# Kizuna42/office-person-detection-vit

Measured on AMD Instinct MI355X. Metric: frames/sec (Phase-2 DETR detect) at 800x1333 batch 8, higher is better.
Workload: dtype f16

## Files before the change

office_person_detection_vit_amd/_capi.py:

```python

from __future__ import annotations

import ctypes as C
import os
from typing import Optional

_HERE = os.path.dirname(os.path.abspath(__file__))
LIB_PATH = os.path.join(_HERE, "libopd_hip.so")
TEST_LIB_PATH = os.path.join(_HERE, "libopd_hip_test.so")

OPD_PIXELS_U8_BGR_HWC = 0
OPD_PIXELS_F32_NCHW = 1
OPD_MEM_HOST = 0
OPD_MEM_DEVICE = 1
OPD_MEM_HOST_PIXELS_DEVICE_OUT = 2
OPD_FLAG_NO_GRAPH = 1
OPD_FLAG_MULTI_STREAM = 2
OPD_REID_MODEL_CLIP = 0
OPD_REID_MODEL_OSNET = 1
OPD_TRACK_FEAT_NONE, OPD_TRACK_FEAT_ENCODER, OPD_TRACK_FEAT_COLOR, OPD_TRACK_FEAT_REID = 0, 1, 2, 3
OPD_FLAG_BF16 = 4
OPD_FLOOR_HOMOGRAPHY, OPD_FLOOR_PWA, OPD_FLOOR_TPS = 0, 1, 2
OPD_FLOOR_VALID, OPD_FLOOR_WITHIN, OPD_FLOOR_EXTRAPOLATED = 1, 2, 4
OPD_FLOOR_MAX_POINTS, OPD_FLOOR_MAX_TRIANGLES, OPD_FLOOR_MAX_ZONES, OPD_FLOOR_MAX_VERTICES = 256, 512, 64, 64
# ... 187 lines not shown
    "opd_lwt_destroy": (None, [C.c_void_p]),
    "opd_lwt_reset": (C.c_int, [C.c_void_p]),
    "opd_lwt_info": (C.c_int, [C.c_void_p, C.POINTER(OpdLwtStatus)]),
    "opd_lwt_update": (C.c_int, [C.c_void_p, C.c_void_p, C.c_int, C.c_int, C.c_int, C.c_void_p, C.c_int, C.c_void_p]),
    "opd_lwt_interpolate": (C.c_int, [C.c_void_p, C.c_void_p, C.c_int, C.c_int, C.c_int, C.POINTER(OpdLwtRec), C.c_int, C.POINTER(C.c_int)]),
    "opd_lwt_get": (C.c_int, [C.c_void_p, C.POINTER(OpdLwtTrack), C.c_int, C.POINTER(C.c_int)]),
    "opd_detr_detect_frames_floor": (C.c_int, [C.c_void_p, C.c_void_p, C.POINTER(C.c_void_p)] + [C.c_int] * 5 + [C.c_float, C.c_int, C.POINTER(OpdDet), C.POINTER(C.c_int32),
                                                C.c_void_p]),
    "opd_last_error": (C.c_char_p, []),
    "opd_version": (C.c_char_p, []),
}

TEST_API = {
    "opd_test_conv_gemm": (C.c_int, [C.c_void_p] * 6 + [C.c_int] * 15),
    "opd_test_gemm_splitk_ln": (C.c_int, [C.c_void_p] * 8 + [C.c_int] * 3),
    "opd_test_gemm_k256": (C.c_int, [C.c_void_p] * 5 + [C.c_int] * 5),
    "opd_test_gemm_ln": (C.c_int, [C.c_void_p] * 8 + [C.c_int] * 2),
    "opd_test_bench_gemm_ln": (C.c_int, [C.c_int] * 4 + [C.POINTER(C.c_float)]),
    "opd_test_gemm_ln_deep": (C.c_int, [C.c_void_p] * 7 + [C.c_int] + [C.c_void_p] * 3 + [C.c_int] * 3),
    "opd_test_set_heads2": (C.c_int, [C.c_int]),
    "opd_test_set_heads_spare_rows": (C.c_int, [C.c_int]),
    "opd_test_enc_ffn": (C.c_int, [C.c_void_p] * 9 + [C.c_int] + [C.c_void_p] * 3 + [C.c_int] * 3 + [C.c_void_p] * 2 + [C.c_int] * 2 + [C.c_void_p] * 5 + [C.c_int]),
    "opd_test_bench_enc_ffn": (C.c_int, [C.c_int] * 6 + [C.POINTER(C.c_float)]),
    "opd_test_bench_conv": (C.c_int, [C.c_int] * 11 + [C.POINTER(C.c_float)]),
    "opd_test_trace_btail": (C.c_int, [C.c_int] * 6 + [C.POINTER(C.c_ulonglong), C.c_int, C.POINTER(C.c_int)]),
    "opd_test_trace_conv": (C.c_int, [C.c_int] * 10 + [C.POINTER(C.c_ulonglong), C.c_int, C.POINTER(C.c_int)]),
    "opd_test_btail": (C.c_int, [C.c_void_p] * 10 + [C.c_int] * 6),
    "opd_test_bench_btail": (C.c_int, [C.c_int] * 8 + [C.POINTER(C.c_float)]),
    "opd_test_bench_btail_sc2": (C.c_int, [C.c_int] * 6 + [C.POINTER(C.c_float)]),
    "opd_test_btail_repeat": (C.c_int, [C.c_void_p] * 8 + [C.c_int] * 6 + [C.POINTER(C.c_int)]),
    "opd_test_attention": (C.c_int, [C.c_void_p] * 4 + [C.c_int] * 4 + [C.c_float]),
    "opd_test_layernorm": (C.c_int, [C.c_void_p] * 5 + [C.c_int]),
    "opd_test_maxpool": (C.c_int, [C.c_void_p] * 2 + [C.c_int] * 6),
    "opd_test_preprocess_u8": (C.c_int, [C.c_void_p] * 2 + [C.c_int] * 5 + [C.c_void_p]),
    "opd_test_attention_masked": (C.c_int, [C.c_void_p] * 4 + [C.c_int] * 4 + [C.c_float, C.c_void_p, C.c_int]),
    "opd_test_stem2": (C.c_int, [C.c_void_p] * 4 + [C.c_int] * 5),
    "opd_test_stem_pool": (C.c_int, [C.c_void_p] * 4 + [C.c_int] * 7),
    "opd_test_set_fuse_stem_pool": (C.c_int, [C.c_void_p, C.c_int]),
    "opd_test_set_pos_shadow": (C.c_int, [C.c_void_p, C.c_int]),
    "opd_test_stem_pool_u8": (C.c_int, [C.c_void_p] * 6 + [C.c_int] * 3),
    "opd_test_set_fuse_btail": (C.c_int, [C.c_void_p, C.c_int]),
    "opd_test_set_fuse_gemm_ln": (C.c_int, [C.c_void_p, C.c_int]),
    "opd_test_f32_to_f16": (C.c_uint16, [C.c_float]),
    "opd_test_f16_to_f32": (C.c_float, [C.c_uint16]),
    "opd_test_normalise_key": (C.c_int, [C.c_char_p, C.c_char_p, C.c_int]),
    "opd_test_inspect_checkpoint": (C.c_int, [C.c_char_p, C.POINTER(C.c_int32)]),
    "opd_test_resize_coeffs": (C.c_int, [C.c_int, C.c_int, C.c_void_p, C.c_void_p, C.c_int]),
    "opd_test_valid_prefix": (C.c_int, [C.c_int] * 3),
    "opd_test_trunk_plan": (C.c_int, [C.c_void_p] + [C.c_int] * 6 + [C.c_void_p, C.c_int, C.c_void_p]),
    "opd_test_trunk_plan_one_launch": (C.c_int, [C.c_void_p] + [C.c_int] * 6 + [C.c_void_p, C.c_void_p, C.c_int]),
    "opd_test_transformer_plan": (C.c_int, [C.c_void_p] + [C.c_int] * 7 + [C.c_void_p, C.c_void_p, C.c_int]),
    "opd_test_sine_pos_embed": (C.c_int, [C.c_int] * 5 + [C.c_void_p]),
    "opd_test_conv_dual": (C.c_int, [C.c_void_p] * 6 + [C.c_int] * 13),
    "opd_test_btail_sc": (C.c_int, [C.c_void_p] * 11 + [C.c_int] * 3),
    "opd_test_btail_sc2": (C.c_int, [C.c_void_p] * 11 + [C.c_int] * 4),
    "opd_test_btail_chain": (C.c_int, [C.c_void_p] * 13 + [C.c_int] * 4),
    "opd_test_bench_attention": (C.c_int, [C.c_void_p] * 3 + [C.c_int] * 6 + [C.c_float, C.c_int, C.POINTER(C.c_float)]),
    "opd_test_trace_attention": (C.c_int, [C.c_void_p] * 3 + [C.c_int] * 6 + [C.c_float, C.c_void_p, C.c_int, C.POINTER(C.c_int)]),
    "opd_test_heads": (C.c_int, [C.c_void_p] * 13 + [C.c_int] * 2),
    "opd_test_postprocess": (C.c_int, [C.c_void_p] * 3 + [C.c_int] * 3 + [C.c_float, C.c_void_p, C.c_void_p]),
    "opd_test_roi_features": (C.c_int, [C.c_void_p] * 2 + [C.c_int] * 3 + [C.c_void_p]),
    "opd_test_set_conv_flags": (C.c_int, [C.c_int]),
    "opd_test_set_gemm_ln_kloop": (C.c_int, [C.c_int]),
    "opd_test_set_encffn_wprefetch": (C.c_int, [C.c_int]),
    "opd_test_set_pos_frames": (C.c_int, [C.c_int]),
    "opd_test_set_repeat": (C.c_int, [C.c_int]),
    "opd_test_repeat_result": (C.c_int, [C.POINTER(C.c_int), C.POINTER(C.c_int)]),
    "opd_test_repeat_selftest": (C.c_int, [C.c_int, C.c_int, C.POINTER(C.c_int)]),
    "opd_test_conv_splitk": (C.c_int, [C.c_void_p] * 4 + [C.c_int] * 13),
    "opd_test_reduce_act16": (C.c_int, [C.c_void_p, C.c_int, C.c_longlong, C.c_longlong, C.c_int, C.c_void_p]),
    "opd_test_gemm_alt": (C.c_int, [C.c_void_p] * 5 + [C.c_int] * 5),
    "opd_test_gemm_frame_bias": (C.c_int, [C.c_void_p] * 4 + [C.c_int] * 7),
    "opd_test_reduce_ln_pos": (C.c_int, [C.c_void_p, C.c_int] + [C.c_void_p] * 5 + [C.c_int] * 2 + [C.c_void_p] * 3 + [C.c_int]),
    "opd_test_set_graph_guard": (C.c_int, [C.c_int]),
    "opd_test_set_alloc_poison": (C.c_int, [C.c_int]),
    "opd_test_check_redzones": (C.c_int, [C.c_void_p]),
    "opd_test_set_taps": (C.c_int, [C.c_void_p, C.c_int]),
    "opd_test_read_taps": (C.c_int, [C.c_void_p, C.c_void_p, C.c_int, C.c_char_p, C.c_int]),
    "opd_test_round_f16_diffused": (C.c_int, [C.c_void_p, C.c_int, C.c_int, C.c_int]),
    "opd_test_dec_qkv": (C.c_int, [C.c_void_p, C.c_void_p, C.c_int] + [C.c_void_p] * 5 + [C.c_int] * 2 + [C.c_void_p] * 4),
    "opd_test_dec_self": (C.c_int, [C.c_void_p] * 10 + [C.c_int, C.c_int, C.c_float, C.c_void_p]),
    "opd_test_attention_map": (C.c_int, [C.c_void_p, C.c_int, C.c_void_p, C.c_int, C.c_void_p] + [C.c_int] * 3 + [C.c_float, C.c_void_p, C.c_int, C.c_void_p]),
    "opd_test_attention_split": (C.c_int, [C.c_void_p] * 3 + [C.c_int] * 4 + [C.c_float, C.c_int, C.c_void_p, C.c_int, C.c_void_p, C.c_void_p]),
    "opd_test_dec_cross_out": (C.c_int, [C.c_void_p, C.c_void_p, C.c_int, C.c_void_p, C.c_int] + [C.c_void_p] * 4 + [C.c_int, C.c_void_p]),
    "opd_test_dec_ffn": (C.c_int, [C.c_void_p] * 4 + [C.c_int, C.c_int, C.c_void_p]),
    "opd_test_bench_dec": (C.c_int, [C.c_int] * 6 + [C.POINTER(C.c_float)]),
    "opd_test_heads_fused": (C.c_int, [C.c_void_p, C.c_void_p, C.c_int] + [C.c_void_p] * 13 + [C.c_int, C.c_int, C.c_void_p, C.c_void_p]),
    "opd_test_set_elem_bf16": (C.c_int, [C.c_int]),
    "opd_test_set_btail_res_regs": (C.c_int, [C.c_int]),
    "opd_test_stem_reduce": (C.c_int, [C.c_void_p] * 10 + [C.c_int] * 4),
    "opd_test_trace_dec_self": (C.c_int, [C.c_int, C.c_int, C.c_void_p]),
    "opd_test_reid_geometry": (C.c_int, [C.c_void_p, C.c_int, C.c_int, C.c_int, C.c_void_p]),
    "opd_test_reid_coeffs": (C.c_int, [C.c_int] * 4 + [C.c_void_p, C.c_void_p, C.c_int]),
    "opd_test_reid_lut": (C.c_int, [C.c_void_p]),
    "opd_test_reid_pixels_host": (C.c_int, [C.c_void_p, C.c_int, C.c_int, C.c_void_p] + [C.c_int] * 3 + [C.c_void_p]),
    "opd_test_reid_pixels": (C.c_int, [C.c_void_p, C.POINTER(C.c_void_p), C.c_void_p, C.c_int, C.c_int, C.c_void_p, C.c_void_p, C.c_int,
                                       C.c_void_p]),
    "opd_test_reid_attention": (C.c_int, [C.c_void_p, C.c_void_p] + [C.c_int] * 3),
    "opd_test_reid_layernorm": (C.c_int, [C.c_void_p] * 5 + [C.c_int] * 3),
    "opd_test_reid_gemm": (C.c_int, [C.c_int, C.c_void_p, C.c_void_p, C.c_void_p, C.c_int, C.c_void_p] + [C.c_int] * 3),
    "opd_test_reid_l2norm": (C.c_int, [C.c_void_p] + [C.c_int] * 2),
    "opd_test_osnet_lut": (C.c_int, [C.c_void_p]),
    "opd_test_osnet_pixels_host": (C.c_int, [C.c_void_p, C.c_int, C.c_int, C.c_void_p, C.c_int, C.c_void_p]),
    "opd_test_osnet_stem": (C.c_int, [C.c_void_p] * 4 + [C.c_int] * 2),
    "opd_test_osnet_gemm": (C.c_int, [C.c_int, C.c_void_p, C.c_int, C.c_int, C.c_void_p, C.c_int, C.c_int, C.c_void_p, C.c_void_p, C.c_void_p,
                                      C.c_int, C.c_void_p] + [C.c_int] * 6),
    "opd_test_osnet_dwconv": (C.c_int, [C.c_void_p] * 4 + [C.c_int] * 7),
    "opd_test_osnet_gate": (C.c_int, [C.c_void_p] * 7 + [C.c_int] * 4),
    "opd_test_osnet_avgpool2": (C.c_int, [C.c_void_p] * 2 + [C.c_int] * 4),
    "opd_test_osnet_head": (C.c_int, [C.c_void_p] * 4 + [C.c_int] * 3),
    "opd_test_reid_kernel_table": (C.c_int, [C.c_void_p, C.POINTER(C.c_void_p), C.c_void_p, C.c_int, C.c_void_p, C.c_void_p, C.c_int, C.c_int,
                                             C.POINTER(OpdKernelStat), C.c_int, C.POINTER(C.c_int)]),
    "opd_test_crop_plan_device": (C.c_int, [C.c_int, C.c_void_p] + [C.c_int] * 3 + [C.c_void_p] * 7 + [C.c_int]),
    "opd_test_crop_plan_host": (C.c_int, [C.c_int, C.c_void_p] + [C.c_int] * 3 + [C.c_void_p] * 7 + [C.c_int]),
    "opd_test_crop_plan_staged": (C.c_int, [C.c_int, C.c_void_p] + [C.c_int] * 3 + [C.c_void_p] * 7 + [C.c_int]),
    "opd_test_nms_plan_host": (C.c_int, [C.POINTER(OpdDet), C.POINTER(C.c_int32), C.c_int, C.c_int, C.c_int, C.c_float]),
    "opd_test_tile_merge_host": (C.c_int, [C.c_void_p, C.c_void_p, C.c_int, C.c_int, C.c_int, C.c_void_p, C.c_int, C.c_int,
                                           C.POINTER(OpdTileParams), C.POINTER(OpdTileDet), C.POINTER(C.c_int32)]),
    "opd_test_tile_resize": (C.c_int, [C.c_void_p, C.c_int, C.c_int, C.c_int, C.c_void_p, C.c_int, C.c_int, C.c_int, C.c_void_p]),
    "opd_flow_test_level": (C.c_int, [C.c_void_p, C.c_int, C.c_int, C.c_void_p, C.POINTER(C.c_int), C.POINTER(C.c_int), C.POINTER(C.c_int)]),
    "opd_floor_test_tables": (C.c_int, [C.POINTER(OpdFloorConfig), C.c_void_p, C.c_void_p, C.c_void_p, C.c_int, C.c_void_p, C.POINTER(C.c_int)]),
    "opd_track_test_matrices": (C.c_int, [C.c_void_p, C.c_void_p, C.c_void_p, C.c_void_p, C.c_int, C.POINTER(C.c_int), C.POINTER(C.c_int)]),
    "opd_track_test_state": (C.c_int, [C.c_void_p, C.c_int, C.c_void_p, C.c_void_p, C.POINTER(C.c_int32), C.c_void_p]),
    "opd_track_test_ingest": (C.c_int, [C.c_int, C.c_void_p] + [C.c_int] * 5 + [C.c_void_p, C.c_int, C.c_void_p, C.c_int, C.c_int, C.c_int] + [C.c_void_p] * 5),
    "opd_track_test_assoc": (C.c_int, [C.c_int] + [C.c_void_p] * 3 + [C.c_int, C.c_int, C.c_void_p, C.c_void_p, C.c_int, C.c_double, C.c_int] + [C.c_void_p] * 12),
    "opd_track_test_bench_assoc": (C.c_int, [C.c_int] + [C.c_void_p] * 3 + [C.c_int, C.c_int, C.c_void_p, C.c_void_p, C.c_int, C.c_double, C.c_int, C.c_int,
                                              C.POINTER(C.c_float), C.POINTER(C.c_float)]),
    "opd_test_lwt_interpolate_scripted": (C.c_int, [C.c_void_p, C.c_void_p, C.c_void_p, C.POINTER(OpdLwtRec), C.c_int, C.POINTER(C.c_int)]),
}

_lib: Optional[C.CDLL] = None
_lib_has_hooks = False


def load_library(test_hooks: bool = False) -> C.CDLL:
    global _lib, _lib_has_hooks
    test_hooks = test_hooks or os.environ.get("OPD_TEST_HOOKS") == "1"
    if _lib is not None:
        if test_hooks and not _lib_has_hooks:
            raise RuntimeError("the product library is already loaded in this process; load the test build first "
                               "(_capi.load_library(test_hooks=True) or OPD_TEST_HOOKS=1)")
        return _lib
    path = TEST_LIB_PATH if test_hooks else LIB_PATH
    if not os.path.exists(path):
        raise RuntimeError(
            f"HIP extension not built: {path} is missing (run `python -c 'import __graft_entry__ as g; g.build()'`). "
            "This package has no CPU fallback.")
    lib = C.CDLL(path)
    for table in (API, TEST_API) if test_hooks else (API,):
        for name, (res, args) in table.items():
            fn = getattr(lib, name)
            fn.restype = res
            fn.argtypes = args
    _lib, _lib_has_hooks = lib, test_hooks
    return lib


def last_error() -> str:
    return load_library().opd_last_error().decode("utf-8", "replace")


def check(rc: int, what: str) -> None:
    if rc != 0:
        raise RuntimeError(f"{what} failed (code {rc}): {last_error()}")
```

office_person_detection_vit_amd/csrc/kernels_attn.hip:

```cpp
#include <hip/hip_runtime.h>
#include <type_traits>
#include <math.h>
#include "opd_kprims.h"

typedef short short4v __attribute__((__vector_size__(4 * sizeof(short))));

namespace {

constexpr float LAZY_T = 8.0f;

__device__ __forceinline__ half4 lds_tr16(const unsigned char* p) {
    short4v t = __builtin_amdgcn_ds_read_tr16_b64_v4i16(
        (__attribute__((address_space(3))) short4v*)(const_cast<unsigned char*>(p)));
    half4 r;
    __builtin_memcpy(&r, &t, 8);
    return r;
}

__device__ __forceinline__ float xmax16_32(const float v) {
    float a = v, b = v;
    asm volatile("s_nop 1\n\tv_permlane16_swap_b32 %0, %1\n\tv_max_f32 %0, %0, %1" : "+v"(a), "+v"(b));
    float c = a;
    asm volatile("s_nop 1\n\tv_permlane32_swap_b32 %0, %1\n\tv_max_f32 %0, %0, %1" : "+v"(a), "+v"(c));
    return a;
}

#define ATTN_STAMP(i)                                                                                        \
    do {                                                                                                     \
        if constexpr (TRACE) {                                                                               \
            unsigned long long now_;                                                                         \
            asm volatile("s_memtime %0\n\ts_waitcnt lgkmcnt(0)" : "=s"(now_)::"memory");                     \
            tsum[i] += now_ - tlast;                                                                         \
            tlast = now_;                                                                                    \
        }                                                                                                    \
    } while (0)

template <bool MASKED, int KT, bool TRACE = false, bool SPLIT = false>
__global__ __launch_bounds__(256) void attention_kernel(AttnParams p) {
    constexpr int NKT = KT / 16;
    constexpr int RPT = KT / 64;
    constexpr int K_BYTES = KT * 64, TILE_BYTES = KT * 128;
    __shared__ __attribute__((aligned(1024))) unsigned char lds[2 * TILE_BYTES];
    const int tid = threadIdx.x;
    const int lane = tid & 63;
    const int wave = __builtin_amdgcn_readfirstlane(tid >> 6);
    const int g = lane >> 4;
    const int li = lane & 15;
    const int nq = (p.Lq + 63) >> 6;
    const int nsp = SPLIT ? p.splits : 1;
    const int total = nq * p.heads * p.B * nsp;
    const int chunk = (total + 7) >> 3;
    const int n0 = (int)(blockIdx.x & 7u) * chunk + (int)(blockIdx.x >> 3);
    if (n0 >= total) return;
    const int split = SPLIT ? n0 % nsp : 0, n = SPLIT ? n0 / nsp : n0;
    const int b = n / (nq * p.heads), h = (n / nq) % p.heads;
    const int q = (n % nq) * 64 + wave * 16 + li;
    const bool q_ok = q < p.Lq;

    half8 qf;
#pragma unroll
    for (int j = 0; j < 8; ++j) qf[j] = (elem_t)0.f;
    if (q_ok) qf = *reinterpret_cast<const half8*>(p.q + ((size_t)b * p.Lq + q) * p.ldq + h * 32 + g * 8);
    half8 ones;
#pragma unroll
    for (int j = 0; j < 8; ++j) ones[j] = (elem_t)1.f;

    const __amdgpu_buffer_rsrc_t rsrc_k = buf_rsrc(p.k, (unsigned)((size_t)p.B * p.Lk * p.ldk * 2));
    const __amdgpu_buffer_rsrc_t rsrc_v = buf_rsrc(p.v, (unsigned)((size_t)p.B * p.Lk * p.ldv * 2));
    const int vr = ((lane >> 4) & 1) * 8 + ((lane >> 1) & 7), vc = (lane >> 5) * 2 + (lane & 1);
    const unsigned koff = (unsigned)(((size_t)b * p.Lk + wave * 16 + (lane & 15)) * p.ldk + h * 32 + (lane >> 4) * 8) * 2u;
    const unsigned voff = (unsigned)(((size_t)b * p.Lk + wave * 16 + vr) * p.ldv + h * 32 + vc * 8) * 2u;
    auto dma_tile = [&](int t, int buf) {
        unsigned char* base = lds + buf * TILE_BYTES;
#pragma unroll
        for (int i = 0; i < RPT; ++i) {
            const int row0 = t * KT + i * 64;
            dma16_buf(rsrc_k, base + (i * 4 + wave) * 1024, koff, (unsigned)(row0 * p.ldk) * 2u);
            dma16_buf(rsrc_v, base + K_BYTES + (i * 4 + wave) * 1024, voff, (unsigned)(row0 * p.ldv) * 2u);
        }
    };

    unsigned long long tsum[5] = {0, 0, 0, 0, 0}, tlast = 0, tbegin = 0, rbegin = 0;
    if constexpr (TRACE) {
        asm volatile("s_memrealtime %0\n\ts_waitcnt lgkmcnt(0)" : "=s"(rbegin)::"memory");
        asm volatile("s_memtime %0\n\ts_waitcnt lgkmcnt(0)" : "=s"(tbegin)::"memory");
        tlast = tbegin;
    }
    float m_ref = -INFINITY;
    float4v oacc[2] = {float4v{0.f, 0.f, 0.f, 0.f}, float4v{0.f, 0.f, 0.f, 0.f}};
    float4v lacc = float4v{0.f, 0.f, 0.f, 0.f};

    const int kv_rows = MASKED ? p.key_valid[2 * b] : 0, kv_cols = MASKED ? p.key_valid[2 * b + 1] : 0;
    const int ntiles = (p.Lk + KT - 1) / KT;
    const int tps = SPLIT ? (ntiles + nsp - 1) / nsp : ntiles;
    const int t0 = split * tps, t1 = SPLIT ? (t0 + tps < ntiles ? t0 + tps : ntiles) : ntiles;
    const float scale2 = p.scale * 1.44269504088896340736f;
    if (SPLIT && t0 >= t1) {
        if (q_ok) {
            const size_t prow = (size_t)split * p.B * p.Lq + (size_t)b * p.Lq + q;
#pragma unroll
            for (int dt = 0; dt < 2; ++dt) *reinterpret_cast<float4v*>(p.part_o + prow * (p.heads * 32) + h * 32 + dt * 16 + g * 4) = float4v{0.f, 0.f, 0.f, 0.f};
            if (g == 0) *reinterpret_cast<float2v*>(p.part_ml + (prow * p.heads + h) * 2) = float2v{-INFINITY, 0.f};
        }
        return;
    }
    dma_tile(t0, 0);
    __syncthreads();

    auto tile_step = [&](const int t, auto last_tag) {
        constexpr bool LAST = decltype(last_tag)::value;
        const int buf = (t - t0) & 1;
        if (!LAST && (!SPLIT || t + 1 < t1)) dma_tile(t + 1, buf ^ 1);
        ATTN_STAMP(0);
        const unsigned char* Kl = lds + buf * TILE_BYTES;
        const unsigned char* Vl = Kl + K_BYTES;

        float4v s[NKT];
#pragma unroll
        for (int kt = 0; kt < NKT; ++kt) {
            const half8 kf = *reinterpret_cast<const half8*>(Kl + kt * 1024 + lane * 16);
            s[kt] = OPD_MFMA_16x16x32(kf, qf, float4v{0.f, 0.f, 0.f, 0.f});
        }
        float mx = -INFINITY;
        if (MASKED) {
#pragma unroll
            for (int kt = 0; kt < NKT; ++kt)
#pragma unroll
                for (int r = 0; r < 4; ++r) {
                    const int key = t * KT + kt * 16 + g * 4 + r;
                    const int kr = key / p.key_row, kc = key - kr * p.key_row;
                    const bool ok = key < p.Lk && kr < kv_rows && kc < kv_cols;
                    s[kt][r] = ok ? s[kt][r] : -INFINITY;
                    mx = fmaxf(mx, s[kt][r]);
                }
        } else if (!LAST) {
#pragma unroll
            for (int kt = 0; kt < NKT; ++kt)
#pragma unroll
                for (int r = 0; r < 4; ++r) mx = fmaxf(mx, s[kt][r]);
        } else {
#pragma unroll
            for (int kt = 0; kt < NKT; ++kt)
#pragma unroll
                for (int r = 0; r < 4; ++r) {
                    const int key = t * KT + kt * 16 + g * 4 + r;
                    s[kt][r] = key < p.Lk ? s[kt][r] : -INFINITY;
                    mx = fmaxf(mx, s[kt][r]);
                }
        }
        if (__any(mx * scale2 > m_ref + LAZY_T)) {
            const float mq = xmax16_32(mx) * scale2;
            const bool up = mq > m_ref + LAZY_T;
            const float m_new = up ? mq : m_ref;
            const float alpha = up ? __builtin_amdgcn_exp2f(m_ref - m_new) : 1.0f;
#pragma unroll
            for (int dt = 0; dt < 2; ++dt)
#pragma unroll
                for (int r = 0; r < 4; ++r) oacc[dt][r] *= alpha;
#pragma unroll
            for (int r = 0; r < 4; ++r) lacc[r] *= alpha;
            m_ref = m_new;
        }
        ATTN_STAMP(1);
        const float mn = (SPLIT && MASKED && m_ref == -INFINITY) ? 0.f : -m_ref;
        const float2v sc2 = {scale2, scale2}, mneg = {mn, mn};
#pragma unroll
        for (int kt = 0; kt < NKT; ++kt)
#pragma unroll
            for (int r = 0; r < 4; r += 2) {
                const float2v a = __builtin_elementwise_fma(float2v{s[kt][r], s[kt][r + 1]}, sc2, mneg);
                s[kt][r] = __builtin_amdgcn_exp2f(a[0]);
                s[kt][r + 1] = __builtin_amdgcn_exp2f(a[1]);
            }
#pragma unroll
        for (int kb = 0; kb < NKT / 2; ++kb) {
            half8 pf;
#pragma unroll
            for (int r = 0; r < 4; ++r) {
                pf[r] = (elem_t)s[2 * kb][r];
                pf[4 + r] = (elem_t)s[2 * kb + 1][r];
            }
#pragma unroll
            for (int dt = 0; dt < 2; ++dt) {
                const unsigned char* a0 = Vl + kb * 2048 + (dt * 32 + (g >> 1) * 16 + ((g & 1) * 4 + (li >> 2)) * 2 + ((li >> 1) & 1)) * 16 + (li & 1) * 8;
                const half4 lo = lds_tr16(a0);
                const half4 hi = lds_tr16(a0 + 1024);
                half8 vf;
#pragma unroll
                for (int r = 0; r < 4; ++r) { vf[r] = lo[r]; vf[4 + r] = hi[r]; }
                oacc[dt] = OPD_MFMA_16x16x32(vf, pf, oacc[dt]);
            }
            lacc = OPD_MFMA_16x16x32(ones, pf, lacc);
        }
        ATTN_STAMP(2);
        if (TRACE && !LAST) { asm volatile("s_waitcnt vmcnt(0)" ::: "memory"); }
        ATTN_STAMP(3);
        __syncthreads();
        ATTN_STAMP(4);
    };
    if constexpr (SPLIT) {
        for (int t = t0; t < t1; ++t) {
            if (t + 1 == ntiles) tile_step(t, std::true_type{});
            else tile_step(t, std::false_type{});
        }
    } else {
        for (int t = 0; t + 1 < ntiles; ++t) tile_step(t, std::false_type{});
        tile_step(ntiles - 1, std::true_type{});
    }

    if constexpr (TRACE) {
        if (tid == 0 && p.trace) {
            unsigned long long rend;
            asm volatile("s_memrealtime %0\n\ts_waitcnt lgkmcnt(0)" : "=s"(rend)::"memory");
            unsigned long long* tr = p.trace + (size_t)blockIdx.x * 12;
            for (int i = 0; i < 5; ++i) tr[i] = tsum[i];
            tr[5] = 0;
            tr[6] = tlast - tbegin;
            tr[7] = (unsigned long long)ntiles;
            tr[8] = rbegin; tr[9] = rend;
            tr[10] = (unsigned long long)__builtin_amdgcn_s_getreg((20 << 0) | (0 << 6) | (3 << 11));
            tr[11] = (unsigned long long)__builtin_amdgcn_s_getreg((4 << 0) | (0 << 6) | (31 << 11));
        }
    }
    if constexpr (SPLIT) {
        if (q_ok) {
            const size_t prow = (size_t)split * p.B * p.Lq + (size_t)b * p.Lq + q;
#pragma unroll
            for (int dt = 0; dt < 2; ++dt) *reinterpret_cast<float4v*>(p.part_o + prow * (p.heads * 32) + h * 32 + dt * 16 + g * 4) = oacc[dt];
            if (g == 0) *reinterpret_cast<float2v*>(p.part_ml + (prow * p.heads + h) * 2) = float2v{m_ref, lacc[0]};
        }
        return;
    }
    if (q_ok) {
        const float inv = 1.0f / lacc[0];
        f16_t* orow = p.o + ((size_t)b * p.Lq + q) * p.ldo + h * 32 + g * 4;
#pragma unroll
        for (int dt = 0; dt < 2; ++dt) {
            half4 o;
#pragma unroll
            for (int r = 0; r < 4; ++r) o[r] = (elem_t)(oacc[dt][r] * inv);
            *reinterpret_cast<half4*>(orow + dt * 16) = o;
        }
    }
}

}

hipError_t OPD_SYM(opd_launch_attention)(const AttnParams& p, hipStream_t stream) {
    if (p.B <= 0 || p.heads <= 0 || p.Lq <= 0 || p.Lk <= 0) return hipErrorInvalidValue;
    if (p.splits > 0) {
        if (!p.part_o || !p.part_ml || p.trace || (p.ldq % 8) || (p.ldk % 8) || (p.ldv % 8) || (p.key_valid && p.key_row < 1)) return hipErrorInvalidValue;
        if ((size_t)p.B * p.Lk * p.ldk * 2 >= (1ull << 32) || (size_t)p.B * p.Lk * p.ldv * 2 >= (1ull << 32)) return hipErrorInvalidValue;
        const int total = ((p.Lq + 63) / 64) * p.heads * p.B * p.splits;
        dim3 grid(8 * ((total + 7) / 8));
        if (p.key_valid) OPD_LAUNCH((attention_kernel<true, 128, false, true>), grid, dim3(256), 0, stream, p);
        else OPD_LAUNCH((attention_kernel<false, 128, false, true>), grid, dim3(256), 0, stream, p);
        return hipGetLastError();
    }
    if ((p.ldq % 8) || (p.ldk % 8) || (p.ldv % 8) || (p.ldo % 4)) return hipErrorInvalidValue;
    if (p.key_valid && p.key_row < 1) return hipErrorInvalidValue;
    if ((size_t)p.B * p.Lk * p.ldk * 2 >= (1ull << 32) || (size_t)p.B * p.Lk * p.ldv * 2 >= (1ull << 32)) return hipErrorInvalidValue;
    const int total = ((p.Lq + 63) / 64) * p.heads * p.B;
    dim3 grid(8 * ((total + 7) / 8));
    const bool wide = p.Lq <= 128 && p.Lk > 128;
    if (p.trace) {
        OPD_LAUNCH((attention_kernel<false, 64, true>), grid, dim3(256), 0, stream, p);
    } else if (p.key_valid) {
        if (wide) OPD_LAUNCH((attention_kernel<true, 128>), grid, dim3(256), 0, stream, p);
        else OPD_LAUNCH((attention_kernel<true, 64>), grid, dim3(256), 0, stream, p);
    } else {
        if (wide) OPD_LAUNCH((attention_kernel<false, 128>), grid, dim3(256), 0, stream, p);
        else OPD_LAUNCH((attention_kernel<false, 64>), grid, dim3(256), 0, stream, p);
    }
    return hipGetLastError();
}
```

office_person_detection_vit_amd/csrc/opd_api.cpp:

```cpp
#include <algorithm>
#include <new>
#include <optional>
#include <stdexcept>

#include "opd_floor.h"
#include "opd_model.h"
#include "opd_nms.h"
#include "opd_reid.h"
#include "opd_tile.h"
#include "opd_track.h"

namespace opd {

static inline bool pixels_on_device(int mem_kind) { return mem_kind == OPD_MEM_DEVICE; }
static inline bool outputs_on_device(int mem_kind) { return mem_kind != OPD_MEM_HOST; }

static int check_device_outputs(int mem_kind, const void* out, const void* counts, const char* who) {
    if (!outputs_on_device(mem_kind)) return OPD_OK;
    if (!device_accessible(out) || !device_accessible(counts))
        return fail(OPD_EINVAL, std::string(who) + ": this mem_kind takes DEVICE output pointers; the ones given are not device-accessible memory");
    return OPD_OK;
}

int check_shape(opd_detr* m, const void* pixels, int pixel_format, int mem_kind, int B, int H, int W) {
// ... 321 lines not shown
        HIPCHK(hipMemcpyAsync(enc_features, m->d_x32, (size_t)B * m->last_fh * m->last_fw * m->arch.d_model * 4, kind, m->stream));
    HIPCHK(hipStreamSynchronize(m->stream));
    if (m->profiling == 1) timed_collect(m);
    return OPD_OK;
}

static int check_tiles(const std::string& who, const opd_tile_params* p, const int32_t* tiles, int n_tiles, int h, int w, bool one_size) {
    if (!p || !tiles) return fail(OPD_EINVAL, who + ": null argument");
    if (p->struct_size != (int32_t)sizeof(opd_tile_params)) return fail(OPD_EINVAL, who + ": opd_tile_params.struct_size mismatch");
    if (n_tiles < 1) return fail(OPD_EINVAL, who + ": n_tiles < 1");
    if (!frame_size_ok(h, w)) return fail(OPD_EINVAL, who + ": frame size " + std::to_string(h) + " x " + std::to_string(w) + " out of range");
    for (int t = 0; t < n_tiles; ++t) {
        const int32_t* g = tiles + 4 * t;
        if (g[0] < 0 || g[1] < 0 || g[2] < 1 || g[3] < 1 || (long long)g[0] + g[2] > h || (long long)g[1] + g[3] > w)
            return fail(OPD_EINVAL, who + ": tile " + std::to_string(t) + " (y0 " + std::to_string(g[0]) + ", x0 " + std::to_string(g[1]) + ", " + std::to_string(g[2]) + " x " +
                                        std::to_string(g[3]) + ") lies outside the " + std::to_string(h) + " x " + std::to_string(w) + " frame");
        if (one_size && (g[2] != tiles[2] || g[3] != tiles[3]))
            return fail(OPD_EINVAL, who + ": tiles of more than one size (" + std::to_string(tiles[2]) + " x " + std::to_string(tiles[3]) + " and " + std::to_string(g[2]) + " x " +
                                        std::to_string(g[3]) + "): one forward has one model size");
    }
    return OPD_OK;
}

static int merge_tiles(opd_detr* m, const opd_det* recs, const int32_t* tile_counts, int n_frames, int n_tiles, int stride, const int32_t* tiles, int h, int w,
                       const opd_tile_params* p, opd_tile_det* out, int32_t* counts) {
    const size_t nt = (size_t)n_frames * n_tiles, nr = nt * stride;
    DevMem tmp;
    TileMergeParams mp{};
    mp.recs = tmp.up(recs, nr); mp.tile_counts = tmp.up(tile_counts, nt); mp.tiles_yxhw = tmp.up(tiles, (size_t)n_tiles * 4);
    mp.out = tmp.alloc<opd_tile_det>(nr); mp.counts = tmp.alloc<int32_t>((size_t)n_frames);
    const int32_t zero = 0;
    mp.flag = tmp.up(&zero, 1);
    if (!tmp.ok) return fail(OPD_ENOMEM, "opd_detr_merge_tiles: device allocation failed");
    fill_tile_merge(&mp, p, n_frames, n_tiles, stride, h, w);
    if (m->profiling == 1) m->timer.reset();
    RCCHK(launch(m, m->stream, CLS_OTHER, 0.0, [&] { return opd_launch_tile_merge(mp, m->stream); }));
    HIPCHK(hipStreamSynchronize(m->stream));
    int32_t over = 0;
    HIPCHK(hipMemcpy(counts, mp.counts, (size_t)n_frames * 4, hipMemcpyDeviceToHost));
    HIPCHK(hipMemcpy(out, mp.out, nr * sizeof(opd_tile_det), hipMemcpyDeviceToHost));
    HIPCHK(hipMemcpy(&over, mp.flag, 4, hipMemcpyDeviceToHost));
    if (m->profiling == 1) timed_collect(m);
    if (over) return fail(OPD_EINVAL, "opd_detr_merge_tiles: a tile holds more records than its slots (its frame comes back empty)");
    return OPD_OK;
}

}

static void drop_streams(opd_detr* m) {
    if (m->ev_fork) (void)hipEventDestroy(m->ev_fork);
    if (m->ev_join) (void)hipEventDestroy(m->ev_join);
    if (m->stream2) (void)hipStreamDestroy(m->stream2);
    if (m->stream) (void)hipStreamDestroy(m->stream);
    m->ev_fork = m->ev_join = nullptr; m->stream2 = m->stream = nullptr;
}

Switches opd::read_switches(int flags) {
    Switches sw;
    auto env = [](const char* name, int* v) { if (const char* e = getenv(name)) *v = atoi(e); };
    env("OPD_DUAL_OVER_TAIL", &sw.dual_over_tail);
    env("OPD_SC2_TAIL", &sw.sc2_tail);
    env("OPD_TAIL_REV", &sw.tail_rev);
    env("OPD_TAIL3", &sw.tail3);
    env("OPD_TAIL_RC", &sw.tail_rc);
    sw.tail_rc = sw.tail_rc != 0;
    env("OPD_WPREFETCH", &sw.wprefetch);
    env("OPD_W8", &sw.w8);
    if (sw.w8 < 0) sw.w8 = (flags & OPD_FLAG_MULTI_STREAM) ? 1 : 0;
    env("OPD_SMALL_SPLITK", &sw.small_splitk);
    env("OPD_SMALL_ENC", &sw.small_enc);
    env("OPD_Y_STRIDE2", &sw.y_stride2);
    env("OPD_RES_DMA128", &sw.res_dma128);
    env("OPD_STEM_REDUCE", &sw.stem_reduce);
    env("OPD_TAIL3_SPLIT", &sw.tail3_split);
    env("OPD_FUSE_PREP", &sw.fuse_prep);
    env("OPD_POS_SHADOW", &sw.pos_shadow);
    env("OPD_DEEP_FC2", &sw.deep_fc2);
    env("OPD_WROUND", &sw.wround);
    env("OPD_FUSED_DEC", &sw.fused_dec);
    env("OPD_FUSED_ENC_FFN", &sw.fused_enc_ffn);
    env("OPD_ENC_TAIL", &sw.enc_tail);
    env("OPD_ENC_FRONT", &sw.enc_front);
    env("OPD_HEADS2", &sw.heads2);
    env("OPD_DBG_DEC_LAYERS", &sw.dbg_dec_layers);
    env("OPD_DBG_BTAIL", &sw.dbg_btail);
    env("OPD_DBG_SKIP", &sw.dbg_skip);
    env("OPD_DBG_GEMM", &sw.dbg_gemm);
    return sw;
}

static int open_handle(std::unique_ptr<opd_detr> m, const StateDict* sd, opd_detr** out) {
    auto cleanup = [&](int code) {
        for (void* p : m->allocs) (void)hipFree(p);
        drop_streams(m.get());
        return code;
    };
    hipError_t he = hipSetDevice(m->device);
    if (he == hipSuccess) he = hipStreamCreateWithFlags(&m->stream, hipStreamNonBlocking);
    if (he == hipSuccess) he = hipStreamCreateWithFlags(&m->stream2, hipStreamNonBlocking);
    if (he == hipSuccess) he = hipEventCreateWithFlags(&m->ev_fork, hipEventDisableTiming);
    if (he == hipSuccess) he = hipEventCreateWithFlags(&m->ev_join, hipEventDisableTiming);
    if (he != hipSuccess) { drop_streams(m.get()); return fail(OPD_EHIP, std::string("device/stream setup failed: ") + hipGetErrorString(he)); }
    int rc;
    if (sd) {
        int cus = 0;
        if (hipDeviceGetAttribute(&cus, hipDeviceAttributeMultiprocessorCount, m->device) == hipSuccess && cus > 0) m->num_cus = cus;
        m->weights = std::make_shared<WeightSet>();
        m->weights->device = m->device;
        if ((rc = build_weights(m.get(), *sd))) return cleanup(rc);
    }
    m->weights_sealed = true;
    if ((rc = build_workspace(m.get()))) return cleanup(rc);
    for (auto& e : m->ev)
        if (hipEventCreate(&e) != hipSuccess) return cleanup(fail(OPD_EHIP, "hipEventCreate failed"));
    *out = m.release();
    ++g_handle_epoch;
    return OPD_OK;
}

static int create_impl(const opd_config* cfg, const char* weights_path, int device_ordinal, opd_detr** out) {
    if (!cfg || !weights_path || !out) return fail(OPD_EINVAL, "opd_detr_create: null argument");
    if (cfg->struct_size != (int32_t)sizeof(opd_config)) return fail(OPD_EINVAL, "opd_config.struct_size mismatch");
    if (cfg->max_batch < 1 || cfg->max_height < 32 || cfg->max_width < 32) return fail(OPD_EINVAL, "opd_config maxima must be >= 1 x 32 x 32");
    StateDict sd;
    std::string err;
    int rc = load_safetensors(weights_path, &sd, &err);
    if (rc) return fail(rc, err);
    std::unique_ptr<opd_detr> m(new opd_detr());
    rc = infer_arch(sd, &m->arch, &err);
    if (rc) return fail(rc, err);
    m->cfg = *cfg;
    m->dtype = (cfg->flags & OPD_FLAG_BF16) ? OPD_DT_BF16 : OPD_DT_F16;
    m->sw = read_switches(cfg->flags);
    m->device = device_ordinal;
    RCCHK(use_device("opd_detr_create", device_ordinal, "device_ordinal out of range"));
    return open_handle(std::move(m), &sd, out);
}

static int clone_impl(const opd_detr* src, opd_detr** out) {
    if (!src || !out) return fail(OPD_EINVAL, "opd_detr_clone: null argument");
    std::unique_ptr<opd_detr> m(new opd_detr());
    static_cast<DetrWeights&>(*m) = *src;
    m->weights = src->weights;
    m->arch = src->arch; m->cfg = src->cfg; m->device = src->device; m->dtype = src->dtype;
    m->sw = src->sw; m->num_cus = src->num_cus;
    return open_handle(std::move(m), nullptr, out);
}

extern "C" {

const char* opd_version(void) {
    const char* text = "";
    (void)api_call_unlocked("opd_version", [&] { text = "opd_hip 0.2 gfx950 (fp16 MFMA operands, fp32 accumulate; OPD_FLAG_BF16: bf16 operands)"; return OPD_OK; });
    return text;
}

int opd_detr_create(const opd_config* cfg, const char* weights_path, int device_ordinal, opd_detr** out) { return api_call("opd_detr_create", [&] {
    if (out) *out = nullptr;
    return create_impl(cfg, weights_path, device_ordinal, out);
}, API_CREATE); }
int opd_detr_clone(const opd_detr* src, opd_detr** out) { return api_call("opd_detr_clone", [&] {
    if (out) *out = nullptr;
    return clone_impl(src, out);
}); }
void opd_detr_destroy(opd_detr* m) { (void)api_call("opd_detr_destroy", [&]() -> int {
    if (!m) return OPD_OK;
// ... 415 lines not shown
```

office_person_detection_vit_amd/csrc/opd_kernels.h:

```cpp
#pragma once
#include <hip/hip_runtime.h>
#include <stdint.h>
#include <vector>
#include "opd_pack.h"

typedef uint16_t f16_t;
enum { OPD_DT_F16 = 0, OPD_DT_BF16 = 1 };

#include <mutex>
#define OPD_SET_MAX_LDS_ONCE(kernel, bytes)                                                                                  \
    do {                                                                                                                     \
        static std::once_flag once_[16];                                                                                     \
        static hipError_t err_[16];                                                                                          \
        int dev_ = 0;                                                                                                        \
        if (hipGetDevice(&dev_) != hipSuccess || dev_ < 0 || dev_ >= 16) return hipErrorInvalidDevice;    \
        std::call_once(once_[dev_], [&] { err_[dev_] = hipFuncSetAttribute(reinterpret_cast<const void*>(kernel), hipFuncAttributeMaxDynamicSharedMemorySize, (bytes)); }); \
        if (err_[dev_] != hipSuccess) return err_[dev_];                                                                     \
    } while (0)

extern thread_local const char* opd_last_kernel_name;
extern thread_local int opd_dbg_skip_launch;
const char* opd_kernel_name(const char* fmt, ...);
#define OPD_LAUNCH(kernel, ...)                       \
    do {                                              \
// ... 246 lines not shown
__host__ __device__ inline bool opd_color_rect(double x, double y, double w, double h, int H, int W, int* x1, int* y1, int* x2, int* y2) {
    *x1 = opd_py_int(fmax(0.0, x));
    *y1 = opd_py_int(fmax(0.0, y));
    *x2 = opd_py_int(fmin((double)W, x + w));
    *y2 = opd_py_int(fmin((double)H, y + h));
    return *x2 > *x1 && *y2 > *y1;
}
struct ColorParams {
    const ColorCrop* crops;
    const void* records;
    const int32_t* counts;
    const uint8_t* frames;
    int Q, fh, fw, label;
    int n;
    uint32_t* acc;
    float* out;
};
hipError_t opd_launch_color_features(const ColorParams& p, int spans, hipStream_t stream);

struct DecQkvParams {
    const float* h_in;
    const float* partials;
    int nsplit;
    const float* b2;
    const float *ln_g, *ln_b;
    float* h_out;
    const f16_t* w;
    const float* bias;
    f16_t* q16;
    f16_t* k16;
    f16_t* vT;
    int M, Q;
};
hipError_t opd_launch_dec_qkv(const DecQkvParams& p, hipStream_t stream);
struct DecSelfParams {
    const f16_t *q16, *k16, *vT;
    float* h;
    const f16_t* wo;
    const float *bo, *ln_g, *ln_b;
    const f16_t* wq;
    const float* rbq;
    f16_t* qc16;
    int qc_bf16;
    int B, Q;
    float scale;
    unsigned long long* trace;
};
hipError_t opd_launch_dec_self(const DecSelfParams& p, hipStream_t stream);
struct DecCrossOutParams {
    const float* part_o;
    const float* part_ml;
    int splits;
    const float* res;
    int res_period;
    float* h;
    const f16_t* wo;
    const float *bo, *ln_g, *ln_b;
    int M;
};
hipError_t opd_launch_dec_cross_out(const DecCrossOutParams& p, hipStream_t stream);
#define OPD_DEC_FFN_CHUNK 128
struct DecFfnParams {
    const float* h;
    const f16_t* w1;
    const float* b1;
    const f16_t* w2;
    float* partials;
    int M, F;
};
hipError_t opd_launch_dec_ffn(const DecFfnParams& p, hipStream_t stream);

struct AttnParams {
    const f16_t *q, *k, *v;
    f16_t* o;
    int B, heads, Lq, Lk;
    int ldq, ldk, ldv, ldo;
    float scale;
    const int32_t* key_valid;
    int key_row;
    unsigned long long* trace;
    int splits;
    float *part_o, *part_ml;
    int dtype;
};
hipError_t opd_launch_attention(const AttnParams& p, hipStream_t stream);

#define OPD_DECL_ELEM(name, ...)          \
    hipError_t name##_f16(__VA_ARGS__);   \
    hipError_t name##_bf16(__VA_ARGS__);
OPD_DECL_ELEM(opd_launch_conv_gemm, const ConvGemmParams& p, hipStream_t stream)
OPD_DECL_ELEM(opd_launch_conv_w8, const ConvGemmParams& p, hipStream_t stream)
OPD_DECL_ELEM(opd_launch_stem_pool_u8, const uint8_t* frames, const int32_t* valid_hw, const f16_t* w, const float* bias, f16_t* out, int B, int H, int W, int OH,
              int OW, int PH, int PW, hipStream_t stream, const StemReduce& red)
OPD_DECL_ELEM(opd_launch_stem_pool, const f16_t* x4p, const f16_t* w, const float* bias, f16_t* out, int B, int Hp, int Wp, int OH, int OW, int PH, int PW,
              hipStream_t stream, const StemReduce& red)
OPD_DECL_ELEM(opd_launch_btail, const BtailParams& p, hipStream_t stream)
OPD_DECL_ELEM(opd_launch_btail256, const BtailParams& p, hipStream_t stream)
OPD_DECL_ELEM(opd_launch_gemm_ln, const GemmLnParams& p, hipStream_t stream)
OPD_DECL_ELEM(opd_launch_enc_ffn, const EncFfnParams& p, hipStream_t stream)
OPD_DECL_ELEM(opd_launch_gemm_k256, const GemmK256Params& p, hipStream_t stream)
OPD_DECL_ELEM(opd_launch_attention, const AttnParams& p, hipStream_t stream)
OPD_DECL_ELEM(opd_launch_attention_map, const f16_t* q, int ldq, const f16_t* k, int ldk, const int32_t* sel, int nsel, int heads, int Lk, float scale,
              const int32_t* key_valid2, int key_row, void* stat, float* out, hipStream_t stream)
OPD_DECL_ELEM(opd_launch_preprocess_u8, const uint8_t* frames, f16_t* out, int B, int H, int W, int Hp, int Wp, const int32_t* valid_hw, hipStream_t stream)
OPD_DECL_ELEM(opd_launch_preprocess_f32, const float* pv, f16_t* out, int B, int H, int W, int Hp, int Wp, const int32_t* valid_hw, hipStream_t stream)
OPD_DECL_ELEM(opd_launch_maxpool, const f16_t* x, f16_t* out, int B, int H, int W, int C, int OH, int OW, hipStream_t stream)
OPD_DECL_ELEM(opd_launch_layernorm, const float* x, const float* gamma, const float* beta, float* y, f16_t* y16, int rows, hipStream_t stream)
OPD_DECL_ELEM(opd_launch_broadcast_rows, const float* c, float* y, f16_t* y16, int rows, hipStream_t stream)
OPD_DECL_ELEM(opd_launch_reduce_ln, const float* partials, int nsplit, size_t slab_stride, const float* residual, const float* gamma, const float* beta, float* y,
              f16_t* y16, int rows, hipStream_t stream)
OPD_DECL_ELEM(opd_launch_reduce_ln_pos, const float* partials, int nsplit, size_t slab_stride, const float* residual, const float* gamma, const float* beta,
              float* y, f16_t* y16, int rows, const float* pos, const float* const* pos_ptrs, int period, f16_t* yp16, hipStream_t stream)
OPD_DECL_ELEM(opd_launch_cast_f16, const float* x, f16_t* y, size_t n, hipStream_t stream)
OPD_DECL_ELEM(opd_launch_reduce_act16, const float* partials, int nsplit, size_t slab_stride, f16_t* out, size_t n, int relu, hipStream_t stream)
```

office_person_detection_vit_amd/csrc/opd_model.cpp:

```cpp
#include <algorithm>

#include "opd_model.h"

namespace opd {

std::atomic<int> g_alloc_poison{-1};

static void compute_dims(int B, int H, int W, Dims* d) {
    d->B = B; d->H = H; d->W = W;
    d->H1 = down2(H); d->W1 = down2(W);
    d->H2 = down2(d->H1); d->W2 = down2(d->W1);
    d->stage_h[0] = d->H2; d->stage_w[0] = d->W2;
    for (int s = 1; s < 4; ++s) { d->stage_h[s] = down2(d->stage_h[s - 1]); d->stage_w[s] = down2(d->stage_w[s - 1]); }
}

int fill_qc0(opd_detr* m) {
    if (!m->qc0 || !m->d_qd16) return OPD_OK;
    const size_t QD = (size_t)m->arch.queries * m->arch.d_model;
    for (int b = 0; b < m->cfg.max_batch; ++b) HIPCHK(hipMemcpy(m->d_qd16 + b * QD, m->qc0, QD * 2, hipMemcpyDeviceToDevice));
    return OPD_OK;
}

static int conv_splits(const opd_detr* m, const Conv& c, int stage) {
    if (!m->sw.small_splitk || stage < 0 || stage > 3 || c.stem || c.K % 64 != 0 || c.Cout % 64 != 0) return 1;
// ... 102 lines not shown
        explicit Unseal(opd_detr* mm) : m(mm) { m->weights_sealed = false; }
        ~Unseal() { m->weights_sealed = true; }
    } unseal(m);
    const Arch& a = m->arch;
    const int D = a.d_model, hw = fh * fw;
    std::unique_ptr<Plan> p(new Plan());
    p->fh = fh; p->fw = fw; p->vh = vh; p->vw = vw;
    std::vector<float> pos;
    sine_pos_embed(fh, fw, vh, vw, D, &pos);
    float* d_pos = nullptr;
    RCCHK(upload_f32(m, &d_pos, pos));
    p->d_pos = d_pos;
    p->rb_enc.resize(a.enc_layers);
    for (int i = 0; i < a.enc_layers; ++i) RCCHK(upload_fold(m, d_pos, m->h_enc_cat_w[i], m->h_enc_cat_b[i], hw, 768, D, &p->rb_enc[i]));
    RCCHK(upload_fold(m, d_pos, m->h_kv_cat_w, m->h_kv_cat_b, hw, a.dec_layers * 512, D, &p->rb_kv));
    HIPCHK(hipStreamSynchronize(m->stream));
    *out = p.get();
    plans.push_back(std::move(p));
    return OPD_OK;
}

static int tap(opd_detr* m, hipStream_t s, const Tap& t) {
    if (!m->taps || !m->d_taps || m->tap_next >= OPD_MAX_TAPS) return OPD_OK;
    HIPCHK(opd_launch_checksum(t.p, t.bytes, m->d_taps + (size_t)m->tap_next * OPD_TAP_BLOCKS, s));
    if ((int)m->tap_names.size() <= m->tap_next) m->tap_names.resize(m->tap_next + 1);
    m->tap_names[m->tap_next++] = t.name;
    return OPD_OK;
}
int launch_end(opd_detr* m, hipStream_t s, std::initializer_list<Tap> taps) {
    if (m->profiling == 1) RCCHK(m->timer.end(s));
    for (const Tap& t : taps)
        if (t.name && t.p) RCCHK(tap(m, s, t));
    return OPD_OK;
}
void timed_collect(opd_detr* m) {
    static const char* const cls_name[4] = {"(convolution)", "(linear layer)", "(attention)", "(other)"};
    for (int c = 0; c < 4; ++c) { m->class_ms[c] = 0.f; m->class_launches[c] = 0; m->class_flops[c] = 0.0; }
    m->ktable.clear();
    (void)m->timer.fold(&m->ktable, cls_name);
    for (const auto& t : m->timer.marks)
        if (t.ms >= 0.f) { m->class_ms[t.cls] += t.ms; m->class_launches[t.cls] += 1; m->class_flops[t.cls] += t.flops; }
    std::sort(m->ktable.begin(), m->ktable.end(), [](const KernelRow& a, const KernelRow& b) { return a.ms > b.ms; });
    for (auto& r : m->ktable) {
        const bool label = std::find_if(cls_name, cls_name + 4, [&](const char* c) { return r.name == c; }) != cls_name + 4;
        if (!label && r.name.size() > 1 && r.name.front() == '(' && r.name.back() == ')') r.name = r.name.substr(1, r.name.size() - 2);
    }
}

struct PosShadow { const float* pos; const float* const* pos_ptrs; int period; f16_t* yp16; };
struct Fwd {
    opd_detr* m;
    hipStream_t stream;
    int B, H, W;
    Dims d;
    int D, F, Q, Md, NKV;
    Plan* plan = nullptr;
    const float* const* enc_bias_ptrs[16] = {};
    const float* const* kv_bias_ptrs = nullptr;
    const float* const* pos_ptrs = nullptr;
    const int32_t *d_valid = nullptr, *d_keyv = nullptr;
    const f16_t* feat = nullptr;
    int fh = 0, fw = 0, hw = 0, M = 0;
    bool shadow = false;
    PosShadow psh{};
    const PosShadow* ps() const { return shadow ? &psh : nullptr; }
    template <typename Fn>
    int launch(int cls, double flops, Fn&& issue, std::initializer_list<Tap> taps = {}) const { return opd::launch(m, stream, cls, flops, issue, taps); }
};

static ConvGemmParams gemm_params(const opd_detr* m, const f16_t* x, const f16_t* w, const float* bias, void* out, int M, int N, int K) {
    ConvGemmParams p{}; p.dtype = m->dtype;
    p.x = x; p.w = w; p.bias = bias; p.out = out; p.zero16 = m->zero_bias;
    p.B = M; p.H = 1; p.W = 1; p.Cin = K; p.OH = 1; p.OW = 1; p.N = N; p.KH = 1; p.KW = 1; p.stride = 1; p.pad = 0;
    p.M = M; p.K = K; p.dbg = m->sw.dbg_gemm; p.wprefetch = m->sw.wprefetch & 1;
    return p;
}
static ConvGemmParams conv_params(const opd_detr* m, const Conv& c, const f16_t* x, int B, int H, int W, int OH, int OW, void* out, bool relu) {
    ConvGemmParams p = gemm_params(m, x, c.w, c.bias, out, B * OH * OW, c.Cout, c.K);
    p.B = B; p.H = H; p.W = W; p.Cin = c.Cin; p.OH = OH; p.OW = OW; p.KH = c.KH; p.KW = c.KW; p.stride = c.stride; p.pad = c.pad;
    p.relu = relu ? 1 : 0; p.stem = c.stem ? 1 : 0;
    return p;
}
static AttnParams attn_params(const Fwd& c, const f16_t* q, int ldq, const f16_t* k, int ldk, const f16_t* v, int ldv, f16_t* o, int ldo, int Lq, int Lk,
                              const int32_t* key_valid, int key_row) {
    AttnParams p{}; p.dtype = c.m->dtype;
    p.key_valid = key_valid; p.key_row = key_row;
    p.q = q; p.k = k; p.v = v; p.o = o; p.B = c.B; p.heads = c.m->arch.heads; p.Lq = Lq; p.Lk = Lk;
    p.ldq = ldq; p.ldk = ldk; p.ldv = ldv; p.ldo = ldo;
    p.scale = 1.0f / sqrtf((float)(c.m->arch.d_model / c.m->arch.heads));
    return p;
}
static double attn_flops(const AttnParams& p) { return 4.0 * p.B * (double)p.heads * p.Lq * p.Lk * 32; }

static int run_conv(const Fwd& c, const Conv& cv, const f16_t* x, int B, int H, int W, int OH, int OW, void* out, bool relu, const f16_t* res16, int stage = -1) {
    opd_detr* m = c.m;
    ConvGemmParams p = conv_params(m, cv, x, B, H, W, OH, OW, out, relu);
    p.res16 = res16;
    const double flops = 2.0 * p.M * (double)cv.Cout * cv.KH * cv.KW * cv.Cin;
    const size_t n = (size_t)p.M * cv.Cout;
    const Tap t{cv.KH == 3 ? "conv3x3" : "conv1x1", out, n * 2};
    if (const int splits = res16 ? 1 : conv_splits(m, cv, stage); splits > 1 && (size_t)splits * n <= m->slab_floats) {
        p.out = m->d_slab; p.out_f32 = 1; p.relu = 0; p.split_k = splits;
        RCCHK(c.launch(CLS_CONV, flops, [&] { return opd_launch_conv_gemm(p, c.stream); }));
        return c.launch(CLS_OTHER, 0.0, [&] { return opd_launch_reduce_act16(m->d_slab, splits, n, reinterpret_cast<f16_t*>(out), n, relu ? 1 : 0, c.stream, m->dtype); }, {t});
    }
    bool w8 = false;
    if (m->sw.w8 && cv.Cout % 256 == 0 && cv.Cout >= 512) {
        const long long tiles = (((long long)OH * OW * m->cfg.max_batch + 127) / 128) * (cv.Cout / 256);
        const bool few = tiles <= 3LL * m->num_cus;
        const int kind = cv.KH == 3 ? (m->sw.w8 & 1) : (cv.K >= 1024 ? (m->sw.w8 & 2) : (cv.K == 512 ? (m->sw.w8 & 4) : 0));
        w8 = few && kind && opd_conv_w8_supported(p);
    }
    return c.launch(CLS_CONV, flops, [&] { return w8 ? opd_launch_conv_w8(p, c.stream) : opd_launch_conv_gemm(p, c.stream); }, {t});
}

static int run_gemm(const Fwd& c, const ConvGemmParams& p) {
    return c.launch(CLS_GEMM, 2.0 * p.M * (double)p.N * p.K, [&] { return opd_launch_conv_gemm(p, c.stream); }, {{"gemm", p.out, (size_t)p.M * p.N * (p.out_f32 ? 4 : 2)}});
}
static int run_linear(const Fwd& c, const f16_t* x, const f16_t* w, const float* bias, int bias_period, int M, int N, int K, f16_t* out, bool relu) {
    ConvGemmParams p = gemm_params(c.m, x, w, bias, out, M, N, K);
    p.bias_period = bias_period; p.relu = relu ? 1 : 0;
    return run_gemm(c, p);
}
static int run_pos_proj(const Fwd& c, const f16_t* w, const float* bias_vec, const float* table, const float* const* table_ptrs, int N, int mod, int pos_cols, f16_t* out) {
    opd_detr* m = c.m;
    ConvGemmParams p = gemm_params(m, c.shadow ? m->d_xp16 : m->d_x16, w, c.shadow ? bias_vec : table, out, c.M, N, c.D);
    if (c.shadow) { p.x_alt = m->d_x16; p.alt_mod = mod; p.alt_cols = pos_cols; }
    else { p.bias_period = c.hw; p.bias_ptrs = table_ptrs; p.bias_pmod = mod; p.bias_pcols = pos_cols; }
    return run_gemm(c, p);
}

static int run_gemm_splitk_ln(const Fwd& c, const f16_t* x, const f16_t* w, const float* bias, int M, int N, int K, int splits, const float* res32,
                              const LNp* ln, float* y32, f16_t* y16, int cls, const PosShadow* ps = nullptr) {
    opd_detr* m = c.m;
    ConvGemmParams p = gemm_params(m, x, w, bias, m->d_slab, M, N, K);
    p.out_f32 = 1; p.split_k = splits; p.dbg = 0; p.wprefetch = 0;
    RCCHK(c.launch(cls, 2.0 * M * (double)N * K, [&] { return opd_launch_conv_gemm(p, c.stream); }, {{"splitk_slabs", m->d_slab, (size_t)splits * M * N * 4}}));
    return c.launch(CLS_OTHER, 0.0, [&] {
        return opd_launch_reduce_ln_pos(m->d_slab, splits, (size_t)M * N, res32, ln ? ln->g : nullptr, ln ? ln->b : nullptr, y32, y16, M, ps ? ps->pos : nullptr,
                                        ps ? ps->pos_ptrs : nullptr, ps ? ps->period : 0, ps ? ps->yp16 : nullptr, c.stream, m->dtype);
    }, {{"reduce_ln", y32, (size_t)M * N * 4}});
}

static int run_gemm_ln(const Fwd& c, const f16_t* x, const f16_t* w, const float* bias, int M, int K, const float* res32, const LNp& ln, float* y32, f16_t* y16) {
    GemmLnParams p{}; p.dtype = c.m->dtype;
    p.x = x; p.w = w; p.bias = bias; p.res32 = res32; p.gamma = ln.g; p.beta = ln.b; p.y32 = y32; p.y16 = y16; p.M = M; p.K = K;
    return c.launch(CLS_GEMM, 2.0 * M * 256.0 * K, [&] { return opd_launch_gemm_ln(p, c.stream); }, {{"gemm_ln", y32, (size_t)M * 256 * 4}});
}
static int run_deep(const Fwd& c, const f16_t* x, const f16_t* w, const float* bias, int K, const float* res32, const LNp* ln, int cls) {
    opd_detr* m = c.m;
    GemmLnParams gp{}; gp.dtype = m->dtype;
    gp.x = x; gp.w = w; gp.bias = bias; gp.res32 = res32; gp.gamma = ln ? ln->g : nullptr; gp.beta = ln ? ln->b : nullptr;
    gp.y32 = m->d_x32; gp.y16 = m->d_x16; gp.M = c.M; gp.K = K; gp.deep_k = 1;
    if (const PosShadow* ps = c.ps()) { gp.pos = ps->pos; gp.pos_ptrs = ps->pos_ptrs; gp.pos_period = ps->period; gp.yp16 = ps->yp16; }
    return c.launch(cls, 2.0 * c.M * (double)c.D * K, [&] { return opd_launch_gemm_ln(gp, c.stream); }, {{ln ? "fc2_ln_ring" : "input_proj_ring", m->d_x32, (size_t)c.M * c.D * 4}});
}

static int run_small_gemm(const Fwd& c, const f16_t* x, const f16_t* w, const float* bias, int bias_period, int M, int N, int K, f16_t* out16, bool relu) {
    GemmK256Params p{}; p.dtype = c.m->dtype;
    p.x = x; p.w = w; p.bias = bias; p.out16 = out16; p.M = M; p.N = N; p.ldx = K; p.ldw = K; p.slices = 1;
    p.bias_period = bias_period; p.relu = relu ? 1 : 0;
    return c.launch(CLS_GEMM, 2.0 * M * (double)N * K, [&] { return opd_launch_gemm_k256(p, c.stream); }, {{"gemm_k256", out16, (size_t)M * N * 2}});
}
static int run_small_gemm_ln(const Fwd& c, const f16_t* x, const f16_t* w, const float* bias, int M, int K, const float* res32, const LNp& ln, float* y32, f16_t* y16) {
    opd_detr* m = c.m;
    GemmK256Params p{}; p.dtype = m->dtype;
    p.x = x; p.w = w; p.bias = bias; p.out32 = m->d_slab; p.M = M; p.N = 256; p.ldx = K; p.ldw = K; p.slices = K / 256;
    RCCHK(c.launch(CLS_GEMM, 2.0 * M * 256.0 * K, [&] { return opd_launch_gemm_k256(p, c.stream); }));
    return c.launch(CLS_OTHER, 0.0, [&] { return opd_launch_reduce_ln(m->d_slab, p.slices, (size_t)M * 256, res32, ln.g, ln.b, y32, y16, M, c.stream, m->dtype); },
                    {{"small_gemm_ln", y32, (size_t)M * 256 * 4}});
}

static int run_attn(const Fwd& c, const f16_t* q, int ldq, const f16_t* k, int ldk, const f16_t* v, int ldv, f16_t* o, int Lq, int Lk,
                    const int32_t* key_valid = nullptr, int key_row = 0) {
    const int D = c.m->arch.d_model;
    const AttnParams p = attn_params(c, q, ldq, k, ldk, v, ldv, o, D, Lq, Lk, key_valid, key_row);
    return c.launch(CLS_ATTN, attn_flops(p), [&] { return opd_launch_attention(p, c.stream); }, {{"attention", o, (size_t)c.B * Lq * D * 2}});
}

TrunkPlan plan_trunk(const Arch& a, const std::vector<Block>& blocks, const opd_config& cfg, const Switches& sw, int B, int H2, int W2, int num_cus,
                     bool taps, int profiling, bool has_stream2) {
    TrunkPlan plan;
    plan.steps.resize(blocks.size());
    plan.split = B;
    const bool multi = (cfg.flags & OPD_FLAG_MULTI_STREAM) != 0;
    int ch = H2, cw = W2, oh3 = 0, ow3 = 0;
    for (int s = 0, bi = 0; s < 4; ++s) {
        for (int l = 0; l < a.depths[s]; ++l, ++bi) {
            const Block& b = blocks[bi];
            const Block* nbk = bi + 1 < (int)blocks.size() ? &blocks[bi + 1] : nullptr;
            const int oh = (b.c1.stride == 2) ? down2(ch) : ch, ow = (b.c1.stride == 2) ? down2(cw) : cw;
            const int C1 = b.c1.Cin;
            const bool sc_in_tail = b.has_sc && sw.fuse_shortcut && sw.fuse_btail && block_has_bias2sc(b) && b.sc.KH == 1 && b.sc.stride == 1 &&
                                    b.sc.Cin == 64 && b.c1.Cin == 64 && b.c1.stride == 1 && b.c2.Cout == 256 && nbk && conv_has_kperm(nbk->c0) &&
                                    nbk->c0.Cin == 256 && nbk->c0.Cout == 64;
            bool tail = sw.fuse_btail && b.c1.KH == 3 && b.c1.Cout == C1 && b.c2.Cin == C1 && b.c2.Cout == 4 * C1 && conv_has_kperm(b.c2) &&
                        opd_btail_supported(C1, 0);
            const bool tail128 = tail && C1 == 128;
            if (sw.dual_over_tail && tail && b.has_sc && !sc_in_tail && block_has_w2sc(b)) tail = false;
            if (C1 == 256 && tail) {
                const long long tiles = ((long long)cfg.max_batch * oh * ow + 127) / 128;
                const bool pays = tiles * 10 >= (long long)num_cus * 6;
                if (sw.tail3 == 0 || (sw.tail3 == 1 && !pays && !multi)) tail = false;
            }
            const bool sc_in_expand = b.has_sc && sw.fuse_shortcut && block_has_w2sc(b) && !sc_in_tail && !tail;
            tail = tail && (size_t)B * ch * cw * C1 * 2 < 0x7ff00000ull;
            TrunkStep& t = plan.steps[bi];
            t.path = tail ? PATH_TAIL : sc_in_expand ? PATH_DUAL : PATH_CONVS;
            t.sc = !b.has_sc ? SC_NONE : (sc_in_tail && tail) ? SC_TAIL : sc_in_expand ? SC_EXPAND : SC_LAUNCH;
            t.res = (t.sc == SC_TAIL || t.sc == SC_EXPAND) ? RES_NONE : t.sc == SC_LAUNCH ? RES_SHORTCUT : RES_TRUNK;
            t.store = STORE_Y;
            t.C3 = 0;
            if (tail && nbk && conv_has_kperm(nbk->c0) && nbk->c0.Cin == 4 * C1 && opd_btail_supported(C1, nbk->c0.Cout)) t.C3 = nbk->c0.Cout;
            t.one_launch = t.one_C3 = t.one_rev = 0;
            if (t.path == PATH_DUAL && sw.sc2_tail && sw.fuse_btail && tail128 && b.sc.KH == 1 && b.sc.stride == b.c1.stride &&
                opd_btail_sc_supported(C1, 0, b.sc.Cin, b.c1.stride) && (size_t)B * ch * cw * b.sc.Cin * 2 < 0x7ff00000ull) {
                t.one_launch = 1;
                if (nbk && conv_has_kperm(nbk->c0) && nbk->c0.Cin == 4 * C1 && opd_btail_sc_supported(C1, nbk->c0.Cout, b.sc.Cin, b.c1.stride)) t.one_C3 = nbk->c0.Cout;
                t.one_rev = sw.tail_rev ? 1 : 0;
            }
            if (tail && sw.y_stride2 && t.C3 && b.c1.stride == 1 && l + 1 == a.depths[s] && nbk && nbk->has_sc && nbk->sc.stride == 2 && nbk->sc.KH == 1 &&
                nbk->c1.stride == 2 && !taps)
                t.store = STORE_Y_STRIDE2;
            if (l > 0 && sw.tail_rc && !taps) {
                TrunkStep& prev = plan.steps[bi - 1];
                if (prev.path == PATH_TAIL && prev.sc == SC_TAIL && prev.C3 == 64 && prev.store == STORE_Y && tail && C1 == 64 && t.C3 == 64 &&
                    t.res == RES_TRUNK) {
                    prev.store = STORE_A1;
                    t.res = RES_REBUILD;
                }
            }
            if (s == 2 && l == 0) { oh3 = oh; ow3 = ow; }
            ch = oh; cw = ow;
        }
    }
    const int s3 = a.depths[0] + a.depths[1], s4 = s3 + a.depths[2];
    bool fused3 = a.depths[2] > 2 && profiling != 1 && !taps && has_stream2 && sw.tail3_split && !multi && B >= 2;
    for (int bi = s3 + 1; bi < s4 && fused3; ++bi) fused3 = plan.steps[bi].path == PATH_TAIL;
    if (fused3) {
        auto tiles_of = [&](int frames) { return ((long long)frames * oh3 * ow3 + 127) / 128; };
        const long long total = tiles_of(B), cus = num_cus, last = total % cus;
        if (total > cus && last > 0 && last < cus / 2) {
            const long long whole = (total / cus) * cus;
            int bA = B - 1;
            while (bA > 1 && tiles_of(bA) > whole) --bA;
            if (tiles_of(bA) <= whole) plan.split = bA;
        }
    }
    int n = 0;
    auto rev = [&](const TrunkStep& t) { return t.path == PATH_TAIL && sw.tail_rev ? (n++ & 1) : 0; };
    for (int bi = 0; bi < s4; ++bi) plan.steps[bi].rev = rev(plan.steps[bi]);
    for (int bi = s3 + 1; bi < s4 && plan.split < B; ++bi) plan.steps[bi].rev_b = rev(plan.steps[bi]);
    for (int bi = s4; bi < (int)blocks.size(); ++bi) plan.steps[bi].rev = rev(plan.steps[bi]);
    return plan;
}

TransformerPlan plan_transformer(const Arch& a, const opd_config& cfg, const Switches& sw, size_t stage4_px, int B, int fh, int fw) {
    TransformerPlan t;
    const int D = a.d_model, F = a.ffn, Q = a.queries, Kp = a.hidden[3];
    const size_t M = (size_t)B * fh * fw, NKV = (size_t)a.dec_layers * 2 * D;
    const bool row256 = D == 256;
    t.shadow = sw.pos_shadow && row256;
    t.small_enc = sw.small_enc && (size_t)cfg.max_batch * stage4_px <= 1400;
    t.enc_splits = t.small_enc ? 8 : 4;
    auto splits_of = [&](int K) { return (K / 64) % t.enc_splits == 0 ? t.enc_splits : 4; };
    auto deep = [&](int K) { return sw.deep_fc2 && row256 && !t.small_enc && K % 64 == 0 && M * K * 2 < 0x7fffff00ull; };
    t.proj_splits = deep(Kp) ? 0 : splits_of(Kp);
    const bool ffn_one = sw.fused_enc_ffn && sw.fuse_gemm_ln && enc_has_ffn_pack(a) && !t.small_enc;
    const int ffn_two = deep(F) ? FFN_FC1_DEEP : FFN_FC1_SPLITK;
    t.enc.resize(a.enc_layers);
    bool prev_tail = false;
    for (int i = 0; i < a.enc_layers; ++i) {
        EncStep& e = t.enc[i];
        const bool last = i + 1 == a.enc_layers;
        e.qkv = prev_tail ? QKV_PREV_TAIL : QKV_LAUNCH;
        e.oproj = ffn_one && sw.enc_front ? OPROJ_IN_FFN : sw.fuse_gemm_ln && row256 ? OPROJ_GEMM_LN : OPROJ_GEMM_THEN_LN;
        e.ffn = ffn_one ? FFN_ONE_LAUNCH : ffn_two;
        e.splits = e.ffn == FFN_FC1_SPLITK ? splits_of(F) : 0;
        e.tail = ffn_one && t.shadow && sw.enc_tail && (!last || M * NKV * 2 < (1ull << 32)) ? enc_pack_tail(a, i) : 0;
        prev_tail = e.tail > 0;
    }
    t.kv_launch = !prev_tail;
    t.dec0 = sw.fuse_dec0 && row256;
    t.dec_fused = sw.fused_dec && t.dec0 && a.heads == 8 && Q <= 128 && (Q & 3) == 0 && F % OPD_DEC_FFN_CHUNK == 0 && F / OPD_DEC_FFN_CHUNK <= 16 &&
                  sw.dec_splits <= 6 && dec_has_frag_weights(a) && M * NKV * 2 < (1ull << 32);
    t.dec_splits = sw.dec_splits;
    t.dec_small_m = sw.small_m_gemm && row256 && F % 256 == 0 && F / 256 <= 8;
    t.dec_oproj = sw.fuse_gemm_ln && row256 ? OPROJ_GEMM_LN : OPROJ_GEMM_THEN_LN;
    t.heads = sw.heads2 && heads_have_frag_weights(a) ? HEADS_SPLIT16 : HEADS_F32;
    t.heads_ln3 = t.dec_fused;
    t.heads_ln = t.dec_fused || sw.fuse_gemm_ln;
    return t;
}

static bool is_ragged(const int32_t* valid_hw, int B, int H, int W) {
    if (!valid_hw) return false;
    for (int b = 0; b < B; ++b)
        if (valid_hw[2 * b] != H || valid_hw[2 * b + 1] != W) return true;
    return false;
}

static int fwd_prepare_ragged(Fwd& c, const int32_t* valid_hw) {
    opd_detr* m = c.m;
    const Arch& a = m->arch;
    const int B = c.B, fh = c.d.stage_h[3], fw = c.d.stage_w[3];
    if (a.enc_layers > 16) return fail(OPD_EINVAL, "ragged batches: at most 16 encoder layers");
    m->h_valid_hw.assign(valid_hw, valid_hw + 2 * B);
    m->h_key_valid.resize((size_t)2 * B);
    m->h_bias_ptrs.assign((size_t)(a.enc_layers + 2) * B, nullptr);
    for (int b = 0; b < B; ++b) {
        const int vh = valid_hw[2 * b], vw = valid_hw[2 * b + 1];
        if (vh < 1 || vw < 1 || vh > c.H || vw > c.W) return fail(OPD_EINVAL, "valid_hw outside the frame canvas");
        const int vfh = valid_prefix(vh, c.H, fh), vfw = valid_prefix(vw, c.W, fw);
        if (vfh < 1 || vfw < 1) return fail(OPD_EINVAL, "frame too small: no valid feature-map position");
        m->h_key_valid[2 * b] = vfh; m->h_key_valid[2 * b + 1] = vfw;
        Plan* pb = nullptr;
        RCCHK(get_plan(m, fh, fw, vfh, vfw, &pb));
        if (b == 0) c.plan = pb;
        for (int i = 0; i < a.enc_layers; ++i) m->h_bias_ptrs[(size_t)i * B + b] = pb->rb_enc[i];
        m->h_bias_ptrs[(size_t)a.enc_layers * B + b] = pb->rb_kv;
        m->h_bias_ptrs[(size_t)(a.enc_layers + 1) * B + b] = pb->d_pos;
    }
    HIPCHK(hipMemcpyAsync(m->d_valid_hw, m->h_valid_hw.data(), (size_t)2 * B * 4, hipMemcpyHostToDevice, c.stream));
    HIPCHK(hipMemcpyAsync(m->d_key_valid, m->h_key_valid.data(), (size_t)2 * B * 4, hipMemcpyHostToDevice, c.stream));
    HIPCHK(hipMemcpyAsync(m->d_bias_ptrs, m->h_bias_ptrs.data(), m->h_bias_ptrs.size() * sizeof(float*), hipMemcpyHostToDevice, c.stream));
    for (int i = 0; i < a.enc_layers; ++i) c.enc_bias_ptrs[i] = m->d_bias_ptrs + (size_t)i * B;
    c.kv_bias_ptrs = m->d_bias_ptrs + (size_t)a.enc_layers * B;
    c.pos_ptrs = m->d_bias_ptrs + (size_t)(a.enc_layers + 1) * B;
    c.d_valid = m->d_valid_hw;
    c.d_keyv = m->d_key_valid;
    return OPD_OK;
}

static bool stem_reduces(const opd_detr* m) {
    if (!m->sw.stem_reduce || !m->sw.fuse_stem_pool || m->taps || m->blocks.empty() || m->arch.depths[0] < 1) return false;
    const Conv& c0 = m->blocks[0].c0;
    return c0.KH == 1 && c0.KW == 1 && c0.stride == 1 && c0.pad == 0 && c0.Cin == 64 && c0.Cout == 64 && c0.w && c0.bias;
}

static int fwd_stem(const Fwd& c, const void* d_pixels, int pixel_format) {
    opd_detr* m = c.m;
    const Dims& d = c.d;
    const int B = c.B, H = c.H, W = c.W;
    const int Hp = 2 * d.H1 + 6, Wp = 2 * d.W1 + 6;
    const bool u8 = pixel_format == OPD_PIXELS_U8_BGR_HWC;
    StemReduce red;
    if (stem_reduces(m)) { red.z0 = m->d_m0; red.w0 = m->blocks[0].c0.w; red.b0 = m->blocks[0].c0.bias; }
    const double flops = 2.0 * B * d.H1 * d.W1 * 64.0 * 147.0 + (red.z0 ? 2.0 * B * d.H2 * d.W2 * 64.0 * 64.0 : 0.0);
    if (m->sw.fuse_prep && m->sw.fuse_stem_pool && u8)
        return c.launch(CLS_CONV, flops, [&] {
            return opd_launch_stem_pool_u8(reinterpret_cast<const uint8_t*>(d_pixels), c.d_valid, m->stem.w, m->stem.bias, m->d_pool, B, H, W, d.H1, d.W1, d.H2, d.W2,
                                           c.stream, m->dtype, red);
        }, {{"stem_pool_u8", m->d_pool, (size_t)B * d.H2 * d.W2 * 64 * 2}});
    RCCHK(c.launch(CLS_OTHER, 0.0, [&] {
        return u8 ? opd_launch_preprocess_u8(reinterpret_cast<const uint8_t*>(d_pixels), m->d_x4, B, H, W, Hp, Wp, c.d_valid, c.stream, m->dtype)
                  : opd_launch_preprocess_f32(reinterpret_cast<const float*>(d_pixels), m->d_x4, B, H, W, Hp, Wp, c.d_valid, c.stream, m->dtype);
    }));
    if (m->sw.fuse_stem_pool)
        return c.launch(CLS_CONV, flops, [&] { return opd_launch_stem_pool(m->d_x4, m->stem.w, m->stem.bias, m->d_pool, B, Hp, Wp, d.H1, d.W1, d.H2, d.W2, c.stream, m->dtype, red); });
    ConvGemmParams p = gemm_params(m, m->d_x4, m->stem.w, m->stem.bias, m->d_stem, B * d.H1 * d.W1, 64, 256);
    p.B = B; p.H = Hp; p.W = Wp; p.OH = d.H1; p.OW = d.W1; p.stride = 2; p.relu = 1; p.stem = 2;
    p.dbg = 0; p.wprefetch = 0;
    RCCHK(c.launch(CLS_CONV, 2.0 * p.M * 64.0 * 147.0, [&] { return opd_launch_conv_gemm(p, c.stream); }));
// ... 34 lines not shown
            BtailParams p{}; p.dtype = m->dtype;
            p.x1 = x1; p.w1 = b.c1.w; p.b1 = b.c1.bias; p.w2p = C1 == 256 ? b.c2.wp : b.c2.w; p.b2 = b.c2.bias; p.res = res;
            p.y = t.store == STORE_A1 ? nullptr : out;
            if (t.sc == SC_TAIL || t.one_launch) { p.xs = cur; p.wsc = b.sc.w; p.b2 = b.bias2sc; }
            f16_t* z = mid(1 - x1_id, (size_t)oh * ow * C3);
            if (C3) { p.w3p = C1 == 256 ? nbk->c0.wp : nbk->c0.w; p.b3 = nbk->c0.bias; p.z = z; }
            f16_t* const a1_keep = m->d_sc + (size_t)b0 * oh * ow * C1;
            if (t.store == STORE_A1) p.a1_out = a1_keep;
            if (t.res == RES_REBUILD) {
                const Block& pb = m->blocks[bi - 1];
                p.rc = 1; p.rc_a1 = a1_keep; p.rc_xs = trunk(st.prev_id, (size_t)ch * cw * pb.c0.Cin); p.rc_w2 = pb.c2.w; p.rc_wsc = pb.sc.w; p.rc_b = pb.bias2sc;
            }
            p.y_stride2 = t.store == STORE_Y_STRIDE2;
            p.B = nb; p.H = ch; p.W = cw; p.OH = oh; p.OW = ow; p.stride = b.c1.stride; p.M = nb * oh * ow; p.C1 = C1; p.C3 = C3;
            p.rev = t.one_launch ? t.one_rev : b0 ? t.rev_b : t.rev;
            p.dbg = m->sw.dbg_btail | (C1 == 128 && !m->sw.res_dma128 ? 16 : 0);
            RCCHK(c.launch(CLS_CONV, 2.0 * p.M * ((double)C1 * 9 * C1 + 4.0 * C1 * C1 + 4.0 * C1 * C3 + (p.xs ? (double)b.sc.Cin * C2 : 0.0)),
                           [&] { return opd_launch_btail(p, c.stream); },
                           {{"btail_y", p.y ? out : nullptr, (size_t)p.M * 4 * C1 * 2}, {"btail_z", C3 ? z : nullptr, (size_t)p.M * C3 * 2}}));
            if (C3) st.z_id = 1 - x1_id;
        } else {
            f16_t* a1 = mid(1 - x1_id, (size_t)oh * ow * C1);
            RCCHK(run_conv(c, b.c1, x1, nb, ch, cw, oh, ow, a1, true, nullptr, s));
            if (t.path == PATH_DUAL) {
                ConvGemmParams p = gemm_params(m, a1, b.w2sc, b.bias2sc, out, nb * oh * ow, C2, C1 + b.sc.Cin);
                p.B = nb; p.H = oh; p.W = ow; p.OH = oh; p.OW = ow; p.Cin = C1; p.K1 = C1; p.relu = 1;
                p.x2 = cur; p.H2 = ch; p.W2 = cw; p.Cin2 = b.sc.Cin; p.stride2 = b.sc.stride;
                RCCHK(c.launch(CLS_CONV, 2.0 * p.M * (double)C2 * p.K, [&] { return opd_launch_conv_gemm(p, c.stream); }, {{"dual_expand", out, (size_t)p.M * C2 * 2}}));
            } else {
                RCCHK(run_conv(c, b.c2, a1, nb, oh, ow, oh, ow, out, true, res));
            }
        }
        st.prev_id = st.cur_id; st.cur_id = out_id; st.ch = oh; st.cw = ow;
    }
    return OPD_OK;
}

static int trunk_stage3_split(const Fwd& c, const TrunkPlan& tp, TrunkState& st) {
    opd_detr* m = c.m;
    RCCHK(trunk_blocks(c, tp, 2, 0, c.B, st, 0, 1));
    if (tp.split == c.B) return trunk_blocks(c, tp, 2, 0, c.B, st, 1);
    TrunkState ta = st, tb = st;
    Fwd c2 = c;
    c2.stream = m->stream2;
    HIPCHK(hipEventRecord(m->ev_fork, c.stream));
    HIPCHK(hipStreamWaitEvent(m->stream2, m->ev_fork, 0));
    const int rc_a = trunk_blocks(c, tp, 2, 0, tp.split, ta, 1);
    const int rc_b = rc_a == OPD_OK ? trunk_blocks(c2, tp, 2, tp.split, c.B - tp.split, tb, 1) : OPD_OK;
    const hipError_t ej = hipEventRecord(m->ev_join, m->stream2);
    const hipError_t ew = ej == hipSuccess ? hipStreamWaitEvent(c.stream, m->ev_join, 0) : ej;
    RCCHK(rc_a);
    RCCHK(rc_b);
    HIPCHK(ew);
    st = ta;
    return OPD_OK;
}

static int fwd_trunk(Fwd& c) {
    opd_detr* m = c.m;
    const TrunkPlan tp = plan_trunk(m->arch, m->blocks, m->cfg, m->sw, c.B, c.d.H2, c.d.W2, m->num_cus, m->taps != 0, m->profiling, m->stream2 != nullptr);
    TrunkState st{0, c.d.H2, c.d.W2, stem_reduces(m) ? 0 : -1, -1};
    for (int s = 0; s < 4; ++s) {
        RCCHK(s == 2 ? trunk_stage3_split(c, tp, st) : trunk_blocks(c, tp, s, 0, c.B, st));
        MARK(2 + s);
    }
    c.feat = st.cur_id == 1 ? m->d_t0 : m->d_t1;
    c.fh = st.ch; c.fw = st.cw; c.hw = st.ch * st.cw; c.M = c.B * c.hw;
    return OPD_OK;
}

static int fwd_encoder(Fwd& c, const TransformerPlan& tp) {
    opd_detr* m = c.m;
    const Arch& a = m->arch;
    const int M = c.M, D = c.D, F = c.F;
    c.shadow = tp.shadow;
    c.psh = PosShadow{c.plan->d_pos, c.pos_ptrs, c.hw, m->d_xp16};
    const PosShadow* ps = c.ps();
    if (!tp.proj_splits) RCCHK(run_deep(c, c.feat, m->proj.w, m->proj.bias, m->proj.K, nullptr, nullptr, CLS_CONV));
    else RCCHK(run_gemm_splitk_ln(c, c.feat, m->proj.w, m->proj.bias, M, D, m->proj.K, tp.proj_splits, nullptr, nullptr, m->d_x32, m->d_x16, CLS_CONV, ps));
    for (int i = 0; i < a.enc_layers; ++i) {
        const EncLayer& L = m->enc[i];
        const EncStep& e = tp.enc[i];
        if (e.qkv == QKV_LAUNCH) RCCHK(run_pos_proj(c, L.wqkv, L.bqkv, c.plan->rb_enc[i], c.enc_bias_ptrs[i], 3 * D, 3 * D, 2 * D, m->d_qkv16));
        RCCHK(run_attn(c, m->d_qkv16, 3 * D, m->d_qkv16 + D, 3 * D, m->d_qkv16 + 2 * D, 3 * D, m->d_attn16, c.hw, c.hw, c.d_keyv, c.fw));
        if (e.oproj == OPROJ_GEMM_LN) {
            RCCHK(run_gemm_ln(c, m->d_attn16, L.o.w, L.o.b, M, D, m->d_x32, L.ln1, m->d_x32, m->d_x16));
        } else if (e.oproj == OPROJ_GEMM_THEN_LN) {
            ConvGemmParams p = gemm_params(m, m->d_attn16, L.o.w, L.o.b, m->d_y32, M, D, D);
            p.out_f32 = 1; p.res32 = m->d_x32;
            RCCHK(run_gemm(c, p));
            RCCHK(c.launch(CLS_OTHER, 0.0, [&] { return opd_launch_layernorm(m->d_y32, L.ln1.g, L.ln1.b, m->d_x32, m->d_x16, M, c.stream, m->dtype); }));
        }
        if (e.ffn == FFN_ONE_LAUNCH) {
            const bool front = e.oproj == OPROJ_IN_FFN, last = i + 1 == a.enc_layers;
            EncFfnParams fp{}; fp.dtype = m->dtype; fp.wprefetch = (m->sw.wprefetch >> 1) & 1;
            fp.x = m->d_x16; fp.wpack = L.ffn_pack; fp.b2 = L.fc2.b; fp.res32 = m->d_x32; fp.gamma = L.ln2.g; fp.beta = L.ln2.b;
            fp.y32 = m->d_x32; fp.y16 = m->d_x16; fp.M = M; fp.F = F; fp.pack_tail = enc_pack_tail(a, i); fp.pack_front = 1;
            if (front) { fp.attn = m->d_attn16; fp.bo = L.o.b; fp.gamma1 = L.ln1.g; fp.beta1 = L.ln1.b; }
            if (ps) { fp.pos = ps->pos; fp.pos_ptrs = ps->pos_ptrs; fp.pos_period = ps->period; fp.yp16 = ps->yp16; }
            if (e.tail) {
                fp.tail = e.tail; fp.tail_pos = L.tail_pos; fp.tail_ld = L.tail_ld;
                fp.tail_out = last ? m->d_memkv16 : m->d_qkv16;
                for (int t = 0; t < e.tail; ++t) fp.tail_col[t] = L.tail_col[t];
            }
            RCCHK(c.launch(CLS_GEMM, 4.0 * M * (double)D * F + 2.0 * M * (double)D * 256 * (fp.tail + (front ? 1 : 0)), [&] { return opd_launch_enc_ffn(fp, c.stream); },
                           {{"enc_ffn", m->d_x32, (size_t)M * D * 4}}));
        } else {
            RCCHK(run_linear(c, m->d_x16, L.fc1.w, L.fc1.b, 0, M, F, D, m->d_ffn16, true));
            if (e.ffn == FFN_FC1_DEEP) RCCHK(run_deep(c, m->d_ffn16, L.fc2.w, L.fc2.b, F, m->d_x32, &L.ln2, CLS_GEMM));
            else RCCHK(run_gemm_splitk_ln(c, m->d_ffn16, L.fc2.w, L.fc2.b, M, D, F, e.splits, m->d_x32, &L.ln2, m->d_x32, m->d_x16, CLS_GEMM, ps));
        }
    }
    return OPD_OK;
}

static int fwd_memory_kv(const Fwd& c, const TransformerPlan& tp) {
    if (!tp.kv_launch) return OPD_OK;
    return run_pos_proj(c, c.m->wkv_all, c.m->bkv_all, c.plan->rb_kv, c.kv_bias_ptrs, c.NKV, 2 * c.D, c.D, c.m->d_memkv16);
}

static int fwd_decoder_fused(const Fwd& c, const TransformerPlan& tp, const float** final_h) {
    opd_detr* m = c.m;
    const Arch& a = m->arch;
    const int B = c.B, D = c.D, F = c.F, Q = c.Q, Md = c.Md;
    const int S = tp.dec_splits, nchunk = F / OPD_DEC_FFN_CHUNK;
    float* hbuf[2] = {m->d_h32, m->d_yd32};
    int cur = 0;
    for (int i = 0; i < a.dec_layers && i < m->sw.dbg_dec_layers; ++i) {
        const DecLayer& L = m->dec[i];
        f16_t* qd = m->d_qd16 + (size_t)i * m->cfg.max_batch * Q * D;
        if (i > 0) {
            const DecLayer& P = m->dec[i - 1];
            DecQkvParams qp{};
            qp.h_in = hbuf[cur]; qp.partials = m->d_ffn_part; qp.nsplit = nchunk; qp.b2 = P.fc2.b; qp.ln_g = P.ln3.g; qp.ln_b = P.ln3.b;
            qp.h_out = hbuf[cur ^ 1]; qp.w = L.wqkv_f; qp.bias = L.rb_self;
            qp.q16 = m->d_dq16; qp.k16 = m->d_dk16; qp.vT = m->d_dvT; qp.M = Md; qp.Q = Q;
            cur ^= 1;
            RCCHK(c.launch(CLS_GEMM, 2.0 * Md * 768.0 * D, [&] { return opd_launch_dec_qkv(qp, c.stream); }, {{"dec_qkv_h", hbuf[cur], (size_t)Md * D * 4}}));
            DecSelfParams sp{};
            sp.q16 = m->d_dq16; sp.k16 = m->d_dk16; sp.vT = m->d_dvT; sp.h = hbuf[cur]; sp.wo = L.so_f; sp.bo = L.so.b;
            sp.ln_g = L.ln1.g; sp.ln_b = L.ln1.b; sp.wq = L.wqc_f; sp.rbq = L.rb_q; sp.qc16 = qd; sp.qc_bf16 = m->dtype == OPD_DT_BF16; sp.B = B; sp.Q = Q;
            sp.scale = 1.0f / sqrtf((float)(D / a.heads));
            RCCHK(c.launch(CLS_GEMM, 4.0 * Md * (double)D * D + 4.0 * B * (double)a.heads * Q * Q * 32, [&] { return opd_launch_dec_self(sp, c.stream); },
                           {{"dec_self_h", hbuf[cur], (size_t)Md * D * 4}}));
        }
        AttnParams ap = attn_params(c, qd, D, m->d_memkv16 + (size_t)i * 2 * D, c.NKV, m->d_memkv16 + (size_t)i * 2 * D + D, c.NKV, nullptr, D, Q, c.hw, c.d_keyv, c.fw);
        ap.splits = S; ap.part_o = m->d_part_o; ap.part_ml = m->d_part_ml;
        RCCHK(c.launch(CLS_ATTN, attn_flops(ap), [&] { return opd_launch_attention(ap, c.stream); }, {{"dec_cross_part", m->d_part_o, (size_t)S * Md * D * 4}}));
        DecCrossOutParams cp{};
        cp.part_o = m->d_part_o; cp.part_ml = m->d_part_ml; cp.splits = S;
        cp.res = i == 0 ? m->dec0_h : hbuf[cur]; cp.res_period = i == 0 ? 1 : 0; cp.h = hbuf[cur];
        cp.wo = L.co_f; cp.bo = L.co.b; cp.ln_g = L.ln2.g; cp.ln_b = L.ln2.b; cp.M = Md;
        RCCHK(c.launch(CLS_GEMM, 2.0 * Md * (double)D * D, [&] { return opd_launch_dec_cross_out(cp, c.stream); }, {{"dec_cross_h", hbuf[cur], (size_t)Md * D * 4}}));
        DecFfnParams fp{};
        fp.h = hbuf[cur]; fp.w1 = L.fc1_f; fp.b1 = L.fc1.b; fp.w2 = L.fc2_f;
        fp.partials = m->d_ffn_part; fp.M = Md; fp.F = F;
        RCCHK(c.launch(CLS_GEMM, 4.0 * Md * (double)D * F, [&] { return opd_launch_dec_ffn(fp, c.stream); }, {{"dec_ffn_part", m->d_ffn_part, (size_t)nchunk * Md * D * 4}}));
    }
    *final_h = hbuf[cur];
    return OPD_OK;
}

static int fwd_decoder_chain(const Fwd& c, const TransformerPlan& tp) {
    opd_detr* m = c.m;
    const Arch& a = m->arch;
    const int D = c.D, F = c.F, Q = c.Q, Md = c.Md;
    if (tp.dec0) {
        RCCHK(c.launch(CLS_OTHER, 0.0, [&] { return opd_launch_broadcast_rows(m->dec0_h, m->d_h32, m->d_h16, Md, c.stream, m->dtype); },
                       {{"dec0_broadcast", m->d_h32, (size_t)Md * D * 4}}));
    } else {
        HIPCHK(hipMemsetAsync(m->d_h32, 0, (size_t)Md * D * 4, c.stream));
        HIPCHK(hipMemsetAsync(m->d_h16, 0, (size_t)Md * D * 2, c.stream));
    }
    auto linear = [&](const f16_t* x, const f16_t* w, const float* bias, int bias_period, int N, int K, f16_t* out, bool relu) {
        return tp.dec_small_m ? run_small_gemm(c, x, w, bias, bias_period, Md, N, K, out, relu) : run_linear(c, x, w, bias, bias_period, Md, N, K, out, relu);
    };
    auto out_proj_ln = [&](const Lin& o, const LNp& ln) {
        return tp.dec_oproj == OPROJ_GEMM_LN ? run_gemm_ln(c, m->d_attnd16, o.w, o.b, Md, D, m->d_h32, ln, m->d_h32, m->d_h16)
                                              : run_gemm_splitk_ln(c, m->d_attnd16, o.w, o.b, Md, D, D, 4, m->d_h32, &ln, m->d_h32, m->d_h16, CLS_GEMM);
    };
    for (int i = 0; i < a.dec_layers && i < m->sw.dbg_dec_layers; ++i) {
        const DecLayer& L = m->dec[i];
        if (!(tp.dec0 && i == 0)) {
            RCCHK(linear(m->d_h16, L.wqkv, L.rb_self, Q, 3 * D, D, m->d_qkvd16, false));
            RCCHK(run_attn(c, m->d_qkvd16, 3 * D, m->d_qkvd16 + D, 3 * D, m->d_qkvd16 + 2 * D, 3 * D, m->d_attnd16, Q, Q));
            RCCHK(out_proj_ln(L.so, L.ln1));
        }
        f16_t* qd = m->d_qd16 + (size_t)i * m->cfg.max_batch * Q * D;
        RCCHK(linear(m->d_h16, L.wq_c, L.rb_q, Q, D, D, qd, false));
        RCCHK(run_attn(c, qd, D, m->d_memkv16 + (size_t)i * 2 * D, c.NKV, m->d_memkv16 + (size_t)i * 2 * D + D, c.NKV, m->d_attnd16, Q, c.hw, c.d_keyv, c.fw));
        RCCHK(out_proj_ln(L.co, L.ln2));
        RCCHK(linear(m->d_h16, L.fc1.w, L.fc1.b, 0, F, D, m->d_ffnd16, true));
        if (tp.dec_small_m) RCCHK(run_small_gemm_ln(c, m->d_ffnd16, L.fc2.w, L.fc2.b, Md, F, m->d_h32, L.ln3, m->d_h32, m->d_h16));
        else RCCHK(run_gemm_splitk_ln(c, m->d_ffnd16, L.fc2.w, L.fc2.b, Md, D, F, 8, m->d_h32, &L.ln3, m->d_h32, m->d_h16, CLS_GEMM));
    }
    return OPD_OK;
}

static int fwd_heads(const Fwd& c, const TransformerPlan& tp, const float* h) {
    opd_detr* m = c.m;
    const Arch& a = m->arch;
    HeadParams hp{};
    hp.hs = h;
    if (tp.heads_ln3) {
        const DecLayer& P = m->dec[a.dec_layers - 1];
        hp.partials = m->d_ffn_part; hp.nsplit = c.F / OPD_DEC_FFN_CHUNK; hp.ffn_b2 = P.fc2.b; hp.ln3_gamma = P.ln3.g; hp.ln3_beta = P.ln3.b;
    }
    if (tp.heads_ln) {
        hp.ln_gamma = m->dec_ln.g; hp.ln_beta = m->dec_ln.b;
    } else {
        RCCHK(c.launch(CLS_OTHER, 0.0, [&] { return opd_launch_layernorm(h, m->dec_ln.g, m->dec_ln.b, m->d_hs32, nullptr, c.Md, c.stream, m->dtype); }));
        hp.hs = m->d_hs32;
    }
    hp.wc = m->wc; hp.bc = m->bc; hp.w1 = m->w1; hp.b1 = m->b1; hp.w2 = m->w2; hp.b2 = m->b2;
    hp.w3 = m->w3; hp.b3 = m->b3; hp.logits = m->d_logits; hp.boxes = m->d_boxes; hp.rows = c.Md; hp.ncls = a.ncls;
    const bool split16 = tp.heads == HEADS_SPLIT16;
    if (split16) { hp.wc_f = m->wc_f; hp.w1_f = m->w1_f; hp.w2_f = m->w2_f; }
    return c.launch(CLS_OTHER, 2.0 * c.Md * 256.0 * (a.ncls + 256 + 256 + 4), [&] { return split16 ? opd_launch_heads2(hp, c.stream) : opd_launch_heads(hp, c.stream); },
                    {{"heads_logits", m->d_logits, (size_t)c.Md * a.ncls * 4}});
}

static int enqueue_forward(opd_detr* m, const void* d_pixels, int pixel_format, int B, int H, int W, const int32_t* valid_hw = nullptr) {
    const Arch& a = m->arch;
    Fwd c{};
    c.m = m; c.stream = m->stream; c.B = B; c.H = H; c.W = W;
    compute_dims(B, H, W, &c.d);
    c.D = a.d_model; c.F = a.ffn; c.Q = a.queries; c.Md = B * c.Q; c.NKV = a.dec_layers * 2 * c.D;
    const bool ragged = is_ragged(valid_hw, B, H, W);
    if (ragged) RCCHK(fwd_prepare_ragged(c, valid_hw));
// ... 57 lines not shown
```

office_person_detection_vit_amd/csrc/opd_model.h:

```cpp
#pragma once
#include <math.h>
#include <stdlib.h>
#include <string.h>

#include <atomic>
#include <initializer_list>
#include <memory>
#include <mutex>
#include <shared_mutex>
#include <string>
#include <vector>

#include "opd_device.h"
#include "opd_kernels.h"
#include "opd_loader.h"

namespace opd {


struct Conv {
    f16_t* w = nullptr;
    f16_t* wp = nullptr;
    float* bias = nullptr;
    int Cin = 0, Cout = 0, KH = 1, KW = 1, stride = 1, pad = 0, K = 0;
    bool stem = false;
};
struct Lin {
    f16_t* w = nullptr;
    float* b = nullptr;
    int N = 0, K = 0;
};
struct LNp {
    float* g = nullptr;
    float* b = nullptr;
};
struct Block {
    Conv c0, c1, c2, sc;
    bool has_sc = false;
    float* bias2sc = nullptr;
    f16_t* w2sc = nullptr;
};
inline bool conv_has_kperm(const Conv& c) { return c.KH == 1 && c.KW == 1 && c.Cin % 32 == 0 && c.Cin <= 1024; }
inline bool block_has_bias2sc(const Block& b) { return b.has_sc && b.sc.Cout == b.c2.Cout; }
inline bool block_has_w2sc(const Block& b) {
    return block_has_bias2sc(b) && b.sc.KH == 1 && b.c2.KH == 1 && b.c2.Cout % 128 == 0 && b.c2.Cin >= 128;
}
inline bool enc_has_ffn_pack(const Arch& a) { return a.d_model == 256 && a.ffn % 128 == 0; }
inline int enc_pack_tail(const Arch& a, int i, int* pos = nullptr) {
    const bool last = i + 1 == a.enc_layers;
    const int n = !last ? 3 : 2 * a.dec_layers <= 16 ? 2 * a.dec_layers : 0;
    if (pos) *pos = !last ? 2 : n / 2;
    return n;
}
inline bool dec_has_frag_weights(const Arch& a) { return a.d_model % 32 == 0 && a.ffn % 32 == 0; }
inline bool heads_have_frag_weights(const Arch& a) { return a.d_model == 256 && a.ncls <= 128; }
struct EncLayer {
    f16_t* wqkv = nullptr;
    float* bqkv = nullptr;
    Lin o, fc1, fc2;
    LNp ln1, ln2;
    unsigned char* ffn_pack = nullptr;
    int tail_pos = 0, tail_ld = 0;
    int tail_col[16] = {};
};
struct DecLayer {
    f16_t* wqkv = nullptr;
    f16_t* wq_c = nullptr;
    Lin so, co, fc1, fc2;
    LNp ln1, ln2, ln3;
    float* rb_self = nullptr;
    float* rb_q = nullptr;
    f16_t *wqkv_f = nullptr, *so_f = nullptr, *wqc_f = nullptr, *co_f = nullptr, *fc1_f = nullptr, *fc2_f = nullptr;
};

struct Plan {
    int fh = 0, fw = 0;
    int vh = 0, vw = 0;
    std::vector<float*> rb_enc;
    float* rb_kv = nullptr;
    float* d_pos = nullptr;
};

struct Dims {
    int B, H, W, H1, W1, H2, W2;
    int stage_h[4], stage_w[4];
};

inline int down2(int n) { return (n - 1) / 2 + 1; }

struct Switches {
    int small_m_gemm = 1;
    int fuse_gemm_ln = 1;
    int deep_fc2 = 1;
    int fuse_dec0 = 1;
    int enc_front = 1;
    int enc_tail = 0;
    int fused_enc_ffn = 1;
    int fused_dec = 1;
    int dec_splits = 3;
    int heads2 = 1;
    int fuse_btail = 1;
    int fuse_shortcut = 1;
    int dual_over_tail = 1;
    int sc2_tail = 1;
    int tail_rev = 1;
    int tail3 = 1;
    int tail3_split = 1;
    int tail_rc = 1;
    int y_stride2 = 1;
    int stem_reduce = 1;
    int res_dma128 = 1;
    int wprefetch = 3;
    int w8 = -1;
    int small_splitk = 1;
    int small_enc = 1;
    int fuse_stem_pool = 1;
    int fuse_prep = 1;
    int pos_shadow = 1;
    int wround = 1;
    int dbg_btail = 0, dbg_gemm = 0;
    int dbg_dec_layers = 1 << 20;
    int dbg_skip = 0;
};

enum TrunkPath { PATH_TAIL, PATH_CONVS, PATH_DUAL };
enum TrunkShortcut { SC_NONE, SC_TAIL, SC_EXPAND, SC_LAUNCH };
enum TrunkResidual { RES_NONE, RES_TRUNK, RES_SHORTCUT, RES_REBUILD };
enum TrunkStore { STORE_Y, STORE_A1, STORE_Y_STRIDE2 };
struct TrunkStep {
    int path, sc, res, store;
    int C3;
    int rev, rev_b;
    int one_launch;
    int one_C3;
    int one_rev;
};
struct TrunkPlan {
    std::vector<TrunkStep> steps;
    int split = 0;
};
TrunkPlan plan_trunk(const Arch& a, const std::vector<Block>& blocks, const opd_config& cfg, const Switches& sw, int B, int H2, int W2, int num_cus,
                     bool taps, int profiling, bool has_stream2);

enum EncQkv { QKV_LAUNCH, QKV_PREV_TAIL };
enum OutProj { OPROJ_IN_FFN, OPROJ_GEMM_LN, OPROJ_GEMM_THEN_LN };
enum EncFfn { FFN_ONE_LAUNCH, FFN_FC1_DEEP, FFN_FC1_SPLITK };
enum HeadsKernel { HEADS_F32, HEADS_SPLIT16 };
struct EncStep {
    int qkv, oproj, ffn;
    int splits;
    int tail;
};
struct TransformerPlan {
    bool shadow = false;
    bool small_enc = false;
    int enc_splits = 4;
    int proj_splits = 0;
    std::vector<EncStep> enc;
    bool kv_launch = true;
    bool dec_fused = false;
    int dec_splits = 0;
    bool dec0 = false;
    bool dec_small_m = false;
    int dec_oproj = OPROJ_GEMM_LN;
    int heads = HEADS_F32;
    bool heads_ln3 = false;
    bool heads_ln = false;
};
struct FrameBounds { size_t lvl[6], side[6]; };
FrameBounds frame_bounds(const opd_config& cfg);
TransformerPlan plan_transformer(const Arch& a, const opd_config& cfg, const Switches& sw, size_t stage4_px, int B, int fh, int fw);
Switches read_switches(int flags);

}

using namespace opd;

struct RedZoned { void* base; size_t bytes; int poison; };
struct WeightSet {
    std::vector<void*> allocs;
    std::vector<RedZoned> zoned;
    int device = 0;
    std::mutex plan_mu;
    std::vector<std::unique_ptr<Plan>> plans;
    ~WeightSet() {
        (void)hipSetDevice(device);
        for (void* p : allocs) (void)hipFree(p);
    }
};

struct DetrWeights {
    int64_t weight_bytes = 0;
    Conv stem;
    std::vector<Block> blocks;
    std::vector<int> stage_first;
    Conv proj;
    std::vector<EncLayer> enc;
    std::vector<DecLayer> dec;
    f16_t* wkv_all = nullptr;
    float* bkv_all = nullptr;
    float* dec0_h = nullptr;
    f16_t* qc0 = nullptr;
    LNp dec_ln;
    float *wc = nullptr, *bc = nullptr, *w1 = nullptr, *b1 = nullptr, *w2 = nullptr, *b2 = nullptr, *w3 = nullptr, *b3 = nullptr;
    f16_t *wc_f = nullptr, *w1_f = nullptr, *w2_f = nullptr;
    float* zero_bias = nullptr;

    std::vector<std::vector<float>> h_enc_cat_w, h_enc_cat_b;
    std::vector<float> h_kv_cat_w, h_kv_cat_b;
};

struct opd_detr : DetrWeights {
    Arch arch;
    opd_config cfg{};
    Switches sw;
    int dtype = 0;
    int device = 0;
    hipStream_t stream = nullptr;
    hipStream_t stream2 = nullptr;
    hipEvent_t ev_fork = nullptr, ev_join = nullptr;
    std::vector<void*> allocs;
    std::vector<RedZoned> zoned;
    std::shared_ptr<WeightSet> weights;
    bool weights_sealed = false;
    int64_t workspace_bytes = 0;

    uint8_t* d_u8 = nullptr;
    float* d_pv = nullptr;
    f16_t *d_x4 = nullptr, *d_stem = nullptr, *d_pool = nullptr, *d_t0 = nullptr, *d_t1 = nullptr, *d_m0 = nullptr,
          *d_m1 = nullptr, *d_sc = nullptr;
    float *d_x32 = nullptr, *d_y32 = nullptr, *d_slab = nullptr;
    f16_t* d_xp16 = nullptr;
    f16_t *d_x16 = nullptr, *d_qkv16 = nullptr, *d_attn16 = nullptr, *d_ffn16 = nullptr, *d_memkv16 = nullptr;
    float *d_h32 = nullptr, *d_yd32 = nullptr, *d_hs32 = nullptr;
    f16_t *d_h16 = nullptr, *d_qkvd16 = nullptr, *d_qd16 = nullptr, *d_attnd16 = nullptr, *d_ffnd16 = nullptr;
    f16_t *d_dq16 = nullptr, *d_dk16 = nullptr, *d_dvT = nullptr;
    float *d_part_o = nullptr, *d_part_ml = nullptr, *d_ffn_part = nullptr;
    float *d_logits = nullptr, *d_boxes = nullptr;
    opd_det* d_records = nullptr;
    int32_t *d_counts = nullptr, *d_orig_hw = nullptr;
    int32_t *d_valid_hw = nullptr, *d_key_valid = nullptr;
    const float** d_bias_ptrs = nullptr;
    std::vector<int32_t> h_valid_hw, h_key_valid;
    std::vector<const float*> h_bias_ptrs;
    hipEvent_t ev_async[4] = {};
    unsigned async_next = 0;
    bool async_pending[4] = {};
    struct AsyncHost { void* pinned = nullptr; opd_det* out = nullptr; int32_t* counts = nullptr; int B = 0; };
    AsyncHost async_host[4];
    void* sync_pinned = nullptr;
    uint32_t* d_color_acc = nullptr;
    opd_floor_rec* d_floor = nullptr;
    opd_floor_rec* h_floor = nullptr;
    float* d_feat_all = nullptr;
// ... 139 lines not shown
```

office_person_detection_vit_amd/csrc/opd_test_api.cpp:

```cpp
#include <string.h>

#include <algorithm>
#include <vector>

#include "opd_test_util.h"

using namespace opd;

int opd::g_conv_flags = 0, opd::g_gemm_ln_kloop = 0, opd::g_test_dtype = 0, opd::g_encffn_wprefetch = 0, opd::g_pos_frames = 0, opd::g_btail_dbg = 0;
TAPI int opd_test_set_encffn_wprefetch(int on) { g_encffn_wprefetch = on ? 1 : 0; return OPD_OK; }
TAPI int opd_test_set_pos_frames(int frames) { g_pos_frames = frames > 0 ? frames : 0; return OPD_OK; }
TAPI int opd_test_set_elem_bf16(int on) { g_test_dtype = on ? OPD_DT_BF16 : OPD_DT_F16; return OPD_OK; }
TAPI int opd_test_set_conv_flags(int flags) { g_conv_flags = flags; return OPD_OK; }
TAPI int opd_test_set_gemm_ln_kloop(int on) { g_gemm_ln_kloop = on ? 1 : 0; return OPD_OK; }
TAPI int opd_test_set_btail_res_regs(int on) { g_btail_dbg = on ? 16 : 0; return OPD_OK; }

static int g_repeat = 0, g_rep_launches = 0, g_rep_diff = 0, g_rep_keep = 0;
TAPI int opd_test_set_repeat(int reps) {
    g_repeat = reps >= 2 ? reps : 0;
    g_rep_launches = g_rep_diff = 0;
    return OPD_OK;
}
TAPI int opd_test_repeat_result(int* launches, int* n_diff) {
    if (!launches || !n_diff) return fail(OPD_EINVAL, "repeat_result: null pointer");
// ... 521 lines not shown
    p.x1 = dm.up(x1, HW * C1);
    p.w1 = dm.up(w1, (size_t)C1 * 9 * C1);
    p.b1 = dm.up(b1, C1);
    btail_weights(dm, p, C1, C3, w2, w3);
    p.b2 = dm.up(b2sc, C2);
    p.xs = dm.up(xs, HW * Csc);
    p.wsc = dm.up(wsc, (size_t)C2 * Csc);
    p.y = dm.alloc<uint16_t>(M * C2);
    p.b3 = C3 ? dm.up(b3, C3) : nullptr;
    p.z = C3 ? dm.alloc<uint16_t>(M * C3) : nullptr;
    if (!dm.ok) return fail(OPD_ENOMEM, "test alloc failed");
    RCCHK(launch_repeated([&](int rep) { p.rev = rep & 1; return LAUNCHED(opd_launch_btail(p, nullptr)); }, {{p.y, M * C2 * 2, 0xff}, {p.z, M * C3 * 2, 0xff}}));
    HIPCHK(hipDeviceSynchronize());
    RCCHK(down(y, p.y, M * C2));
    return C3 ? down(z, p.z, M * C3) : OPD_OK;
}

TAPI int opd_test_btail_chain(const uint16_t* x1, const uint16_t* xs, const uint16_t* const* w1, const float* const* b1, const uint16_t* const* w2,
                              const float* const* b2, const uint16_t* wsc, const uint16_t* const* w3, const float* const* b3, uint16_t* const* yb,
                              uint16_t* const* zb, uint16_t* const* yc, uint16_t* const* zc, int B, int H, int W, int fill) {
    DevMem dm;
    const size_t M = (size_t)B * H * W;
    const uint16_t* d_x1 = dm.up(x1, M * 64);
    const uint16_t* d_xs = dm.up(xs, M * 64);
    const uint16_t* d_wsc = dm.up(wsc, (size_t)256 * 64);
    const uint16_t *d_w1[3], *d_w2[3], *d_w3[3];
    const float *d_b1[3], *d_b2[3], *d_b3[3];
    for (int i = 0; i < 3; ++i) {
        const int c3 = i == 2 ? 128 : 64;
        d_w1[i] = dm.up(w1[i], (size_t)64 * 9 * 64); d_b1[i] = dm.up(b1[i], 64);
        d_w2[i] = dm.up(w2[i], (size_t)256 * 64); d_b2[i] = dm.up(b2[i], 256);
        d_w3[i] = dm.up(w3[i], (size_t)c3 * 256); d_b3[i] = dm.up(b3[i], c3);
    }
    uint16_t* ya = dm.alloc<uint16_t>(M * 256);
    uint16_t* za = dm.alloc<uint16_t>(M * 64);
    uint16_t* a1a = dm.alloc<uint16_t>(M * 64);
    uint16_t* d_yb = dm.alloc<uint16_t>(M * 256);
    uint16_t* d_zb = dm.alloc<uint16_t>(M * 64);
    uint16_t* d_yc = dm.alloc<uint16_t>(M * 256);
    uint16_t* d_zc = dm.alloc<uint16_t>(M * 128);
    if (!dm.ok) return fail(OPD_ENOMEM, "test alloc failed");
    for (int route = 0; route < 2; ++route) {
        HIPCHK(hipMemset(ya, 0xEE, M * 256 * 2));
        HIPCHK(hipMemset(d_yc, fill, M * 256 * 2));
        auto base = [&](int i, const uint16_t* in, uint16_t* y, uint16_t* z, int c3) {
            BtailParams p{}; p.dtype = g_test_dtype;
            p.x1 = in; p.w1 = d_w1[i]; p.b1 = d_b1[i]; p.w2p = d_w2[i]; p.b2 = d_b2[i]; p.y = y; p.w3p = d_w3[i]; p.b3 = d_b3[i]; p.z = z;
            btail_geometry(p, B, H, W, 1, 64, c3);
            return p;
        };
        BtailParams pa = base(0, d_x1, ya, za, 64);
        pa.xs = d_xs; pa.wsc = d_wsc;
        if (route) { pa.y = nullptr; pa.a1_out = a1a; }
        HIPCHK(opd_launch_btail(pa, nullptr));
        BtailParams pb = base(1, za, d_yb, d_zb, 64);
        if (route) { pb.rc = 1; pb.rc_a1 = a1a; pb.rc_xs = d_xs; pb.rc_w2 = d_w2[0]; pb.rc_wsc = d_wsc; pb.rc_b = d_b2[0]; }
        else pb.res = ya;
        HIPCHK(opd_launch_btail(pb, nullptr));
        BtailParams pc = base(2, d_zb, d_yc, d_zc, 128);
        pc.y_stride2 = route;
        pc.res = d_yb;
        HIPCHK(opd_launch_btail(pc, nullptr));
        HIPCHK(hipDeviceSynchronize());
        RCCHK(down(yb[route], d_yb, M * 256));
        RCCHK(down(zb[route], d_zb, M * 64));
        RCCHK(down(yc[route], d_yc, M * 256));
        RCCHK(down(zc[route], d_zc, M * 128));
    }
    return OPD_OK;
}

static int attention_params(DevMem& dm, AttnParams& p, const uint16_t* q, const uint16_t* k, const uint16_t* v, int B, int heads, int Lq, int Lk,
                            float scale, const int32_t* key_valid, int key_row) {
    const int D = heads * 32;
    p.dtype = g_test_dtype;
    p.q = dm.up(q, (size_t)B * Lq * D);
    p.k = dm.up(k, (size_t)B * Lk * D);
    p.v = dm.up(v, (size_t)B * Lk * D);
    p.key_valid = key_valid ? dm.up(key_valid, (size_t)B * 2) : nullptr;
    p.B = B; p.heads = heads; p.Lq = Lq; p.Lk = Lk; p.ldq = p.ldk = p.ldv = p.ldo = D; p.scale = scale; p.key_row = key_row;
    return D;
}
static int run_attention(const uint16_t* q, const uint16_t* k, const uint16_t* v, uint16_t* o, int B, int heads, int Lq, int Lk, float scale,
                         const int32_t* key_valid, int key_row) {
    DevMem dm;
    AttnParams p{};
    const size_t n = (size_t)B * Lq * attention_params(dm, p, q, k, v, B, heads, Lq, Lk, scale, key_valid, key_row);
    p.o = dm.alloc<uint16_t>(n);
    if (!dm.ok) return fail(OPD_ENOMEM, "test alloc failed");
    RCCHK(launch_repeated([&](int) { return LAUNCHED(opd_launch_attention(p, nullptr)); }, {{p.o, n * 2, 0xff}}));
    HIPCHK(hipDeviceSynchronize());
    return down(o, p.o, n);
}
TAPI int opd_test_attention(const uint16_t* q, const uint16_t* k, const uint16_t* v, uint16_t* o, int B, int heads, int Lq, int Lk,
                            float scale) {
    return run_attention(q, k, v, o, B, heads, Lq, Lk, scale, nullptr, 0);
}
TAPI int opd_test_attention_masked(const uint16_t* q, const uint16_t* k, const uint16_t* v, uint16_t* o, int B, int heads, int Lq,
                                   int Lk, float scale, const int32_t* key_valid, int key_row) {
    return run_attention(q, k, v, o, B, heads, Lq, Lk, scale, key_valid, key_row);
}
TAPI int opd_test_attention_split(const uint16_t* q, const uint16_t* k, const uint16_t* v, int B, int heads, int Lq, int Lk, float scale, int splits,
                                  const int32_t* key_valid, int key_row, float* part_o, float* part_ml) {
    DevMem dm;
    AttnParams p{};
    const int D = attention_params(dm, p, q, k, v, B, heads, Lq, Lk, scale, key_valid, key_row);
    const size_t no = (size_t)splits * B * Lq * D, nm = (size_t)splits * B * Lq * heads * 2;
    p.part_o = dm.alloc<float>(no); p.part_ml = dm.alloc<float>(nm); p.splits = splits;
    if (!dm.ok) return fail(OPD_ENOMEM, "test alloc failed");
    RCCHK(launch_repeated([&](int) { return LAUNCHED(opd_launch_attention(p, nullptr)); }, {{p.part_o, no * 4, 0xff}, {p.part_ml, nm * 4, 0xff}}));
    HIPCHK(hipDeviceSynchronize());
    RCCHK(down(part_o, p.part_o, no));
    return down(part_ml, p.part_ml, nm);
}

TAPI int opd_test_attention_map(const uint16_t* q, int ldq, const uint16_t* k, int ldk, const int32_t* sel, int nsel, int heads, int Lk, float scale,
                                const int32_t* key_valid2, int key_row, float* out) {
    if (!q || !k || !sel || !out || nsel <= 0 || heads <= 0 || Lk <= 0 || key_row <= 0 || ldq < heads * 32 || ldk < heads * 32)
        return fail(OPD_EINVAL, "attention_map: bad arguments");
    int qrows = 0;
    for (int i = 0; i < nsel; ++i) {
        if (sel[i] < 0) return fail(OPD_EINVAL, "attention_map: negative query index");
        qrows = std::max(qrows, sel[i] + 1);
    }
    DevMem dm;
    const uint16_t* dq = dm.up(q, (size_t)qrows * ldq);
    const uint16_t* dk = dm.up(k, (size_t)Lk * ldk);
    const int32_t* dsel = dm.up(sel, (size_t)nsel);
    const int32_t* dvalid = key_valid2 ? dm.up(key_valid2, 2) : nullptr;
    float* stat = dm.alloc<float>((size_t)nsel * heads * 2);
    float* dout = dm.alloc<float>((size_t)Lk);
    if (!dm.ok) return fail(OPD_ENOMEM, "test alloc failed");
    HIPCHK(opd_launch_attention_map(dq, ldq, dk, ldk, dsel, nsel, heads, Lk, scale, dvalid, key_row, stat, dout, nullptr, g_test_dtype));
    HIPCHK(hipDeviceSynchronize());
    return down(out, dout, (size_t)Lk);
}

TAPI int opd_test_layernorm(const float* x, const float* g, const float* b, float* y, uint16_t* y16, int rows) {
    DevMem dm;
    const size_t n = (size_t)rows * 256;
    const float* dx = dm.up(x, n);
    const float* dg = dm.up(g, 256);
    const float* db = dm.up(b, 256);
    float* dy = dm.alloc<float>(n);
    uint16_t* dy16 = dm.alloc<uint16_t>(n);
    if (!dm.ok) return fail(OPD_ENOMEM, "test alloc failed");
    HIPCHK(opd_launch_layernorm(dx, dg, db, dy, dy16, rows, nullptr, g_test_dtype));
    HIPCHK(hipDeviceSynchronize());
    RCCHK(down(y, dy, n));
    return down(y16, dy16, n);
}

TAPI int opd_test_maxpool(const uint16_t* x, uint16_t* out, int B, int H, int W, int C, int OH, int OW) {
    DevMem dm;
    const size_t n = (size_t)B * OH * OW * C;
    const uint16_t* dx = dm.up(x, (size_t)B * H * W * C);
    uint16_t* dout = dm.alloc<uint16_t>(n);
    if (!dm.ok) return fail(OPD_ENOMEM, "test alloc failed");
    HIPCHK(opd_launch_maxpool(dx, dout, B, H, W, C, OH, OW, nullptr, g_test_dtype));
    HIPCHK(hipDeviceSynchronize());
    return down(out, dout, n);
}

TAPI int opd_test_preprocess_u8(const uint8_t* frames, uint16_t* out, int B, int H, int W, int Hp, int Wp, const int32_t* valid_hw) {
    DevMem dm;
    const size_t n = (size_t)B * Hp * Wp * 4;
    const uint8_t* din = dm.up(frames, (size_t)B * H * W * 3);
    uint16_t* dout = dm.alloc<uint16_t>(n);
    const int32_t* dvalid = valid_hw ? dm.up(valid_hw, (size_t)B * 2) : nullptr;
    if (!dm.ok) return fail(OPD_ENOMEM, "test alloc failed");
    HIPCHK(opd_launch_preprocess_u8(din, dout, B, H, W, Hp, Wp, dvalid, nullptr, g_test_dtype));
    HIPCHK(hipDeviceSynchronize());
    return down(out, dout, n);
}

TAPI int opd_test_stem2(const uint16_t* x4p, const uint16_t* w, const float* bias, uint16_t* out, int B, int Hp, int Wp, int OH, int OW) {
    DevMem dm;
    ConvGemmParams p{}; p.dtype = g_test_dtype;
    conv_geometry(p, B, Hp, Wp, 256, OH, OW, 64, 1, 1, 2, 0);
    p.K = 256; p.relu = 1; p.stem = 2;
    const size_t n = (size_t)p.M * 64;
    p.x = dm.up(x4p, (size_t)B * Hp * Wp * 4);
    p.w = dm.up(w, (size_t)64 * 256);
    p.bias = dm.up(bias, 64);
    p.zero16 = zeros<float>(dm, 64);
    uint16_t* dout = dm.alloc<uint16_t>(n);
    p.out = dout;
    if (!dm.ok) return fail(OPD_ENOMEM, "test alloc failed");
    HIPCHK(opd_launch_conv_gemm(p, nullptr));
    HIPCHK(hipDeviceSynchronize());
    return down(out, dout, n);
}

TAPI int opd_test_stem_pool(const uint16_t* x4p, const uint16_t* w, const float* bias, uint16_t* out, int B, int Hp, int Wp, int OH, int OW,
                            int PH, int PW) {
    DevMem dm;
// ... 246 lines not shown
```

office_person_detection_vit_amd/csrc/opd_test_bench_api.cpp:

```cpp
#include <vector>

#include "opd_test_util.h"

using namespace opd;

TAPI int opd_test_bench_gemm_ln(int M, int K, int deep, int iters, float* us_out) {
    DevMem dm;
    GemmLnParams p{}; p.dtype = g_test_dtype;
    p.x = filled16(dm, (size_t)M * K, 0x2c);
    p.w = filled16(dm, (size_t)256 * K, 0x1c);
    float* f = zeros<float>(dm, 1024);
    float* res = zeros<float>(dm, (size_t)M * 256);
    p.y16 = dm.alloc<uint16_t>((size_t)M * 256);
    if (!dm.ok) return fail(OPD_ENOMEM, "bench alloc failed");
    p.bias = f; p.gamma = f + 256; p.beta = f + 512; p.res32 = res; p.y32 = res; p.M = M; p.K = K; p.deep_k = deep;
    return time_launches(3, iters, [&] { return opd_launch_gemm_ln(p, nullptr); }, us_out);
}

TAPI int opd_test_bench_enc_ffn(int M, int F, int iters, int dbg, int tail, int front, float* us_out) {
    if (M <= 0 || F <= 0 || F % 128) return fail(OPD_EINVAL, "bench_enc_ffn: F must be a multiple of 128");
    DevMem dm;
    EncFfnParams p{}; p.dtype = g_test_dtype;
    uint16_t* x = filled16(dm, (size_t)M * 256, 0x2c);
    p.wpack = filled<unsigned char>(dm, opd_encffn_pack_bytes(F, tail, 1), 0x1c);
// ... 73 lines not shown
TAPI int opd_test_trace_btail(int B, int H, int W, int C1, int C3, int dbg, unsigned long long* trace_out, int max_wgs, int* wgs_out) {
    if (!opd_btail_supported(C1, C3)) return fail(OPD_EINVAL, "btail: unsupported (C1, C3)");
    DevMem dm;
    const int wgs = (int)(((size_t)B * H * W + 127) / 128);
    if (wgs > max_wgs) return fail(OPD_EINVAL, "trace buffer too small");
    BtailParams p{};
    btail_layer(dm, p, B, H, W, C1, C3, 1, dbg);
    unsigned long long* tr = zeros<unsigned long long>(dm, (size_t)wgs * 16);
    if (!dm.ok) return fail(OPD_ENOMEM, "trace alloc failed");
    for (int i = 0; i < 2; ++i) HIPCHK(opd_launch_btail(p, nullptr));
    p.trace = tr;
    HIPCHK(opd_launch_btail(p, nullptr));
    HIPCHK(hipDeviceSynchronize());
    *wgs_out = wgs;
    return down(trace_out, tr, (size_t)wgs * 16);
}

TAPI int opd_test_bench_btail(int B, int H, int W, int C1, int C3, int stride, int dbg, int iters, float* us_out) {
    if (!opd_btail_supported(C1, C3)) return fail(OPD_EINVAL, "btail: unsupported (C1, C3)");
    DevMem dm;
    const int C2 = 4 * C1;
    BtailParams p{};
    btail_layer(dm, p, B, H, W, C1, C3, stride, dbg);
    uint16_t* a1 = dm.alloc<uint16_t>((size_t)p.M * C1);
    float* zero = zeros<float>(dm, 4096);
    if (!dm.ok) return fail(OPD_ENOMEM, "bench alloc failed");
    ConvGemmParams c[3] = {};
    c[0].x = p.x1; c[0].w = p.w1; c[0].out = a1;
    conv_geometry(c[0], B, H, W, C1, p.OH, p.OW, C1, 3, 3, stride, 1);
    c[1].x = a1; c[1].w = p.w2p; c[1].res16 = p.res; c[1].out = p.y;
    conv_geometry(c[1], B, p.OH, p.OW, C1, p.OH, p.OW, C2, 1, 1, 1, 0);
    c[2].x = p.y; c[2].w = p.w3p; c[2].out = p.z;
    conv_geometry(c[2], B, p.OH, p.OW, C2, p.OH, p.OW, C3 ? C3 : 64, 1, 1, 1, 0);
    for (auto& q : c) { q.bias = p.b1; q.zero16 = zero; q.relu = 1; }
    for (int k = 0; k < 4; ++k) {
        us_out[k] = 0.f;
        if (k == 3 && !C3) break;
        if (k > 0 && dbg) continue;
        RCCHK(time_launches(2, iters, [&] { return k == 0 ? opd_launch_btail(p, nullptr) : opd_launch_conv_gemm(c[k - 1], nullptr); }, &us_out[k]));
    }
    return OPD_OK;
}

TAPI int opd_test_bench_btail_sc2(int B, int H, int W, int C3, int dbg, int iters, float* us_out) {
    const int C1 = 128, C2 = 512, Csc = 256;
    if (!opd_btail_sc_supported(C1, C3, Csc, 2)) return fail(OPD_EINVAL, "btail_sc2: unsupported C3");
    DevMem dm;
    BtailParams p{};
    btail_layer(dm, p, B, H, W, C1, C3, 2, dbg);
    p.res = nullptr;
    p.xs = filled16(dm, (size_t)B * H * W * Csc, 0x2c);
    p.wsc = filled16(dm, (size_t)C2 * Csc, 0x1c);
    uint16_t* a1 = dm.alloc<uint16_t>((size_t)p.M * C1);
    uint16_t* w2sc = filled16(dm, (size_t)C2 * (C1 + Csc), 0x1c);
    float* zero = zeros<float>(dm, 4096);
    if (!dm.ok) return fail(OPD_ENOMEM, "bench alloc failed");
    ConvGemmParams c[3] = {};
    c[0].x = p.x1; c[0].w = p.w1; c[0].out = a1;
    conv_geometry(c[0], B, H, W, C1, p.OH, p.OW, C1, 3, 3, 2, 1);
    c[1].x = a1; c[1].w = w2sc; c[1].out = p.y; c[1].x2 = p.xs;
    conv_geometry(c[1], B, p.OH, p.OW, C1, p.OH, p.OW, C2, 1, 1, 1, 0);
    c[1].K = C1 + Csc; c[1].K1 = C1; c[1].H2 = H; c[1].W2 = W; c[1].Cin2 = Csc; c[1].stride2 = 2;
    c[2].x = p.y; c[2].w = p.w3p; c[2].out = p.z;
    conv_geometry(c[2], B, p.OH, p.OW, C2, p.OH, p.OW, C3 ? C3 : 64, 1, 1, 1, 0);
    for (auto& q : c) { q.dtype = g_test_dtype; q.bias = p.b1; q.zero16 = zero; q.relu = 1; }
    for (int k = 0; k < 4; ++k) {
        us_out[k] = 0.f;
        if (k > 0 && dbg) continue;
        RCCHK(time_launches(2, iters, [&] { return k == 0 ? opd_launch_btail(p, nullptr) : opd_launch_conv_gemm(c[k - 1], nullptr); }, &us_out[k]));
    }
    return OPD_OK;
}

static void attention_operands(DevMem& dm, AttnParams& p, const uint16_t* q, const uint16_t* k, const uint16_t* v, int B, int heads, int Lq, int Lk,
                               int ldq, int ldkv, float scale) {
    p.dtype = g_test_dtype;
    p.q = dm.up(q, (size_t)B * Lq * ldq);
    p.k = dm.up(k, (size_t)B * Lk * ldkv);
    p.v = dm.up(v, (size_t)B * Lk * ldkv);
    p.o = dm.alloc<uint16_t>((size_t)B * Lq * heads * 32);
    p.B = B; p.heads = heads; p.Lq = Lq; p.Lk = Lk; p.ldq = ldq; p.ldk = p.ldv = ldkv; p.ldo = heads * 32; p.scale = scale;
}

TAPI int opd_test_bench_attention(const uint16_t* q, const uint16_t* k, const uint16_t* v, int B, int heads, int Lq, int Lk, int ldq, int ldkv,
                                  float scale, int iters, float* us_out) {
    DevMem dm;
    AttnParams p{};
    attention_operands(dm, p, q, k, v, B, heads, Lq, Lk, ldq, ldkv, scale);
    if (!dm.ok) return fail(OPD_ENOMEM, "bench alloc failed");
    return time_launches(3, iters, [&] { return opd_launch_attention(p, nullptr); }, us_out);
}

TAPI int opd_test_trace_attention(const uint16_t* q, const uint16_t* k, const uint16_t* v, int B, int heads, int Lq, int Lk, int ldq, int ldkv,
                                  float scale, unsigned long long* trace_out, int max_wgs, int* wgs_out) {
    DevMem dm;
    AttnParams p{};
    attention_operands(dm, p, q, k, v, B, heads, Lq, Lk, ldq, ldkv, scale);
    const int total = ((Lq + 63) / 64) * heads * B, grid = 8 * ((total + 7) / 8);
    unsigned long long* tr = zeros<unsigned long long>(dm, (size_t)grid * 12);
    if (!dm.ok) return fail(OPD_ENOMEM, "trace alloc failed");
    for (int i = 0; i < 2; ++i) HIPCHK(opd_launch_attention(p, nullptr));
    p.trace = tr;
    HIPCHK(opd_launch_attention(p, nullptr));
    HIPCHK(hipDeviceSynchronize());
    const int n = grid < max_wgs ? grid : max_wgs;
    *wgs_out = n;
    return down(trace_out, tr, (size_t)n * 12);
}

TAPI int opd_test_bench_dec(int B, int Q, int Lk, int F, int splits, int iters, float* us5) {
    DevMem dm;
    const int M = B * Q, nchunk = F / OPD_DEC_FFN_CHUNK;
    const size_t n = (size_t)M * 256;
    DecQkvParams a{}; DecSelfParams b{}; AttnParams c{}; DecCrossOutParams d{}; DecFfnParams e{};
    float *vec = zeros<float>(dm, 4096), *h0 = zeros<float>(dm, n), *h1 = zeros<float>(dm, n), *part = zeros<float>(dm, n * nchunk), *tabs = zeros<float>(dm, (size_t)Q * 768), *po = zeros<float>(dm, n * splits),
          *pml = zeros<float>(dm, (size_t)splits * M * 16);
    const size_t nv = (size_t)B * 8 * 8 * 512;
    uint16_t *q16 = zeros<uint16_t>(dm, n), *k16 = zeros<uint16_t>(dm, nv), *vT = zeros<uint16_t>(dm, nv), *qc = zeros<uint16_t>(dm, n);
    uint16_t *w768 = zeros<uint16_t>(dm, 2 * 768 * 256), *w256 = zeros<uint16_t>(dm, 2 * 65536), *wf = zeros<uint16_t>(dm, (size_t)2 * F * 256), *mem = zeros<uint16_t>(dm, (size_t)B * Lk * 512);
    if (!dm.ok) return fail(OPD_ENOMEM, "test alloc failed");
    a.h_in = h0; a.partials = part; a.nsplit = nchunk; a.b2 = vec; a.ln_g = vec; a.ln_b = vec; a.h_out = h1; a.w = w768; a.bias = tabs;
    a.q16 = q16; a.k16 = k16; a.vT = vT; a.M = M; a.Q = Q;
    b.q16 = q16; b.k16 = k16; b.vT = vT; b.h = h1; b.wo = w256; b.bo = vec; b.ln_g = vec; b.ln_b = vec; b.wq = w256;
    b.rbq = tabs; b.qc16 = qc; b.B = B; b.Q = Q; b.scale = 0.17677669f;
    c.q = qc; c.k = mem; c.v = mem + 256; c.B = B; c.heads = 8; c.Lq = Q; c.Lk = Lk; c.ldq = 256; c.ldk = c.ldv = 512; c.ldo = 256; c.scale = 0.17677669f;
    c.splits = splits; c.part_o = po; c.part_ml = pml;
    d.part_o = po; d.part_ml = pml; d.splits = splits; d.res = h1; d.h = h1; d.wo = w256; d.bo = vec; d.ln_g = vec; d.ln_b = vec; d.M = M;
    e.h = h1; e.w1 = wf; e.b1 = vec; e.w2 = wf; e.partials = part; e.M = M; e.F = F;
    for (int k = 0; k < 5; ++k) {
        auto run = [&]() -> hipError_t {
            switch (k) {
                case 0: return opd_launch_dec_qkv(a, nullptr);
                case 1: return opd_launch_dec_self(b, nullptr);
                case 2: return opd_launch_attention(c, nullptr);
                case 3: return opd_launch_dec_cross_out(d, nullptr);
                default: return opd_launch_dec_ffn(e, nullptr);
            }
        };
        RCCHK(time_launches(3, iters, run, &us5[k]));
    }
    return OPD_OK;
}

TAPI int opd_test_trace_dec_self(int B, int Q, unsigned long long* trace_out) {
    DevMem dm;
    DecSelfParams b{};
    const size_t n = (size_t)B * Q * 256, nv = (size_t)B * 8 * 8 * 512, stamps = (size_t)((Q + 15) / 16) * B * 8;
    b.q16 = zeros<uint16_t>(dm, n); b.k16 = zeros<uint16_t>(dm, nv); b.vT = zeros<uint16_t>(dm, nv); b.h = zeros<float>(dm, n);
    b.wo = zeros<uint16_t>(dm, 2 * 65536); b.wq = zeros<uint16_t>(dm, 2 * 65536);
    b.bo = b.ln_g = b.ln_b = zeros<float>(dm, 4096);
    b.rbq = zeros<float>(dm, (size_t)Q * 256); b.qc16 = zeros<uint16_t>(dm, n); b.B = B; b.Q = Q; b.scale = 0.17677669f;
    unsigned long long* tr = dm.alloc<unsigned long long>(stamps);
    if (!dm.ok) return fail(OPD_ENOMEM, "test alloc failed");
    for (int i = 0; i < 3; ++i) HIPCHK(opd_launch_dec_self(b, nullptr));
    b.trace = tr;
    HIPCHK(opd_launch_dec_self(b, nullptr));
    HIPCHK(hipDeviceSynchronize());
    return down(trace_out, tr, stamps);
}
```

office_person_detection_vit_amd/csrc/opd_test_model_api.cpp:

```cpp
#include <string.h>

#include <algorithm>
#include <string>
#include <vector>

#include "opd_model.h"
#include "opd_test_util.h"

TAPI uint16_t opd_test_f32_to_f16(float f) { return opd::f32_to_f16(f); }
TAPI float opd_test_f16_to_f32(uint16_t h) { return opd::f16_to_f32(h); }
TAPI int opd_test_normalise_key(const char* in, char* out, int cap) {
    const std::string k = opd::normalise_key(in);
    if ((int)k.size() + 1 > cap) return OPD_EINVAL;
    memcpy(out, k.c_str(), k.size() + 1);
    return OPD_OK;
}
TAPI int opd_test_inspect_checkpoint(const char* path, int32_t* info8) {
    opd::StateDict sd;
    std::string err;
    int rc = opd::load_safetensors(path, &sd, &err);
    if (rc) return fail(rc, err);
    opd::Arch a;
    rc = opd::infer_arch(sd, &a, &err);
    if (rc) return fail(rc, err);
    for (int i = 0; i < 4; ++i) info8[i] = a.depths[i];
    info8[4] = a.enc_layers; info8[5] = a.dec_layers; info8[6] = a.queries; info8[7] = a.ncls;
    return OPD_OK;
}
TAPI int opd_test_resize_coeffs(int in_size, int out_size, int32_t* bounds, int32_t* coeffs, int coeffs_capacity) {
    std::vector<int32_t> b, k;
    int ksize = 0;
    opd_resize_coeffs(in_size, out_size, &b, &k, &ksize);
    if ((int)k.size() > coeffs_capacity) return fail(OPD_EINVAL, "coefficient buffer too small");
    memcpy(bounds, b.data(), b.size() * 4);
    memcpy(coeffs, k.data(), k.size() * 4);
    return ksize;
}
TAPI int opd_test_valid_prefix(int valid, int in, int out) { return valid_prefix(valid, in, out); }
TAPI int opd_test_sine_pos_embed(int h, int w, int vh, int vw, int D, float* out) {
    if (!out || h < 1 || w < 1 || vh < 1 || vw < 1 || vh > h || vw > w || D < 2 || (D & 1)) return fail(OPD_EINVAL, "bad sine_pos_embed arguments");
    std::vector<float> pos;
    sine_pos_embed(h, w, vh, vw, D, &pos);
    memcpy(out, pos.data(), pos.size() * sizeof(float));
    return OPD_OK;
}
TAPI int opd_test_round_f16_diffused(float* w, int rows, int taps, int cin) {
    if (!w || rows < 0 || taps < 1 || cin < 1) return fail(OPD_EINVAL, "opd_test_round_f16_diffused: bad arguments");
    opd::round_f16_diffused(w, (size_t)rows, taps, cin);
    return OPD_OK;
}
static int test_trunk_plan(const int* depths, int max_batch, int flags, int B, int H, int W, int num_cus, const Switches& sw, int max_steps, TrunkPlan* out) {
    if (!depths || B < 1 || H < 1 || W < 1 || num_cus < 1) return fail(OPD_EINVAL, "bad trunk_plan arguments");
    Arch a;
    std::vector<Block> blocks;
    auto conv = [](int cin, int cout, int k, int stride) {
        Conv c;
        c.Cin = cin; c.Cout = cout; c.KH = c.KW = k; c.stride = stride; c.pad = k / 2; c.K = k * k * cin;
        return c;
    };
    for (int s = 0, cin = 64; s < 4; ++s) {
        a.depths[s] = depths[s];
        if (depths[s] < 1) return fail(OPD_EINVAL, "every stage needs a block");
        const int cout = a.hidden[s], mid = cout / 4;
        for (int l = 0; l < depths[s]; ++l) {
            const int stride = (l == 0 && s > 0) ? 2 : 1;
            Block b;
            b.has_sc = l == 0;
            if (b.has_sc) b.sc = conv(cin, cout, 1, stride);
            b.c0 = conv(cin, mid, 1, 1); b.c1 = conv(mid, mid, 3, stride); b.c2 = conv(mid, cout, 1, 1);
            blocks.push_back(b);
            cin = cout;
        }
    }
    if ((int)blocks.size() > max_steps) return fail(OPD_EINVAL, "steps_out too small");
    opd_config cfg{};
    cfg.struct_size = sizeof(opd_config); cfg.max_batch = max_batch; cfg.max_height = H; cfg.max_width = W; cfg.flags = flags;
    *out = plan_trunk(a, blocks, cfg, sw, B, down2(down2(H)), down2(down2(W)), num_cus, false, 0, true);
    return (int)blocks.size();
}
TAPI int opd_test_trunk_plan(const int* depths, int max_batch, int flags, int B, int H, int W, int num_cus, int* steps_out, int max_steps, int* split_out) {
    if (!steps_out || !split_out) return fail(OPD_EINVAL, "bad trunk_plan arguments");
    TrunkPlan plan;
    const int n = test_trunk_plan(depths, max_batch, flags, B, H, W, num_cus, Switches{}, max_steps, &plan);
    if (n < 0) return n;
    for (size_t i = 0; i < plan.steps.size(); ++i) {
        const TrunkStep& t = plan.steps[i];
        const int row[7] = {t.path, t.sc, t.res, t.store, t.C3, t.rev, t.rev_b};
        memcpy(steps_out + 7 * i, row, sizeof(row));
    }
    *split_out = plan.split;
    return n;
}
TAPI int opd_test_trunk_plan_one_launch(const int* depths, int max_batch, int flags, int B, int H, int W, int num_cus, int* steps_out, int* one_out, int max_steps) {
    if (!one_out) return fail(OPD_EINVAL, "bad trunk_plan arguments");
    TrunkPlan plan;
    const int n = test_trunk_plan(depths, max_batch, flags, B, H, W, num_cus, read_switches(flags), max_steps, &plan);
    if (n < 0) return n;
    for (size_t i = 0; i < plan.steps.size(); ++i) {
        const TrunkStep& t = plan.steps[i];
        const int row[7] = {t.path, t.sc, t.res, t.store, t.C3, t.rev, t.rev_b}, one[3] = {t.one_launch, t.one_C3, t.one_rev};
        if (steps_out) memcpy(steps_out + 7 * i, row, sizeof(row));
        memcpy(one_out + 3 * i, one, sizeof(one));
    }
    return n;
}
TAPI int opd_test_transformer_plan(const int* arch7, int max_batch, int max_height, int max_width, int flags, int B, int H, int W, int* head_out, int* enc_out,
                                   int max_layers) {
    if (!arch7 || !head_out || !enc_out || max_batch < 1 || max_height < 32 || max_width < 32 || B < 1 || H < 1 || W < 1)
        return fail(OPD_EINVAL, "bad transformer_plan arguments");
    Arch a;
    a.d_model = arch7[0]; a.heads = arch7[1]; a.ffn = arch7[2]; a.enc_layers = arch7[3]; a.dec_layers = arch7[4]; a.queries = arch7[5]; a.ncls = arch7[6];
    if (a.enc_layers < 1 || a.dec_layers < 1 || a.enc_layers > max_layers) return fail(OPD_EINVAL, "transformer_plan: layer counts");
    opd_config cfg{};
    cfg.struct_size = sizeof(opd_config); cfg.max_batch = max_batch; cfg.max_height = max_height; cfg.max_width = max_width; cfg.flags = flags;
    const size_t px = frame_bounds(cfg).lvl[5];
    int fh = H, fw = W;
    for (int k = 0; k < 5; ++k) { fh = down2(fh); fw = down2(fw); }
    const TransformerPlan t = plan_transformer(a, cfg, read_switches(flags), px, B, fh, fw);
    const int head[14] = {t.shadow, t.small_enc, t.enc_splits, t.proj_splits, t.kv_launch, t.dec_fused, t.dec_splits, t.dec0, t.dec_small_m,
                          t.dec_oproj, t.heads, t.heads_ln3, t.heads_ln, (int)((size_t)max_batch * px)};
    memcpy(head_out, head, sizeof(head));
    for (size_t i = 0; i < t.enc.size(); ++i) {
        const EncStep& e = t.enc[i];
        const int row[5] = {e.qkv, e.oproj, e.ffn, e.splits, e.tail};
        memcpy(enc_out + 5 * i, row, sizeof(row));
    }
    return (int)t.enc.size();
}

TAPI int opd_test_set_fuse_gemm_ln(opd_detr* m, int on) {
    if (!m) return fail(OPD_EINVAL, "null model handle");
    m->sw.fuse_gemm_ln = on ? 1 : 0;
    m->sw.small_m_gemm = on ? 1 : 0;
    m->sw.deep_fc2 = on ? 1 : 0;
    m->sw.fuse_dec0 = on ? 1 : 0;
    m->sw.fused_dec = on ? 1 : 0;
    if (fill_qc0(m) != OPD_OK) return OPD_EHIP;
    drop_graphs(m);
    return OPD_OK;
}
TAPI int opd_test_set_fuse_btail(opd_detr* m, int on) {
    if (!m) return fail(OPD_EINVAL, "null model handle");
    m->sw.fuse_btail = (on & 1) ? 1 : 0;
    m->sw.fuse_shortcut = (on & 2) ? 1 : 0;
    drop_graphs(m);
    return OPD_OK;
}
TAPI int opd_test_set_pos_shadow(opd_detr* m, int on) {
    if (!m) return fail(OPD_EINVAL, "null model handle");
    m->sw.pos_shadow = on ? 1 : 0;
    drop_graphs(m);
    return OPD_OK;
}
TAPI int opd_test_set_fuse_stem_pool(opd_detr* m, int on) {
    if (!m) return fail(OPD_EINVAL, "null model handle");
    m->sw.fuse_stem_pool = (on & 1) ? 1 : 0;
    m->sw.fuse_prep = (on & 2) ? 1 : 0;
    drop_graphs(m);
    return OPD_OK;
}

TAPI int opd_test_set_alloc_poison(int byte) {
    g_alloc_poison = byte < 0 ? -1 : (byte & 255);
    return OPD_OK;
}
TAPI int opd_test_check_redzones(opd_detr* m) {
    ApiScope api_scope;
    if (!m) return fail(OPD_EINVAL, "null model handle");
    HIPCHK(hipSetDevice(m->device));
    HIPCHK(hipDeviceSynchronize());
    std::vector<unsigned char> h(OPD_REDZONE);
    int bad = 0;
    std::string first;
    auto scan = [&](const std::vector<RedZoned>& v, const char* what) -> int {
        for (size_t i = 0; i < v.size(); ++i)
            for (int side = 0; side < 2; ++side) {
                const unsigned char* z = static_cast<const unsigned char*>(v[i].base) + (side ? OPD_REDZONE + v[i].bytes : 0);
                RCCHK(down(h.data(), z, OPD_REDZONE));
                size_t lo = OPD_REDZONE, hi = 0;
                for (size_t k = 0; k < OPD_REDZONE; ++k)
                    if (h[k] != (unsigned char)v[i].poison) { lo = std::min(lo, k); hi = k; }
                if (lo <= hi) {
                    if (!bad++) first = std::string(what) + " buffer #" + std::to_string(i) + " (" + std::to_string(v[i].bytes) + " bytes): " +
                                        (side ? "zone BEHIND it" : "zone IN FRONT of it") + " overwritten at zone offsets " + std::to_string(lo) + " .. " + std::to_string(hi);
                }
            }
        return OPD_OK;
    };
    RCCHK(scan(m->zoned, "handle"));
    if (m->weights) RCCHK(scan(m->weights->zoned, "weight-set"));
    if (bad) g_err = first;
    return bad;
}
TAPI int opd_test_set_graph_guard(int on) {
    g_graph_guard = on ? 1 : 0;
    return OPD_OK;
}
TAPI int opd_test_set_taps(opd_detr* m, int on) {
    ApiScope api_scope;
    if (!m) return fail(OPD_EINVAL, "null model handle");
    HIPCHK(hipSetDevice(m->device));
    if (on && !m->d_taps) RCCHK(dalloc(m, &m->d_taps, (size_t)OPD_MAX_TAPS * OPD_TAP_BLOCKS, false));
    m->taps = on ? 1 : 0;
    drop_graphs(m);
    return OPD_OK;
}
TAPI int opd_test_read_taps(opd_detr* m, unsigned long long* sums, int cap, char* names, int names_cap) {
    ApiScope api_scope;
    if (!m || !sums || !m->d_taps) return fail(OPD_EINVAL, "opd_test_read_taps: taps are not enabled");
// ... 17 lines not shown
```

office_person_detection_vit_amd/csrc/opd_weights.cpp:

```cpp
#include <algorithm>

#include "opd_model.h"

namespace opd {

template <typename E>
static int upload(opd_detr* m, E** dst, const std::vector<E>& v) {
    RCCHK(dalloc(m, dst, v.size(), true));
    HIPCHK(hipMemcpy(*dst, v.data(), v.size() * sizeof(E), hipMemcpyHostToDevice));
    return OPD_OK;
}
int upload_f32(opd_detr* m, float** dst, const std::vector<float>& v) { return upload(m, dst, v); }
int upload_fold(opd_detr* m, const float* d_x, const std::vector<float>& w, const std::vector<float>& b, int rows, int N, int K, float** out) {
    float *d_w = nullptr, *d_b = nullptr;
    RCCHK(upload_f32(m, &d_w, w));
    RCCHK(upload_f32(m, &d_b, b));
    RCCHK(dalloc(m, out, (size_t)rows * N, true));
    HIPCHK(opd_launch_gemm_f32(d_x, d_w, d_b, *out, rows, N, K, N, m->stream));
    return OPD_OK;
}
static std::vector<f16_t> to_h16(const opd_detr* m, const std::vector<float>& v) {
    std::vector<f16_t> h(v.size());
    if (m->dtype == OPD_DT_BF16) for (size_t i = 0; i < v.size(); ++i) h[i] = f32_to_bf16(v[i]);
    else for (size_t i = 0; i < v.size(); ++i) h[i] = f32_to_f16(v[i]);
// ... 44 lines not shown
            for (int kh = 0; kh < KH; ++kh)
                for (int kw = 0; kw < KW; ++kw) wt[o * Kt + (size_t)(kh * KW + kw) * Cin + ci] = w.data[(((size_t)o * Cin + ci) * KH + kh) * KW + kw] * scale[o];
    if (m->sw.wround) round_f16_diffused(wt.data(), (size_t)Cout, KH * KW, Cin, m->dtype == OPD_DT_BF16);
    if (c->stem) {
        std::vector<float> padded((size_t)Cout * 256, 0.f);
        for (int o = 0; o < Cout; ++o)
            for (int kh = 0; kh < 7; ++kh)
                for (int kw = 0; kw < 7; ++kw)
                    for (int ci = 0; ci < 3; ++ci) padded[(size_t)o * 256 + kh * 32 + kw * 4 + ci] = wt[(size_t)o * 147 + (kh * 7 + kw) * 3 + ci];
        wt.swap(padded);
    }
    std::vector<f16_t> w16 = to_h16(m, wt);
    RCCHK(upload(m, &c->w, w16));
    if (conv_has_kperm(*c)) {
        std::vector<f16_t> wp(w16.size());
        opd_permute_k32(w16.data(), wp.data(), Cout, Cin);
        RCCHK(upload(m, &c->wp, wp));
    }
    RCCHK(upload_f32(m, &c->bias, bias));
    if (host) { host->w16 = std::move(w16); host->bias = std::move(bias); }
    return OPD_OK;
}

static int make_lin(opd_detr* m, const StateDict& sd, const std::string& prefix, Lin* l) {
    const HostTensor& w = T(sd, prefix + ".weight");
    l->N = (int)w.shape[0]; l->K = (int)w.shape[1];
    RCCHK(upload_f16(m, &l->w, w.data));
    RCCHK(upload_f32(m, &l->b, T(sd, prefix + ".bias").data));
    return OPD_OK;
}
static int make_ln(opd_detr* m, const StateDict& sd, const std::string& prefix, LNp* l) {
    RCCHK(upload_f32(m, &l->g, T(sd, prefix + ".weight").data));
    RCCHK(upload_f32(m, &l->b, T(sd, prefix + ".bias").data));
    return OPD_OK;
}
static void append(std::vector<float>& dst, const std::vector<float>& src) { dst.insert(dst.end(), src.begin(), src.end()); }

static void cat3(const StateDict& sd, const std::string& p, int D, std::vector<float>* w_full, std::vector<float>* w_pos, std::vector<float>* b_cat) {
    w_full->clear(); w_pos->clear(); b_cat->clear();
    for (const char* pr : {".q_proj", ".k_proj", ".v_proj"}) { append(*w_full, T(sd, p + pr + ".weight").data); append(*b_cat, T(sd, p + pr + ".bias").data); }
    append(*w_pos, T(sd, p + ".q_proj.weight").data); append(*w_pos, T(sd, p + ".k_proj.weight").data);
    w_pos->resize(w_pos->size() + (size_t)D * D, 0.f);
}

static int build_backbone(opd_detr* m, const StateDict& sd) {
    const std::string bb = "model.backbone.model.";
    RCCHK(make_conv(m, sd, bb + "embedder.embedder", 2, &m->stem));
    for (int s = 0; s < 4; ++s) {
        m->stage_first.push_back((int)m->blocks.size());
        for (int l = 0; l < m->arch.depths[s]; ++l) {
            const std::string p = bb + "encoder.stages." + std::to_string(s) + ".layers." + std::to_string(l);
            const int stride = (l == 0 && s > 0) ? 2 : 1;
            Block b;
            ConvHost h2, hs;
            b.has_sc = sd.count(p + ".shortcut.convolution.weight") > 0;
            if (b.has_sc) RCCHK(make_conv(m, sd, p + ".shortcut", stride, &b.sc, &hs));
            RCCHK(make_conv(m, sd, p + ".layer.0", 1, &b.c0));
            RCCHK(make_conv(m, sd, p + ".layer.1", stride, &b.c1));
            RCCHK(make_conv(m, sd, p + ".layer.2", 1, &b.c2, &h2));
            if (block_has_bias2sc(b)) {
                std::vector<float> b2 = h2.bias;
                for (size_t j = 0; j < b2.size(); ++j) b2[j] += hs.bias[j];
                RCCHK(upload_f32(m, &b.bias2sc, b2));
                if (block_has_w2sc(b)) {
                    const size_t K1 = (size_t)b.c2.K, K2 = (size_t)b.sc.K, N = (size_t)b.c2.Cout;
                    std::vector<f16_t> cat(N * (K1 + K2));
                    for (size_t n = 0; n < N; ++n) {
                        memcpy(&cat[n * (K1 + K2)], &h2.w16[n * K1], K1 * 2);
                        memcpy(&cat[n * (K1 + K2) + K1], &hs.w16[n * K2], K2 * 2);
                    }
                    RCCHK(upload(m, &b.w2sc, cat));
                }
            }
            m->blocks.push_back(b);
        }
    }
    const HostTensor& w = T(sd, "model.input_projection.weight");
    m->proj.Cin = (int)w.shape[1]; m->proj.Cout = (int)w.shape[0]; m->proj.K = m->proj.Cin;
    RCCHK(upload_f16(m, &m->proj.w, w.data));
    RCCHK(upload_f32(m, &m->proj.bias, T(sd, "model.input_projection.bias").data));
    return OPD_OK;
}

static int build_encoder(opd_detr* m, const StateDict& sd) {
    const Arch& a = m->arch;
    m->enc.resize(a.enc_layers); m->h_enc_cat_w.resize(a.enc_layers); m->h_enc_cat_b.resize(a.enc_layers);
    for (int i = 0; i < a.enc_layers; ++i) {
        const std::string p = "model.encoder.layers." + std::to_string(i);
        EncLayer& L = m->enc[i];
        std::vector<float> wfull;
        cat3(sd, p + ".self_attn", a.d_model, &wfull, &m->h_enc_cat_w[i], &m->h_enc_cat_b[i]);
        RCCHK(upload_f16(m, &L.wqkv, wfull));
        RCCHK(upload_f32(m, &L.bqkv, m->h_enc_cat_b[i]));
        RCCHK(make_lin(m, sd, p + ".self_attn.o_proj", &L.o));
        RCCHK(make_ln(m, sd, p + ".self_attn_layer_norm", &L.ln1));
        RCCHK(make_lin(m, sd, p + ".mlp.fc1", &L.fc1));
        RCCHK(make_lin(m, sd, p + ".mlp.fc2", &L.fc2));
        RCCHK(make_ln(m, sd, p + ".final_layer_norm", &L.ln2));
    }
    return OPD_OK;
}

static int build_encoder_ffn_packs(opd_detr* m, const StateDict& sd, const std::vector<float>& kv_full) {
    const Arch& a = m->arch;
    if (!enc_has_ffn_pack(a)) return OPD_OK;
    const int D = 256, L = a.dec_layers;
    for (int i = 0; i < a.enc_layers; ++i) {
        EncLayer& E = m->enc[i];
        const std::string p = "model.encoder.layers." + std::to_string(i);
        std::vector<float> wt, bt;
        const int tail = enc_pack_tail(a, i, &E.tail_pos);
        E.tail_ld = tail * D;
        if (i + 1 < a.enc_layers) {
            const std::string n = "model.encoder.layers." + std::to_string(i + 1) + ".self_attn.";
            for (const char* pr : {"q_proj", "k_proj", "v_proj"}) { append(wt, T(sd, n + pr + ".weight").data); append(bt, T(sd, n + pr + ".bias").data); }
            for (int t = 0; t < 3; ++t) E.tail_col[t] = t * D;
        } else if (tail) {
            for (int kv = 0; kv < 2; ++kv)
                for (int l = 0; l < L; ++l) {
                    wt.insert(wt.end(), kv_full.begin() + (size_t)(2 * l + kv) * D * D, kv_full.begin() + (size_t)(2 * l + kv + 1) * D * D);
                    bt.insert(bt.end(), m->h_kv_cat_b.begin() + (size_t)(2 * l + kv) * D, m->h_kv_cat_b.begin() + (size_t)(2 * l + kv + 1) * D);
                    E.tail_col[kv * L + l] = (2 * l + kv) * D;
                }
        }
        RCCHK(upload_encffn(m, &E.ffn_pack, T(sd, p + ".mlp.fc1.weight").data, T(sd, p + ".mlp.fc1.bias").data, T(sd, p + ".mlp.fc2.weight").data, a.ffn, wt, bt, tail,
                            T(sd, p + ".self_attn.o_proj.weight").data));
    }
    return OPD_OK;
}

static int build_decoder_layer0(opd_detr* m, const StateDict& sd) {
    const int D = m->arch.d_model, Q = m->arch.queries;
    const std::string p0 = "model.decoder.layers.0";
    const auto& bv = T(sd, p0 + ".self_attn.v_proj.bias").data;
    const auto& wo = T(sd, p0 + ".self_attn.o_proj.weight").data;
    const auto& bo = T(sd, p0 + ".self_attn.o_proj.bias").data;
    const auto& g = T(sd, p0 + ".self_attn_layer_norm.weight").data;
    const auto& be = T(sd, p0 + ".self_attn_layer_norm.bias").data;
    std::vector<float> x(D), c(D);
    for (int n = 0; n < D; ++n) {
        float acc = 0.f;
        for (int k = 0; k < D; ++k) acc += wo[(size_t)n * D + k] * bv[k];
        x[n] = acc + bo[n];
    }
    float mean = 0.f, var = 0.f;
    for (int n = 0; n < D; ++n) mean += x[n];
    mean /= (float)D;
    for (int n = 0; n < D; ++n) var += (x[n] - mean) * (x[n] - mean);
    var /= (float)D;
    const float rstd = 1.0f / sqrtf(var + 1e-5f);
    for (int n = 0; n < D; ++n) c[n] = (x[n] - mean) * rstd * g[n] + be[n];
    RCCHK(upload_f32(m, &m->dec0_h, c));
    const auto& qpos = T(sd, "model.query_position_embeddings.weight").data;
    const auto& wq = T(sd, p0 + ".encoder_attn.q_proj.weight").data;
    const auto& bq = T(sd, p0 + ".encoder_attn.q_proj.bias").data;
    std::vector<float> q0((size_t)Q * D);
    for (int q = 0; q < Q; ++q)
        for (int n = 0; n < D; ++n) {
            double acc = bq[n];
            for (int k = 0; k < D; ++k) acc += ((double)c[k] + qpos[(size_t)q * D + k]) * wq[(size_t)n * D + k];
            q0[(size_t)q * D + n] = (float)acc;
        }
    return upload_f16(m, &m->qc0, q0);
}

static int build_decoder(opd_detr* m, const StateDict& sd, std::vector<float>* kv_full) {
    const Arch& a = m->arch;
    const int D = a.d_model, Q = a.queries;
    const std::vector<float> zerosW((size_t)D * D, 0.f);
    float* d_qpos = nullptr;
    RCCHK(upload_f32(m, &d_qpos, T(sd, "model.query_position_embeddings.weight").data));
    m->dec.resize(a.dec_layers);
    for (int i = 0; i < a.dec_layers; ++i) {
        const std::string p = "model.decoder.layers." + std::to_string(i);
        DecLayer& L = m->dec[i];
        std::vector<float> wfull, wpos, bcat;
        cat3(sd, p + ".self_attn", D, &wfull, &wpos, &bcat);
        RCCHK(upload_f16(m, &L.wqkv, wfull));
        RCCHK(upload_fold(m, d_qpos, wpos, bcat, Q, 768, D, &L.rb_self));
        RCCHK(make_lin(m, sd, p + ".self_attn.o_proj", &L.so));
        RCCHK(make_ln(m, sd, p + ".self_attn_layer_norm", &L.ln1));
        RCCHK(upload_f16(m, &L.wq_c, T(sd, p + ".encoder_attn.q_proj.weight").data));
        RCCHK(upload_fold(m, d_qpos, T(sd, p + ".encoder_attn.q_proj.weight").data, T(sd, p + ".encoder_attn.q_proj.bias").data, Q, D, D, &L.rb_q));
        append(*kv_full, T(sd, p + ".encoder_attn.k_proj.weight").data);
        append(*kv_full, T(sd, p + ".encoder_attn.v_proj.weight").data);
        append(m->h_kv_cat_w, T(sd, p + ".encoder_attn.k_proj.weight").data);
        append(m->h_kv_cat_w, zerosW);
        append(m->h_kv_cat_b, T(sd, p + ".encoder_attn.k_proj.bias").data);
        append(m->h_kv_cat_b, T(sd, p + ".encoder_attn.v_proj.bias").data);
        RCCHK(make_lin(m, sd, p + ".encoder_attn.o_proj", &L.co));
        RCCHK(make_ln(m, sd, p + ".encoder_attn_layer_norm", &L.ln2));
        RCCHK(make_lin(m, sd, p + ".mlp.fc1", &L.fc1));
        RCCHK(make_lin(m, sd, p + ".mlp.fc2", &L.fc2));
        RCCHK(make_ln(m, sd, p + ".final_layer_norm", &L.ln3));
        if (dec_has_frag_weights(a)) {
            RCCHK(upload_frag(m, &L.wqkv_f, wfull, 3 * D, D));
            RCCHK(upload_frag(m, &L.so_f, T(sd, p + ".self_attn.o_proj.weight").data, D, D));
            RCCHK(upload_frag(m, &L.wqc_f, T(sd, p + ".encoder_attn.q_proj.weight").data, D, D));
// ... 53 lines not shown
```

Baseline: 3190.

## Fold softmax scale and log2e into encoder Q projection weights

Pre-multiplies the encoder Q projection weights and bias by 1/sqrt(d_head)*log2(e) at load time and adds a PRE variant of the attention kernel. The variant seeds the QK MFMA accumulator with the negated running max, so the per-element scale multiply and max subtraction before exp2 are dropped. This aims to cut VALU work in the softmax inner loop of encoder attention. It adds kernel instantiations, and the lazy rescale logic changes, which could affect numerics. The decoder flag dec_q_pre is never set, so only encoder attention uses the new path.

```diff
diff --git a/office_person_detection_vit_amd/_capi.py b/office_person_detection_vit_amd/_capi.py
--- a/office_person_detection_vit_amd/_capi.py
+++ b/office_person_detection_vit_amd/_capi.py
@@ -293,6 +293,11 @@
     "opd_test_dec_self": (C.c_int, [C.c_void_p] * 10 + [C.c_int, C.c_int, C.c_float, C.c_void_p]),
     "opd_test_attention_map": (C.c_int, [C.c_void_p, C.c_int, C.c_void_p, C.c_int, C.c_void_p] + [C.c_int] * 3 + [C.c_float, C.c_void_p, C.c_int, C.c_void_p]),
     "opd_test_attention_split": (C.c_int, [C.c_void_p] * 3 + [C.c_int] * 4 + [C.c_float, C.c_int, C.c_void_p, C.c_int, C.c_void_p, C.c_void_p]),
+    "opd_test_attention_pre": (C.c_int, [C.c_void_p] * 4 + [C.c_int] * 4 + [C.c_float, C.c_void_p, C.c_int, C.c_int]),
+    "opd_test_attention_split_pre": (C.c_int, [C.c_void_p] * 3 + [C.c_int] * 4 + [C.c_float, C.c_int, C.c_void_p, C.c_int, C.c_void_p, C.c_void_p, C.c_int]),
+    "opd_test_bench_attention_pre": (C.c_int, [C.c_void_p] * 3 + [C.c_int] * 6 + [C.c_float, C.c_int, C.POINTER(C.c_float), C.c_int]),
+    "opd_test_trace_attention_pre": (C.c_int, [C.c_void_p] * 3 + [C.c_int] * 6 + [C.c_float, C.c_void_p, C.c_int, C.POINTER(C.c_int), C.c_int]),
+    "opd_test_transformer_plan_attn": (C.c_int, [C.c_void_p] + [C.c_int] * 7 + [C.c_void_p, C.c_void_p, C.c_int]),
     "opd_test_dec_cross_out": (C.c_int, [C.c_void_p, C.c_void_p, C.c_int, C.c_void_p, C.c_int] + [C.c_void_p] * 4 + [C.c_int, C.c_void_p]),
     "opd_test_dec_ffn": (C.c_int, [C.c_void_p] * 4 + [C.c_int, C.c_int, C.c_void_p]),
     "opd_test_bench_dec": (C.c_int, [C.c_int] * 6 + [C.POINTER(C.c_float)]),
diff --git a/office_person_detection_vit_amd/csrc/kernels_attn.hip b/office_person_detection_vit_amd/csrc/kernels_attn.hip
--- a/office_person_detection_vit_amd/csrc/kernels_attn.hip
+++ b/office_person_detection_vit_amd/csrc/kernels_attn.hip
@@ -35,7 +35,7 @@
         }                                                                                                    \
     } while (0)
 
-template <bool MASKED, int KT, bool TRACE = false, bool SPLIT = false>
+template <bool MASKED, int KT, bool TRACE = false, bool SPLIT = false, bool PRE = false>
 __global__ __launch_bounds__(256) void attention_kernel(AttnParams p) {
     constexpr int NKT = KT / 16;
     constexpr int RPT = KT / 64;
@@ -86,6 +86,8 @@
         asm volatile("s_memtime %0\n\ts_waitcnt lgkmcnt(0)" : "=s"(tbegin)::"memory");
         tlast = tbegin;
     }
+    float4v nref = float4v{0.f, 0.f, 0.f, 0.f};
+    float thr = -INFINITY;
     float m_ref = -INFINITY;
     float4v oacc[2] = {float4v{0.f, 0.f, 0.f, 0.f}, float4v{0.f, 0.f, 0.f, 0.f}};
     float4v lacc = float4v{0.f, 0.f, 0.f, 0.f};
@@ -119,7 +121,8 @@
 #pragma unroll
         for (int kt = 0; kt < NKT; ++kt) {
             const half8 kf = *reinterpret_cast<const half8*>(Kl + kt * 1024 + lane * 16);
-            s[kt] = OPD_MFMA_16x16x32(kf, qf, float4v{0.f, 0.f, 0.f, 0.f});
+            if constexpr (PRE) s[kt] = OPD_MFMA_16x16x32(kf, qf, nref);
+            else s[kt] = OPD_MFMA_16x16x32(kf, qf, float4v{0.f, 0.f, 0.f, 0.f});
         }
         float mx = -INFINITY;
         if (MASKED) {
@@ -148,6 +151,30 @@
                     mx = fmaxf(mx, s[kt][r]);
                 }
         }
+        if constexpr (PRE) {
+            if (__any(mx > thr)) {
+                const float mq = xmax16_32(mx);
+                const bool up = mq > thr, first = m_ref == -INFINITY;
+                const float m_new = up ? (first ? mq : m_ref + mq) : m_ref;
+                const float delta = up ? (first ? mq : m_new - m_ref) : 0.f;
+                const float alpha = up ? __builtin_amdgcn_exp2f(m_ref - m_new) : 1.0f;
+#pragma unroll
+                for (int kt = 0; kt < NKT; ++kt)
+#pragma unroll
+                    for (int r = 0; r < 4; ++r) s[kt][r] -= delta;
+#pragma unroll
+                for (int dt = 0; dt < 2; ++dt)
+#pragma unroll
+                    for (int r = 0; r < 4; ++r) oacc[dt][r] *= alpha;
+#pragma unroll
+                for (int r = 0; r < 4; ++r) lacc[r] *= alpha;
+                if (up) {
+                    m_ref = m_new;
+                    thr = LAZY_T;
+                    nref = float4v{-m_new, -m_new, -m_new, -m_new};
+                }
+            }
+        } else
         if (__any(mx * scale2 > m_ref + LAZY_T)) {
             const float mq = xmax16_32(mx) * scale2;
             const bool up = mq > m_ref + LAZY_T;
@@ -164,6 +191,12 @@
         ATTN_STAMP(1);
         const float mn = (SPLIT && MASKED && m_ref == -INFINITY) ? 0.f : -m_ref;
         const float2v sc2 = {scale2, scale2}, mneg = {mn, mn};
+        if constexpr (PRE) {
+#pragma unroll
+            for (int kt = 0; kt < NKT; ++kt)
+#pragma unroll
+                for (int r = 0; r < 4; ++r) s[kt][r] = __builtin_amdgcn_exp2f(s[kt][r]);
+        } else
 #pragma unroll
         for (int kt = 0; kt < NKT; ++kt)
 #pragma unroll
@@ -253,7 +286,10 @@
         if ((size_t)p.B * p.Lk * p.ldk * 2 >= (1ull << 32) || (size_t)p.B * p.Lk * p.ldv * 2 >= (1ull << 32)) return hipErrorInvalidValue;
         const int total = ((p.Lq + 63) / 64) * p.heads * p.B * p.splits;
         dim3 grid(8 * ((total + 7) / 8));
-        if (p.key_valid) OPD_LAUNCH((attention_kernel<true, 128, false, true>), grid, dim3(256), 0, stream, p);
+        if (p.q_prescaled) {
+            if (p.key_valid) OPD_LAUNCH((attention_kernel<true, 128, false, true, true>), grid, dim3(256), 0, stream, p);
+            else OPD_LAUNCH((attention_kernel<false, 128, false, true, true>), grid, dim3(256), 0, stream, p);
+        } else if (p.key_valid) OPD_LAUNCH((attention_kernel<true, 128, false, true>), grid, dim3(256), 0, stream, p);
         else OPD_LAUNCH((attention_kernel<false, 128, false, true>), grid, dim3(256), 0, stream, p);
         return hipGetLastError();
     }
@@ -264,7 +300,16 @@
     dim3 grid(8 * ((total + 7) / 8));
     const bool wide = p.Lq <= 128 && p.Lk > 128;
     if (p.trace) {
-        OPD_LAUNCH((attention_kernel<false, 64, true>), grid, dim3(256), 0, stream, p);
+        if (p.q_prescaled) OPD_LAUNCH((attention_kernel<false, 64, true, false, true>), grid, dim3(256), 0, stream, p);
+        else OPD_LAUNCH((attention_kernel<false, 64, true>), grid, dim3(256), 0, stream, p);
+    } else if (p.q_prescaled) {
+        if (p.key_valid) {
+            if (wide) OPD_LAUNCH((attention_kernel<true, 128, false, false, true>), grid, dim3(256), 0, stream, p);
+            else OPD_LAUNCH((attention_kernel<true, 64, false, false, true>), grid, dim3(256), 0, stream, p);
+        } else {
+            if (wide) OPD_LAUNCH((attention_kernel<false, 128, false, false, true>), grid, dim3(256), 0, stream, p);
+            else OPD_LAUNCH((attention_kernel<false, 64, false, false, true>), grid, dim3(256), 0, stream, p);
+        }
     } else if (p.key_valid) {
         if (wide) OPD_LAUNCH((attention_kernel<true, 128>), grid, dim3(256), 0, stream, p);
         else OPD_LAUNCH((attention_kernel<true, 64>), grid, dim3(256), 0, stream, p);
diff --git a/office_person_detection_vit_amd/csrc/opd_api.cpp b/office_person_detection_vit_amd/csrc/opd_api.cpp
--- a/office_person_detection_vit_amd/csrc/opd_api.cpp
+++ b/office_person_detection_vit_amd/csrc/opd_api.cpp
@@ -427,6 +427,8 @@
     env("OPD_ENC_TAIL", &sw.enc_tail);
     env("OPD_ENC_FRONT", &sw.enc_front);
     env("OPD_HEADS2", &sw.heads2);
+    env("OPD_ATTN_PRE", &sw.attn_pre);
+    sw.attn_pre = sw.attn_pre != 0;
     env("OPD_DBG_DEC_LAYERS", &sw.dbg_dec_layers);
     env("OPD_DBG_BTAIL", &sw.dbg_btail);
     env("OPD_DBG_SKIP", &sw.dbg_skip);
diff --git a/office_person_detection_vit_amd/csrc/opd_kernels.h b/office_person_detection_vit_amd/csrc/opd_kernels.h
--- a/office_person_detection_vit_amd/csrc/opd_kernels.h
+++ b/office_person_detection_vit_amd/csrc/opd_kernels.h
@@ -352,6 +352,7 @@
     int splits;
     float *part_o, *part_ml;
     int dtype;
+    int q_prescaled;
 };
 hipError_t opd_launch_attention(const AttnParams& p, hipStream_t stream);
 
diff --git a/office_person_detection_vit_amd/csrc/opd_model.cpp b/office_person_detection_vit_amd/csrc/opd_model.cpp
--- a/office_person_detection_vit_amd/csrc/opd_model.cpp
+++ b/office_person_detection_vit_amd/csrc/opd_model.cpp
@@ -208,9 +208,9 @@
     return p;
 }
 static AttnParams attn_params(const Fwd& c, const f16_t* q, int ldq, const f16_t* k, int ldk, const f16_t* v, int ldv, f16_t* o, int ldo, int Lq, int Lk,
-                              const int32_t* key_valid, int key_row) {
+                              const int32_t* key_valid, int key_row, bool q_pre = false) {
     AttnParams p{}; p.dtype = c.m->dtype;
-    p.key_valid = key_valid; p.key_row = key_row;
+    p.key_valid = key_valid; p.key_row = key_row; p.q_prescaled = q_pre ? 1 : 0;
     p.q = q; p.k = k; p.v = v; p.o = o; p.B = c.B; p.heads = c.m->arch.heads; p.Lq = Lq; p.Lk = Lk;
     p.ldq = ldq; p.ldk = ldk; p.ldv = ldv; p.ldo = ldo;
     p.scale = 1.0f / sqrtf((float)(c.m->arch.d_model / c.m->arch.heads));
@@ -298,9 +298,9 @@
 }
 
 static int run_attn(const Fwd& c, const f16_t* q, int ldq, const f16_t* k, int ldk, const f16_t* v, int ldv, f16_t* o, int Lq, int Lk,
-                    const int32_t* key_valid = nullptr, int key_row = 0) {
+                    const int32_t* key_valid = nullptr, int key_row = 0, bool q_pre = false) {
     const int D = c.m->arch.d_model;
-    const AttnParams p = attn_params(c, q, ldq, k, ldk, v, ldv, o, D, Lq, Lk, key_valid, key_row);
+    const AttnParams p = attn_params(c, q, ldq, k, ldk, v, ldv, o, D, Lq, Lk, key_valid, key_row, q_pre);
     return c.launch(CLS_ATTN, attn_flops(p), [&] { return opd_launch_attention(p, c.stream); }, {{"attention", o, (size_t)c.B * Lq * D * 2}});
 }
 
@@ -405,6 +405,7 @@
         e.splits = e.ffn == FFN_FC1_SPLITK ? splits_of(F) : 0;
         e.tail = ffn_one && t.shadow && sw.enc_tail && (!last || M * NKV * 2 < (1ull << 32)) ? enc_pack_tail(a, i) : 0;
         prev_tail = e.tail > 0;
+        e.q_pre = sw.attn_pre ? 1 : 0;
     }
     t.kv_launch = !prev_tail;
     t.dec0 = sw.fuse_dec0 && row256;
@@ -605,7 +606,7 @@
         const EncLayer& L = m->enc[i];
         const EncStep& e = tp.enc[i];
         if (e.qkv == QKV_LAUNCH) RCCHK(run_pos_proj(c, L.wqkv, L.bqkv, c.plan->rb_enc[i], c.enc_bias_ptrs[i], 3 * D, 3 * D, 2 * D, m->d_qkv16));
-        RCCHK(run_attn(c, m->d_qkv16, 3 * D, m->d_qkv16 + D, 3 * D, m->d_qkv16 + 2 * D, 3 * D, m->d_attn16, c.hw, c.hw, c.d_keyv, c.fw));
+        RCCHK(run_attn(c, m->d_qkv16, 3 * D, m->d_qkv16 + D, 3 * D, m->d_qkv16 + 2 * D, 3 * D, m->d_attn16, c.hw, c.hw, c.d_keyv, c.fw, e.q_pre != 0));
         if (e.oproj == OPROJ_GEMM_LN) {
             RCCHK(run_gemm_ln(c, m->d_attn16, L.o.w, L.o.b, M, D, m->d_x32, L.ln1, m->d_x32, m->d_x16));
         } else if (e.oproj == OPROJ_GEMM_THEN_LN) {
@@ -667,7 +668,7 @@
             RCCHK(c.launch(CLS_GEMM, 4.0 * Md * (double)D * D + 4.0 * B * (double)a.heads * Q * Q * 32, [&] { return opd_launch_dec_self(sp, c.stream); },
                            {{"dec_self_h", hbuf[cur], (size_t)Md * D * 4}}));
         }
-        AttnParams ap = attn_params(c, qd, D, m->d_memkv16 + (size_t)i * 2 * D, c.NKV, m->d_memkv16 + (size_t)i * 2 * D + D, c.NKV, nullptr, D, Q, c.hw, c.d_keyv, c.fw);
+        AttnParams ap = attn_params(c, qd, D, m->d_memkv16 + (size_t)i * 2 * D, c.NKV, m->d_memkv16 + (size_t)i * 2 * D + D, c.NKV, nullptr, D, Q, c.hw, c.d_keyv, c.fw, tp.dec_q_pre);
         ap.splits = S; ap.part_o = m->d_part_o; ap.part_ml = m->d_part_ml;
         RCCHK(c.launch(CLS_ATTN, attn_flops(ap), [&] { return opd_launch_attention(ap, c.stream); }, {{"dec_cross_part", m->d_part_o, (size_t)S * Md * D * 4}}));
         DecCrossOutParams cp{};
diff --git a/office_person_detection_vit_amd/csrc/opd_model.h b/office_person_detection_vit_amd/csrc/opd_model.h
--- a/office_person_detection_vit_amd/csrc/opd_model.h
+++ b/office_person_detection_vit_amd/csrc/opd_model.h
@@ -99,6 +99,7 @@
     int fused_dec = 1;
     int dec_splits = 3;
     int heads2 = 1;
+    int attn_pre = 1;
     int fuse_btail = 1;
     int fuse_shortcut = 1;
     int dual_over_tail = 1;
@@ -150,6 +151,7 @@
     int qkv, oproj, ffn;
     int splits;
     int tail;
+    int q_pre;
 };
 struct TransformerPlan {
     bool shadow = false;
@@ -160,6 +162,7 @@
     bool kv_launch = true;
     bool dec_fused = false;
     int dec_splits = 0;
+    bool dec_q_pre = false;
     bool dec0 = false;
     bool dec_small_m = false;
     int dec_oproj = OPROJ_GEMM_LN;
@@ -170,6 +173,7 @@
 struct FrameBounds { size_t lvl[6], side[6]; };
 FrameBounds frame_bounds(const opd_config& cfg);
 TransformerPlan plan_transformer(const Arch& a, const opd_config& cfg, const Switches& sw, size_t stage4_px, int B, int fh, int fw);
+inline float attn_q_scale(const Arch& a) { return (1.0f / sqrtf((float)(a.d_model / a.heads))) * 1.44269504088896340736f; }
 Switches read_switches(int flags);
 
 }
diff --git a/office_person_detection_vit_amd/csrc/opd_test_api.cpp b/office_person_detection_vit_amd/csrc/opd_test_api.cpp
--- a/office_person_detection_vit_amd/csrc/opd_test_api.cpp
+++ b/office_person_detection_vit_amd/csrc/opd_test_api.cpp
@@ -627,9 +627,10 @@
     return D;
 }
 static int run_attention(const uint16_t* q, const uint16_t* k, const uint16_t* v, uint16_t* o, int B, int heads, int Lq, int Lk, float scale,
-                         const int32_t* key_valid, int key_row) {
+                         const int32_t* key_valid, int key_row, int q_prescaled = 0) {
     DevMem dm;
     AttnParams p{};
+    p.q_prescaled = q_prescaled ? 1 : 0;
     const size_t n = (size_t)B * Lq * attention_params(dm, p, q, k, v, B, heads, Lq, Lk, scale, key_valid, key_row);
     p.o = dm.alloc<uint16_t>(n);
     if (!dm.ok) return fail(OPD_ENOMEM, "test alloc failed");
@@ -645,10 +646,15 @@
                                    int Lk, float scale, const int32_t* key_valid, int key_row) {
     return run_attention(q, k, v, o, B, heads, Lq, Lk, scale, key_valid, key_row);
 }
-TAPI int opd_test_attention_split(const uint16_t* q, const uint16_t* k, const uint16_t* v, int B, int heads, int Lq, int Lk, float scale, int splits,
-                                  const int32_t* key_valid, int key_row, float* part_o, float* part_ml) {
+TAPI int opd_test_attention_pre(const uint16_t* q, const uint16_t* k, const uint16_t* v, uint16_t* o, int B, int heads, int Lq, int Lk, float scale,
+                                const int32_t* key_valid, int key_row, int q_prescaled) {
+    return run_attention(q, k, v, o, B, heads, Lq, Lk, scale, key_valid, key_row, q_prescaled);
+}
+static int run_attention_split(const uint16_t* q, const uint16_t* k, const uint16_t* v, int B, int heads, int Lq, int Lk, float scale, int splits,
+                               const int32_t* key_valid, int key_row, float* part_o, float* part_ml, int q_prescaled) {
     DevMem dm;
     AttnParams p{};
+    p.q_prescaled = q_prescaled ? 1 : 0;
     const int D = attention_params(dm, p, q, k, v, B, heads, Lq, Lk, scale, key_valid, key_row);
     const size_t no = (size_t)splits * B * Lq * D, nm = (size_t)splits * B * Lq * heads * 2;
     p.part_o = dm.alloc<float>(no); p.part_ml = dm.alloc<float>(nm); p.splits = splits;
@@ -657,6 +663,14 @@
     HIPCHK(hipDeviceSynchronize());
     RCCHK(down(part_o, p.part_o, no));
     return down(part_ml, p.part_ml, nm);
+}
+TAPI int opd_test_attention_split(const uint16_t* q, const uint16_t* k, const uint16_t* v, int B, int heads, int Lq, int Lk, float scale, int splits,
+                                  const int32_t* key_valid, int key_row, float* part_o, float* part_ml) {
+    return run_attention_split(q, k, v, B, heads, Lq, Lk, scale, splits, key_valid, key_row, part_o, part_ml, 0);
+}
+TAPI int opd_test_attention_split_pre(const uint16_t* q, const uint16_t* k, const uint16_t* v, int B, int heads, int Lq, int Lk, float scale, int splits,
+                                      const int32_t* key_valid, int key_row, float* part_o, float* part_ml, int q_prescaled) {
+    return run_attention_split(q, k, v, B, heads, Lq, Lk, scale, splits, key_valid, key_row, part_o, part_ml, q_prescaled);
 }
 
 TAPI int opd_test_attention_map(const uint16_t* q, int ldq, const uint16_t* k, int ldk, const int32_t* sel, int nsel, int heads, int Lk, float scale,
diff --git a/office_person_detection_vit_amd/csrc/opd_test_bench_api.cpp b/office_person_detection_vit_amd/csrc/opd_test_bench_api.cpp
--- a/office_person_detection_vit_amd/csrc/opd_test_bench_api.cpp
+++ b/office_person_detection_vit_amd/csrc/opd_test_bench_api.cpp
@@ -179,19 +179,29 @@
     p.B = B; p.heads = heads; p.Lq = Lq; p.Lk = Lk; p.ldq = ldq; p.ldk = p.ldv = ldkv; p.ldo = heads * 32; p.scale = scale;
 }
 
+static int bench_attention(const uint16_t* q, const uint16_t* k, const uint16_t* v, int B, int heads, int Lq, int Lk, int ldq, int ldkv, float scale, int iters,
+                           float* us_out, int q_prescaled) {
+    DevMem dm;
+    AttnParams p{};
+    p.q_prescaled = q_prescaled ? 1 : 0;
+    attention_operands(dm, p, q, k, v, B, heads, Lq, Lk, ldq, ldkv, scale);
+    if (!dm.ok) return fail(OPD_ENOMEM, "bench alloc failed");
+    return time_launches(3, iters, [&] { return opd_launch_attention(p, nullptr); }, us_out);
+}
 TAPI int opd_test_bench_attention(const uint16_t* q, const uint16_t* k, const uint16_t* v, int B, int heads, int Lq, int Lk, int ldq, int ldkv,
                                   float scale, int iters, float* us_out) {
+    return bench_attention(q, k, v, B, heads, Lq, Lk, ldq, ldkv, scale, iters, us_out, 0);
+}
+TAPI int opd_test_bench_attention_pre(const uint16_t* q, const uint16_t* k, const uint16_t* v, int B, int heads, int Lq, int Lk, int ldq, int ldkv,
+                                      float scale, int iters, float* us_out, int q_prescaled) {
+    return bench_attention(q, k, v, B, heads, Lq, Lk, ldq, ldkv, scale, iters, us_out, q_prescaled);
+}
+
+static int trace_attention(const uint16_t* q, const uint16_t* k, const uint16_t* v, int B, int heads, int Lq, int Lk, int ldq, int ldkv, float scale,
+                           unsigned long long* trace_out, int max_wgs, int* wgs_out, int q_prescaled) {
     DevMem dm;
     AttnParams p{};
-    attention_operands(dm, p, q, k, v, B, heads, Lq, Lk, ldq, ldkv, scale);
-    if (!dm.ok) return fail(OPD_ENOMEM, "bench alloc failed");
-    return time_launches(3, iters, [&] { return opd_launch_attention(p, nullptr); }, us_out);
-}
-
-TAPI int opd_test_trace_attention(const uint16_t* q, const uint16_t* k, const uint16_t* v, int B, int heads, int Lq, int Lk, int ldq, int ldkv,
-                                  float scale, unsigned long long* trace_out, int max_wgs, int* wgs_out) {
-    DevMem dm;
-    AttnParams p{};
+    p.q_prescaled = q_prescaled ? 1 : 0;
     attention_operands(dm, p, q, k, v, B, heads, Lq, Lk, ldq, ldkv, scale);
     const int total = ((Lq + 63) / 64) * heads * B, grid = 8 * ((total + 7) / 8);
     unsigned long long* tr = zeros<unsigned long long>(dm, (size_t)grid * 12);
@@ -203,6 +213,14 @@
     const int n = grid < max_wgs ? grid : max_wgs;
     *wgs_out = n;
     return down(trace_out, tr, (size_t)n * 12);
+}
+TAPI int opd_test_trace_attention(const uint16_t* q, const uint16_t* k, const uint16_t* v, int B, int heads, int Lq, int Lk, int ldq, int ldkv,
+                                  float scale, unsigned long long* trace_out, int max_wgs, int* wgs_out) {
+    return trace_attention(q, k, v, B, heads, Lq, Lk, ldq, ldkv, scale, trace_out, max_wgs, wgs_out, 0);
+}
+TAPI int opd_test_trace_attention_pre(const uint16_t* q, const uint16_t* k, const uint16_t* v, int B, int heads, int Lq, int Lk, int ldq, int ldkv,
+                                      float scale, unsigned long long* trace_out, int max_wgs, int* wgs_out, int q_prescaled) {
+    return trace_attention(q, k, v, B, heads, Lq, Lk, ldq, ldkv, scale, trace_out, max_wgs, wgs_out, q_prescaled);
 }
 
 TAPI int opd_test_bench_dec(int B, int Q, int Lk, int F, int splits, int iters, float* us5) {
diff --git a/office_person_detection_vit_amd/csrc/opd_test_model_api.cpp b/office_person_detection_vit_amd/csrc/opd_test_model_api.cpp
--- a/office_person_detection_vit_amd/csrc/opd_test_model_api.cpp
+++ b/office_person_detection_vit_amd/csrc/opd_test_model_api.cpp
@@ -104,10 +104,9 @@
     }
     return n;
 }
-TAPI int opd_test_transformer_plan(const int* arch7, int max_batch, int max_height, int max_width, int flags, int B, int H, int W, int* head_out, int* enc_out,
-                                   int max_layers) {
-    if (!arch7 || !head_out || !enc_out || max_batch < 1 || max_height < 32 || max_width < 32 || B < 1 || H < 1 || W < 1)
-        return fail(OPD_EINVAL, "bad transformer_plan arguments");
+static int test_transformer_plan(const int* arch7, int max_batch, int max_height, int max_width, int flags, int B, int H, int W, int max_layers, TransformerPlan* out,
+                                 size_t* px_out) {
+    if (!arch7 || max_batch < 1 || max_height < 32 || max_width < 32 || B < 1 || H < 1 || W < 1) return fail(OPD_EINVAL, "bad transformer_plan arguments");
     Arch a;
     a.d_model = arch7[0]; a.heads = arch7[1]; a.ffn = arch7[2]; a.enc_layers = arch7[3]; a.dec_layers = arch7[4]; a.queries = arch7[5]; a.ncls = arch7[6];
     if (a.enc_layers < 1 || a.dec_layers < 1 || a.enc_layers > max_layers) return fail(OPD_EINVAL, "transformer_plan: layer counts");
@@ -116,7 +115,16 @@
     const size_t px = frame_bounds(cfg).lvl[5];
     int fh = H, fw = W;
     for (int k = 0; k < 5; ++k) { fh = down2(fh); fw = down2(fw); }
-    const TransformerPlan t = plan_transformer(a, cfg, read_switches(flags), px, B, fh, fw);
+    *out = plan_transformer(a, cfg, read_switches(flags), px, B, fh, fw);
+    *px_out = px;
+    return OPD_OK;
+}
+TAPI int opd_test_transformer_plan(const int* arch7, int max_batch, int max_height, int max_width, int flags, int B, int H, int W, int* head_out, int* enc_out,
+                                   int max_layers) {
+    if (!head_out || !enc_out) return fail(OPD_EINVAL, "bad transformer_plan arguments");
+    TransformerPlan t;
+    size_t px = 0;
+    RCCHK(test_transformer_plan(arch7, max_batch, max_height, max_width, flags, B, H, W, max_layers, &t, &px));
     const int head[14] = {t.shadow, t.small_enc, t.enc_splits, t.proj_splits, t.kv_launch, t.dec_fused, t.dec_splits, t.dec0, t.dec_small_m,
                           t.dec_oproj, t.heads, t.heads_ln3, t.heads_ln, (int)((size_t)max_batch * px)};
     memcpy(head_out, head, sizeof(head));
@@ -125,6 +133,16 @@
         const int row[5] = {e.qkv, e.oproj, e.ffn, e.splits, e.tail};
         memcpy(enc_out + 5 * i, row, sizeof(row));
     }
+    return (int)t.enc.size();
+}
+TAPI int opd_test_transformer_plan_attn(const int* arch7, int max_batch, int max_height, int max_width, int flags, int B, int H, int W, int* enc_q_pre_out,
+                                        int* dec_q_pre_out, int max_layers) {
+    if (!enc_q_pre_out || !dec_q_pre_out) return fail(OPD_EINVAL, "bad transformer_plan arguments");
+    TransformerPlan t;
+    size_t px = 0;
+    RCCHK(test_transformer_plan(arch7, max_batch, max_height, max_width, flags, B, H, W, max_layers, &t, &px));
+    for (size_t i = 0; i < t.enc.size(); ++i) enc_q_pre_out[i] = t.enc[i].q_pre;
+    *dec_q_pre_out = t.dec_q_pre ? 1 : 0;
     return (int)t.enc.size();
 }
 
diff --git a/office_person_detection_vit_amd/csrc/opd_weights.cpp b/office_person_detection_vit_amd/csrc/opd_weights.cpp
--- a/office_person_detection_vit_amd/csrc/opd_weights.cpp
+++ b/office_person_detection_vit_amd/csrc/opd_weights.cpp
@@ -150,14 +150,24 @@
     return OPD_OK;
 }
 
+static void scale_q_rows(const opd_detr* m, std::vector<float>& v, size_t n) {
+    if (!m->sw.attn_pre) return;
+    const float c = attn_q_scale(m->arch);
+    for (size_t j = 0; j < n; ++j) v[j] *= c;
+}
+
 static int build_encoder(opd_detr* m, const StateDict& sd) {
     const Arch& a = m->arch;
+    const size_t D = (size_t)a.d_model;
     m->enc.resize(a.enc_layers); m->h_enc_cat_w.resize(a.enc_layers); m->h_enc_cat_b.resize(a.enc_layers);
     for (int i = 0; i < a.enc_layers; ++i) {
         const std::string p = "model.encoder.layers." + std::to_string(i);
         EncLayer& L = m->enc[i];
         std::vector<float> wfull;
         cat3(sd, p + ".self_attn", a.d_model, &wfull, &m->h_enc_cat_w[i], &m->h_enc_cat_b[i]);
+        scale_q_rows(m, wfull, D * D);
+        scale_q_rows(m, m->h_enc_cat_w[i], D * D);
+        scale_q_rows(m, m->h_enc_cat_b[i], D);
         RCCHK(upload_f16(m, &L.wqkv, wfull));
         RCCHK(upload_f32(m, &L.bqkv, m->h_enc_cat_b[i]));
         RCCHK(make_lin(m, sd, p + ".self_attn.o_proj", &L.o));
@@ -182,6 +192,8 @@
         if (i + 1 < a.enc_layers) {
             const std::string n = "model.encoder.layers." + std::to_string(i + 1) + ".self_attn.";
             for (const char* pr : {"q_proj", "k_proj", "v_proj"}) { append(wt, T(sd, n + pr + ".weight").data); append(bt, T(sd, n + pr + ".bias").data); }
+            scale_q_rows(m, wt, (size_t)D * D);
+            scale_q_rows(m, bt, (size_t)D);
             for (int t = 0; t < 3; ++t) E.tail_col[t] = t * D;
         } else if (tail) {
             for (int kv = 0; kv < 2; ++kv)
```

After: 3178. About the same (-0.4%).
